# vlad17/runlmc

Measured on AMD Instinct MI355X. Metric: kronecker_toeplitz_mvms_per_sec, higher is better.
Workload: dtype f64

## Files before the change

### runlmc_amd/csrc/rl_direct.h

```cpp
#pragma once
#include "rl_device.h"

#define RL_DZ_VB 4

static __global__ void __launch_bounds__(256)
k_dz_mix(const double* __restrict__ part, const int* __restrict__ run_ptr, int nvec, int D, int r,
         const double* __restrict__ Zt, double* __restrict__ zhat) {
    RL_SMEM(smem);
    double* S = reinterpret_cast<double*>(smem);
    const int tid = threadIdx.x, Dr = D * r;
    const int v0 = blockIdx.x * RL_DZ_VB;
    for (int e = tid; e < Dr; e += 256) {
        const int b = e / r, j = e - b * r;
        const int c0 = run_ptr[b], c1 = run_ptr[b + 1];
#pragma unroll
        for (int k = 0; k < RL_DZ_VB; ++k) {
            const int v = v0 + k < nvec ? v0 + k : nvec - 1;
            const double* src = part + (size_t)v * r + j;
            double s = 0.0;
            for (int c = c0; c < c1; ++c) s += src[(size_t)c * nvec * r];
            S[k * Dr + e] = s;
        }
    }
    __syncthreads();
// ... 154 lines not shown
    S[(size_t)v * Dr + e] = s;
}
static __global__ void __launch_bounds__(256)
k_hz_map(const double* __restrict__ S, const double* __restrict__ Zt, int nvec, int Dr,
         double* __restrict__ P) {
    RL_SMEM(smem);
    double* Sl = reinterpret_cast<double*>(smem);
    const int tid = threadIdx.x, e = blockIdx.x * 256 + tid, v0 = blockIdx.y * RL_HZ_VB;
    const int per = (Dr + gridDim.z - 1) / gridDim.z;
    const int f0 = blockIdx.z * per, f1 = f0 + per < Dr ? f0 + per : Dr, flen = f1 > f0 ? f1 - f0 : 0;
    for (int t = tid; t < flen * RL_HZ_VB; t += 256) {
        const int q = t / flen, f = t - q * flen;
        const int v = v0 + q < nvec ? v0 + q : nvec - 1;
        Sl[f * RL_HZ_VB + q] = S[(size_t)v * Dr + f0 + f];
    }
    __syncthreads();
    if (e >= Dr) return;
    double acc[RL_HZ_VB];
#pragma unroll
    for (int q = 0; q < RL_HZ_VB; ++q) acc[q] = 0.0;
    const double* z = Zt + (size_t)f0 * Dr + e;
#pragma unroll 4
    for (int f = 0; f < flen; ++f) {
        const double zf = z[(size_t)f * Dr];
#pragma unroll
        for (int q = 0; q < RL_HZ_VB; ++q) acc[q] = fma(zf, Sl[f * RL_HZ_VB + q], acc[q]);
    }
#pragma unroll
    for (int q = 0; q < RL_HZ_VB; ++q)
        if (v0 + q < nvec) P[((size_t)blockIdx.z * nvec + v0 + q) * Dr + e] = acc[q];
}
static __global__ void __launch_bounds__(256)
k_hz_collect(const double* __restrict__ P, int nvec, int D, int NB, int slices,
             double* __restrict__ zhat, int nvp = 0) {
    const int R = NB * RL_HZ_BLK, Dr = D * R;
    const int e = blockIdx.x * 256 + threadIdx.x, v = blockIdx.y;
    if (e >= Dr) return;
    if (nvp > 0) {
        double s = 0.0;
        if (v < nvec)
            for (int t = 0; t < slices; ++t) s += P[((size_t)t * nvec + v) * Dr + e];
        zhat[(size_t)e * nvp + v] = s;
        return;
    }
    double s = 0.0;
    for (int t = 0; t < slices; ++t) s += P[((size_t)t * nvec + v) * Dr + e];
    const int a = e / R, ig = e - a * R, k = ig / RL_HZ_BLK, i = ig - k * RL_HZ_BLK;
    zhat[(((size_t)k * nvec + v) * D + a) * RL_HZ_BLK + i] = s;
}

template <int NVT, int RT = 2>
__global__ void __launch_bounds__(256)
k_hz_expand_mm(const double* __restrict__ zT, const double* __restrict__ F, int n, int nvec, int nvp,
               int D, int R, const int* __restrict__ out_end, double* __restrict__ out,
               const double* __restrict__ diag, const double* __restrict__ X2) {
    const int tid = threadIdx.x;
    const int vt0 = blockIdx.y * NVT, nvt = nvp / 16 - vt0 < NVT ? nvp / 16 - vt0 : NVT;
    constexpr int WR = 16 * RT;
#if !defined(RL_EMU)
    const int lane = tid & 63, wave = tid >> 6, li = lane & 15, lk = lane >> 4;
    const int r0 = blockIdx.x * (4 * WR) + wave * WR;
    if (r0 >= n) return;
    rp_double4 C[RT][NVT];
#pragma unroll
    for (int rt = 0; rt < RT; ++rt) {
        const int i = r0 + 16 * rt + li;
        const double dg = i < n ? diag[i] : 0.0;
#pragma unroll
        for (int t = 0; t < NVT; ++t) {
            rp_double4 c = rp_double4{0.0, 0.0, 0.0, 0.0};
            if (t < nvt) {
#pragma unroll
                for (int r = 0; r < 4; ++r) {
                    const int v = (vt0 + t) * 16 + lk + 4 * r;
                    c[r] = i < n && v < nvec ? dg * X2[(size_t)v * n + i] : 0.0;
                }
            }
            C[rt][t] = c;
        }
    }
    const int rlast = r0 + WR - 1 < n ? r0 + WR - 1 : n - 1;
    const int dlo = RL_LR_UNIFORM(rp_output_of(out_end, D, r0));
    const int dhi = RL_LR_UNIFORM(rp_output_of(out_end, D, rlast));
    int irow[RT], drow[RT];
#pragma unroll
    for (int rt = 0; rt < RT; ++rt) {
        irow[rt] = r0 + 16 * rt + li;
        drow[rt] = dlo == dhi ? dlo : rp_output_of(out_end, D, irow[rt] < n ? irow[rt] : n - 1);
    }
    for (int d = dlo; d <= dhi; ++d) {
        bool on[RT];
        const double* fr[RT];
#pragma unroll
        for (int rt = 0; rt < RT; ++rt) {
            on[rt] = irow[rt] < n && drow[rt] == d;
            fr[rt] = F + (size_t)lk * n + (irow[rt] < n ? irow[rt] : n - 1);
        }
        const double* za = zT + ((size_t)d * R + lk) * nvp + (size_t)vt0 * 16 + li;
        double a[3][NVT], b[3][RT];
        auto request = [&](int slot, int j) {
            const int jc = j < R ? j : R - 4;
            const double* zj = za + (size_t)jc * nvp;
#pragma unroll
            for (int t = 0; t < NVT; ++t) a[slot][t] = t < nvt ? zj[16 * t] : 0.0;
#pragma unroll
            for (int rt = 0; rt < RT; ++rt) b[slot][rt] = on[rt] ? fr[rt][(size_t)jc * n] : 0.0;
        };
        request(0, 0);
        request(1, 4);
        for (int j0 = 0; j0 < R; j0 += 12) {
#pragma unroll
            for (int u = 0; u < 3; ++u) {
                request((u + 2) % 3, j0 + 4 * u + 8);
#pragma unroll
                for (int t = 0; t < NVT; ++t) {
                    if (t < nvt) {
#pragma unroll
                        for (int rt = 0; rt < RT; ++rt)
                            C[rt][t] = __builtin_amdgcn_mfma_f64_16x16x4f64(a[u][t], b[u][rt], C[rt][t], 0, 0, 0);
                    }
                }
            }
        }
    }
#pragma unroll
    for (int rt = 0; rt < RT; ++rt) {
        const int i = r0 + 16 * rt + li;
#pragma unroll
        for (int t = 0; t < NVT; ++t) {
            if (t < nvt) {
#pragma unroll
                for (int r = 0; r < 4; ++r) {
                    const int v = (vt0 + t) * 16 + lk + 4 * r;
                    if (i < n && v < nvec) out[(size_t)v * n + i] = C[rt][t][r];
                }
            }
        }
    }
#else
    if (tid >= 4 * WR) return;
    const int i = blockIdx.x * (4 * WR) + tid;
    if (i >= n) return;
    const int d = rp_output_of(out_end, D, i);
    for (int t = 0; t < nvt; ++t)
        for (int q = 0; q < 16; ++q) {
            const int v = (vt0 + t) * 16 + q;
            if (v >= nvec) continue;
            double acc = diag[i] * X2[(size_t)v * n + i];
            for (int j = 0; j < R; ++j) acc = fma(F[(size_t)j * n + i], zT[((size_t)d * R + j) * nvp + v], acc);
            out[(size_t)v * n + i] = acc;
        }
#endif
}
```

### runlmc_amd/csrc/rl_exact.h

```cpp
#pragma once
#include "rl_device.h"

#define EX_T 64
#define EX_KC 32
#define EX_LDK (EX_KC + 1)
#define EX_LDT (EX_T + 1)
#define EX_MAX_SLOT 32
#define EX_MAX_COLS 4
#define EX_MAX_D 64

#define EX_RBF 0
#define EX_MATERN32 1
#define EX_STDPERIODIC 2
#define EX_MATERN52 3
#define EX_COSINE 4
#define EX_SCALED 16
#define EX_MAX_FACT 3
#define EX_PRM2 (4 * EX_MAX_SLOT)

#if !defined(RL_EMU)
typedef double ex_d4 __attribute__((ext_vector_type(4)));
#endif

__device__ __forceinline__ bool ex_bad_pivot(double p) { return !(p > 0.0 && p <= 1.7976931348623157e308); }
// ... 99 lines not shown
            k[f] = t[0];
            d[f][0] = t[1];
            if (leaf == EX_STDPERIODIC) d[f][1] = t[2];
        }
    }
    double val = k[0];
#pragma unroll
    for (int f = 1; f < NF; ++f) val = val * k[f];
#pragma unroll
    for (int p = 1; p < 8; ++p) v[p] = 0.0;
#pragma unroll
    for (int f = 0; f < NF; ++f) {
        double others = 1.0;
#pragma unroll
        for (int g = 0; g < NF; ++g)
            if (g != f) others = others * k[g];
        v[1 + 2 * f] = d[f][0] * others;
        v[2 + 2 * f] = d[f][1] * others;
    }
    v[0] = val;
    if (desc & EX_SCALED) {
        const double c = p0[2];
        v[7] = val;
#pragma unroll
        for (int p = 1; p < 7; ++p) v[p] = c * v[p];
        v[0] = c * val;
    }
}

template <int NF>
__device__ __forceinline__ double ex_value(int desc, const double* prm, int q, double r) {
    double v[8];
    ex_eval_fact<NF>(desc, prm, q, r, v);
    return v[0];
}

__device__ __forceinline__ double ex_dist(const double* xa, const double* xb, const int* cols) {
    double s = 0.0;
    for (int c = 0; c < EX_MAX_COLS; ++c) {
        const int col = cols[c];
        if (col < 0) break;
        const double d = xa[col] - xb[col];
        s += d * d;
    }
    return sqrt(s);
}

#define EX_LEAF_COLS (EX_MAX_FACT * EX_MAX_COLS)

__device__ __forceinline__ void ex_eval_sep(int desc, const double* prm, int q, const double* xa,
                                            const double* xb, const int* lq, double v[8]) {
    const int nf = ex_desc_nf(desc);
    const double r0 = ex_dist(xa, xb, lq);
    const double r1 = nf > 1 ? ex_dist(xa, xb, lq + EX_MAX_COLS) : 0.0;
    const double r2 = nf > 2 ? ex_dist(xa, xb, lq + 2 * EX_MAX_COLS) : 0.0;
    ex_eval_fact<EX_MAX_FACT, true>(desc, prm, q, r0, v, r1, r2);
}

template <int NF, bool SEP = false>
__global__ void __launch_bounds__(256)
k_ex_assemble(double* __restrict__ out, long long ldo, int nrows, int ncols,
              const double* __restrict__ Xa, const int* __restrict__ oa,
              const double* __restrict__ Xb, const int* __restrict__ ob, int P, int Q,
              const int* __restrict__ kinds, const double* __restrict__ prm,
              const int* __restrict__ cols, const double* __restrict__ Bm, int D,
              const double* __restrict__ noise, int diag_off, int lower) {
    if (lower && blockIdx.x > blockIdx.y) return;
    const int i0 = blockIdx.y * EX_T, j0 = blockIdx.x * EX_T;
    for (int u = 0; u < 16; ++u) {
        const int e = threadIdx.x + 256 * u;
        const int i = i0 + e / EX_T, j = j0 + e % EX_T;
        if (i >= nrows || j >= ncols) continue;
        const int a = oa[i], b = ob[j];
        double acc = 0.0;
        for (int q = 0; q < Q; ++q) {
            if constexpr (SEP) {
                double v[8];
                ex_eval_sep(kinds[q], prm, q, Xa + (long long)i * P, Xb + (long long)j * P,
                            cols + q * EX_LEAF_COLS, v);
                acc += Bm[((long long)q * D + a) * D + b] * v[0];
                continue;
            }
            const double r = ex_dist(Xa + (long long)i * P, Xb + (long long)j * P, cols + q * EX_MAX_COLS);
            if constexpr (NF == 1) {
                double v[4];
                ex_eval(kinds[q], prm + 4 * q, r, v);
                acc += Bm[((long long)q * D + a) * D + b] * v[0];
            } else {
                acc += Bm[((long long)q * D + a) * D + b] * ex_value<NF>(kinds[q], prm, q, r);
            }
        }
        if (noise && i + diag_off == j) acc += noise[a];
        out[(long long)i * ldo + j] = acc;
    }
}

#define EX_CR_COLS 256
template <int NF, bool SEP = false>
__global__ void __launch_bounds__(EX_CR_COLS)
k_ex_cross_rows(double* __restrict__ out, long long ldo, int nrows, int ncols, int rg,
                const double* __restrict__ Xt, const int* __restrict__ ot,
                const double* __restrict__ Xb, const int* __restrict__ ob, int P, int Q,
                const int* __restrict__ kinds, const double* __restrict__ prm,
                const int* __restrict__ cols, const double* __restrict__ Bm, int D,
                int stage_cols, int ldx) {
    RL_SMEM(smem);
    double* sx = reinterpret_cast<double*>(smem);
    double* sb = sx + (long long)rg * P;
    double* sc = sb + (long long)rg * Q * D;
    const int tid = threadIdx.x;
    const int t0 = blockIdx.y * rg;
    const int nt = nrows - t0 < rg ? nrows - t0 : rg;
    const long long j = (long long)blockIdx.x * EX_CR_COLS + tid;
    for (int e = tid; e < nt * P; e += EX_CR_COLS) sx[e] = Xt[(long long)t0 * P + e];
    const int QD = Q * D;
    for (int e = tid; e < nt * QD; e += EX_CR_COLS) {
        const int t = e / QD, r = e % QD, q = r / D, b = r % D;
        sb[e] = Bm[((long long)q * D + ot[t0 + t]) * D + b];
    }
    const double* xb = Xb + j * P;
    if (stage_cols) {
        if (j < ncols)
            for (int c = 0; c < P; ++c) sc[tid * ldx + c] = xb[c];
        xb = sc + tid * ldx;
    }
    __syncthreads();
    if (j >= ncols) return;
    const int b = ob[j];
    for (int t = 0; t < nt; ++t) {
        const double* xa = sx + t * P;
        const double* bt = sb + (long long)t * QD + b;
        double acc = 0.0;
        for (int q = 0; q < Q; ++q) {
            if constexpr (SEP) {
                double v[8];
                ex_eval_sep(kinds[q], prm, q, xa, xb, cols + q * EX_LEAF_COLS, v);
                acc += bt[q * D] * v[0];
                continue;
            }
            const double r = ex_dist(xa, xb, cols + q * EX_MAX_COLS);
            if constexpr (NF == 1) {
                double v[4];
                ex_eval(kinds[q], prm + 4 * q, r, v);
                acc += bt[q * D] * v[0];
            } else {
                acc += bt[q * D] * ex_value<NF>(kinds[q], prm, q, r);
            }
        }
        out[(long long)(t0 + t) * ldo + j] = acc;
    }
}

#define EX_RD_CHUNKS 64
__global__ void __launch_bounds__(256)
k_ex_rowdot_part(const double* __restrict__ B, const double* __restrict__ X, long long n,
                 double* __restrict__ part) {
    RL_SMEM(smem);
    double* rd = reinterpret_cast<double*>(smem);
    const int tid = threadIdx.x;
    const long long len = (n + EX_RD_CHUNKS - 1) / EX_RD_CHUNKS;
    const long long i0 = (long long)blockIdx.x * len;
    const long long i1 = i0 + len < n ? i0 + len : n;
    const double* b = B + (long long)blockIdx.y * n;
    const double* x = X + (long long)blockIdx.y * n;
    double dot = 0.0, sq = 0.0;
    for (long long i = i0 + tid; i < i1; i += 256) {
        const double xi = x[i];
        dot += b[i] * xi;
        sq += xi * xi;
    }
    rd[tid] = dot;
    rd[256 + tid] = sq;
    __syncthreads();
    for (int w = 128; w > 0; w >>= 1) {
        if (tid < w) {
            rd[tid] += rd[tid + w];
            rd[256 + tid] += rd[256 + tid + w];
        }
        __syncthreads();
    }
    if (tid == 0) {
        double* p = part + ((long long)blockIdx.y * EX_RD_CHUNKS + blockIdx.x) * 2;
        p[0] = rd[0];
        p[1] = rd[256];
    }
}

__global__ void __launch_bounds__(64)
k_ex_rowdot_sum(const double* __restrict__ part, int k, double* __restrict__ dots,
                double* __restrict__ sqn) {
    const int v = blockIdx.x * 64 + threadIdx.x;
    if (v >= k) return;
    double dot = 0.0, sq = 0.0;
    for (int c = 0; c < EX_RD_CHUNKS; ++c) {
        dot += part[((long long)v * EX_RD_CHUNKS + c) * 2];
        sq += part[((long long)v * EX_RD_CHUNKS + c) * 2 + 1];
    }
    dots[v] = dot;
    sqn[v] = sq;
}

__global__ void __launch_bounds__(256)
k_ex_potrf_diag(double* __restrict__ A, long long lda, int k0, int nk, double* __restrict__ logd,
                int* __restrict__ flag) {
    RL_SMEM(smem);
    double* s = reinterpret_cast<double*>(smem);
    const int tid = threadIdx.x;
    double* base = A + (long long)k0 * lda + k0;
    for (int e = tid; e < nk * nk; e += 256) {
        const int r = e / nk, c = e % nk;
        s[r * EX_LDT + c] = c <= r ? base[(long long)r * lda + c] : 0.0;
    }
    __syncthreads();
    for (int j = 0; j < nk; ++j) {
        const double piv = s[j * EX_LDT + j];
        const double d = sqrt(piv);
        if (tid == 0 && ex_bad_pivot(piv) && *flag > k0 + j) *flag = k0 + j;
        if (tid > j && tid < nk) s[tid * EX_LDT + j] /= d;
        __syncthreads();
        const int m = nk - j - 1;
        for (int e = tid; e < m * m; e += 256) {
            const int r = j + 1 + e / m, c = j + 1 + e % m;
            if (c <= r) s[r * EX_LDT + c] -= s[r * EX_LDT + j] * s[c * EX_LDT + j];
        }
        if (tid == 0) s[j * EX_LDT + j] = d;
        __syncthreads();
    }
    for (int e = tid; e < nk * nk; e += 256) {
        const int r = e / nk, c = e % nk;
        if (c <= r) base[(long long)r * lda + c] = s[r * EX_LDT + c];
    }
    if (tid < nk) logd[k0 + tid] = log(s[tid * EX_LDT + tid]);
}

__global__ void __launch_bounds__(64)
k_ex_trsm_panel(double* __restrict__ A, long long lda, int k0, int nk, int r0, int nrows) {
    RL_SMEM(smem);
    double* L = reinterpret_cast<double*>(smem);
    double* X = L + EX_T * EX_LDT;
    const int tid = threadIdx.x;
    const int row0 = r0 + blockIdx.x * EX_T;
    const int rows = nrows - blockIdx.x * EX_T < EX_T ? nrows - blockIdx.x * EX_T : EX_T;
    const double* Lg = A + (long long)k0 * lda + k0;
    double* Xg = A + (long long)row0 * lda + k0;
    for (int e = tid; e < nk * nk; e += 64) {
        const int r = e / nk, c = e % nk;
        L[r * EX_LDT + c] = c <= r ? Lg[(long long)r * lda + c] : 0.0;
    }
    for (int e = tid; e < rows * nk; e += 64) {
        const int r = e / nk, c = e % nk;
        X[r * EX_LDT + c] = Xg[(long long)r * lda + c];
    }
    __syncthreads();
    if (tid < rows) {
        double* x = X + tid * EX_LDT;
        for (int c = 0; c < nk; ++c) {
            double v = x[c];
            for (int t = 0; t < c; ++t) v -= x[t] * L[c * EX_LDT + t];
            x[c] = v / L[c * EX_LDT + c];
        }
    }
    __syncthreads();
    for (int e = tid; e < rows * nk; e += 64) {
        const int r = e / nk, c = e % nk;
        Xg[(long long)r * lda + c] = X[r * EX_LDT + c];
    }
}

__global__ void __launch_bounds__(64)
k_ex_trtri_diag(double* __restrict__ A, long long lda, int j0, int nk) {
    RL_SMEM(smem);
    double* L = reinterpret_cast<double*>(smem);
    double* W = L + EX_T * EX_LDT;
    const int tid = threadIdx.x;
    double* base = A + (long long)j0 * lda + j0;
    for (int e = tid; e < nk * nk; e += 64) {
        const int r = e / nk, c = e % nk;
        L[r * EX_LDT + c] = c <= r ? base[(long long)r * lda + c] : 0.0;
    }
    __syncthreads();
    if (tid < nk) {
        const int c = tid;
        for (int r = 0; r < c; ++r) W[r * EX_LDT + c] = 0.0;
        W[c * EX_LDT + c] = 1.0 / L[c * EX_LDT + c];
        for (int r = c + 1; r < nk; ++r) {
            double v = 0.0;
            for (int t = c; t < r; ++t) v += L[r * EX_LDT + t] * W[t * EX_LDT + c];
            W[r * EX_LDT + c] = -v / L[r * EX_LDT + r];
        }
    }
    __syncthreads();
    for (int e = tid; e < nk * nk; e += 64) {
        const int r = e / nk, c = e % nk;
        base[(long long)r * lda + c] = W[r * EX_LDT + c];
    }
}

__global__ void __launch_bounds__(64)
k_ex_trsv_diag(const double* __restrict__ A, long long lda, int k0, int nk, double* __restrict__ R,
               long long ldr, int nrhs, int trans) {
    RL_SMEM(smem);
    double* L = reinterpret_cast<double*>(smem);
    double* X = L + EX_T * EX_LDT;
    const int tid = threadIdx.x;
    const int v0 = blockIdx.x * EX_T;
    const int nv = nrhs - v0 < EX_T ? nrhs - v0 : EX_T;
    const double* Lg = A + (long long)k0 * lda + k0;
    for (int e = tid; e < nk * nk; e += 64) {
        const int r = e / nk, c = e % nk;
        L[r * EX_LDT + c] = c <= r ? Lg[(long long)r * lda + c] : 0.0;
    }
    for (int e = tid; e < nv * nk; e += 64) {
        const int v = e / nk, c = e % nk;
        X[v * EX_LDT + c] = R[(long long)(v0 + v) * ldr + k0 + c];
    }
    __syncthreads();
    if (tid < nv) {
        double* x = X + tid * EX_LDT;
        if (!trans) {
            for (int c = 0; c < nk; ++c) {
                double s = x[c];
                for (int t = 0; t < c; ++t) s -= L[c * EX_LDT + t] * x[t];
                x[c] = s / L[c * EX_LDT + c];
            }
        } else {
            for (int c = nk - 1; c >= 0; --c) {
                double s = x[c];
                for (int t = c + 1; t < nk; ++t) s -= L[t * EX_LDT + c] * x[t];
                x[c] = s / L[c * EX_LDT + c];
            }
        }
    }
    __syncthreads();
    for (int e = tid; e < nv * nk; e += 64) {
        const int v = e / nk, c = e % nk;
        R[(long long)(v0 + v) * ldr + k0 + c] = X[v * EX_LDT + c];
    }
}

__global__ void __launch_bounds__(256)
k_ex_gemm(double* __restrict__ C, long long ldc, const double* __restrict__ A, long long sai,
          long long sak, const double* __restrict__ B, long long sbj, long long sbk, int M, int N,
          int K, int kchunk, int a_lower, double s, int beta, int lower_tiles,
          double* __restrict__ P) {
    const int tn = blockIdx.x, tm = blockIdx.y, z = blockIdx.z;
    if (lower_tiles && tn > tm) return;
    const int i0 = tm * EX_T, j0 = tn * EX_T;
    const int kb = z * kchunk;
    int ke = K < kb + kchunk ? K : kb + kchunk;
    if (a_lower && ke > i0 + EX_T) ke = i0 + EX_T;
    RL_SMEM(smem);
    double* sA = reinterpret_cast<double*>(smem);
    double* sB = sA + EX_T * EX_LDK;
    const int tid = threadIdx.x;
#if !defined(RL_EMU)
    const int lane = tid & 63, wave = tid >> 6, li = lane & 15, lk = lane >> 4;
    const int wm = (wave >> 1) * 32, wn = (wave & 1) * 32;
    ex_d4 acc[2][2];
#pragma unroll
    for (int a = 0; a < 2; ++a)
#pragma unroll
        for (int b = 0; b < 2; ++b) acc[a][b] = ex_d4{0.0, 0.0, 0.0, 0.0};
#else
    const int er = tid >> 2, ec = (tid & 3) * 16;
    double acc[16];
    for (int c = 0; c < 16; ++c) acc[c] = 0.0;
#endif
    for (int k0 = kb; k0 < ke; k0 += EX_KC) {
        for (int e = tid; e < EX_T * EX_KC; e += 256) {
            int r, k;
            if (sak == 1) { r = e / EX_KC; k = e % EX_KC; } else { k = e / EX_T; r = e % EX_T; }
            const int gi = i0 + r, gk = k0 + k;
            sA[r * EX_LDK + k] = gi < M && gk < ke ? A[(long long)gi * sai + (long long)gk * sak] : 0.0;
            if (sbk == 1) { r = e / EX_KC; k = e % EX_KC; } else { k = e / EX_T; r = e % EX_T; }
            const int gj = j0 + r, gk2 = k0 + k;
            sB[r * EX_LDK + k] = gj < N && gk2 < ke ? B[(long long)gj * sbj + (long long)gk2 * sbk] : 0.0;
        }
        __syncthreads();
#if !defined(RL_EMU)
#pragma unroll
        for (int kk = 0; kk < EX_KC; kk += 4) {
            const double a0 = sA[(wm + li) * EX_LDK + kk + lk];
            const double a1 = sA[(wm + 16 + li) * EX_LDK + kk + lk];
            const double b0 = sB[(wn + li) * EX_LDK + kk + lk];
            const double b1 = sB[(wn + 16 + li) * EX_LDK + kk + lk];
            acc[0][0] = __builtin_amdgcn_mfma_f64_16x16x4f64(a0, b0, acc[0][0], 0, 0, 0);
            acc[0][1] = __builtin_amdgcn_mfma_f64_16x16x4f64(a0, b1, acc[0][1], 0, 0, 0);
            acc[1][0] = __builtin_amdgcn_mfma_f64_16x16x4f64(a1, b0, acc[1][0], 0, 0, 0);
            acc[1][1] = __builtin_amdgcn_mfma_f64_16x16x4f64(a1, b1, acc[1][1], 0, 0, 0);
        }
#else
        for (int c = 0; c < 16; ++c)
            for (int kk = 0; kk < EX_KC; ++kk) acc[c] += sA[er * EX_LDK + kk] * sB[(ec + c) * EX_LDK + kk];
#endif
        __syncthreads();
    }
    auto put = [&](int i, int j, double v) {
        if (i >= M || j >= N) return;
        if (P) {
            P[(long long)z * M * N + (long long)i * N + j] = v;
        } else {
            double* c = C + (long long)i * ldc + j;
            *c = beta ? *c + s * v : s * v;
        }
    };
#if !defined(RL_EMU)
#pragma unroll
    for (int a = 0; a < 2; ++a)
#pragma unroll
        for (int b = 0; b < 2; ++b)
#pragma unroll
            for (int r = 0; r < 4; ++r)
                put(i0 + wm + 16 * a + lk + 4 * r, j0 + wn + 16 * b + li, acc[a][b][r]);
#else
    for (int c = 0; c < 16; ++c) put(i0 + er, j0 + ec + c, acc[c]);
#endif
}

__global__ void __launch_bounds__(256)
k_ex_reduce(double* __restrict__ C, long long ldc, const double* __restrict__ P, int M, int N,
            int nsplit, double s, int beta) {
    const long long e = (long long)blockIdx.x * 256 + threadIdx.x;
    const long long MN = (long long)M * N;
    if (e >= MN) return;
    double acc = 0.0;
    for (int z = 0; z < nsplit; ++z) acc += P[z * MN + e];
    const long long i = e / N, j = e % N;
    double* c = C + i * ldc + j;
    *c = beta ? *c + s * acc : s * acc;
}

__global__ void __launch_bounds__(256)
k_ex_rownorm2(const double* __restrict__ V, long long n, double* __restrict__ out) {
    RL_SMEM(smem);
    double* red = reinterpret_cast<double*>(smem);
    const double* row = V + (long long)blockIdx.x * n;
    double acc = 0.0;
    for (long long i = threadIdx.x; i < n; i += 256) acc += row[i] * row[i];
    red[threadIdx.x] = acc;
    __syncthreads();
    for (int w = 128; w > 0; w >>= 1) {
        if ((int)threadIdx.x < w) red[threadIdx.x] += red[threadIdx.x + w];
        __syncthreads();
    }
    if (threadIdx.x == 0) out[blockIdx.x] = red[0];
}

__global__ void __launch_bounds__(256)
k_ex_sum2(const double* __restrict__ x, int n, double* __restrict__ out) {
    RL_SMEM(smem);
    double* red = reinterpret_cast<double*>(smem);
    double acc = 0.0;
    for (int i = threadIdx.x; i < n; i += 256) acc += x[i];
    red[threadIdx.x] = acc;
    __syncthreads();
    for (int w = 128; w > 0; w >>= 1) {
        if ((int)threadIdx.x < w) red[threadIdx.x] += red[threadIdx.x + w];
        __syncthreads();
    }
    if (threadIdx.x == 0) *out = 2.0 * red[0];
}

template <int NF, bool SEP = false>
__global__ void __launch_bounds__(256)
k_ex_grad_tiles(const double* __restrict__ Kinv, long long n, const double* __restrict__ alpha,
                const int* __restrict__ tiles, const int* __restrict__ bounds,
                const double* __restrict__ X, int P, int Q, const int* __restrict__ kinds,
                const double* __restrict__ prm, const int* __restrict__ cols,
                const int* __restrict__ dslot, int nslot, double* __restrict__ part) {
    RL_SMEM(smem);
    double* red = reinterpret_cast<double*>(smem);
    const int tid = threadIdx.x, w = blockIdx.x;
    const int r0 = tiles[4 * w], c0 = tiles[4 * w + 1], a = tiles[4 * w + 2], b = tiles[4 * w + 3];
    const int re = bounds[a + 1] < r0 + EX_T ? bounds[a + 1] : r0 + EX_T;
    const int ce = bounds[b + 1] < c0 + EX_T ? bounds[b + 1] : c0 + EX_T;
    double mw[16];
    double dsum = 0.0;
    for (int u = 0; u < 16; ++u) {
        const int e = tid + 256 * u;
        const int i = r0 + e / EX_T, j = c0 + e % EX_T;
        double m = 0.0;
        if (i < re && j < ce && (a != b || j <= i)) {
            m = alpha[i] * alpha[j] - Kinv[(long long)i * n + j];
            if (i == j) dsum += m;
            else if (a == b) m *= 2.0;
        }
        mw[u] = m;
    }
    red[nslot * 256 + tid] = dsum;
    for (int q = 0; q < Q; ++q) {
        const int kind = kinds[q];
        const double* pq = prm + 4 * q;
        const int* cq = cols + q * (SEP ? EX_LEAF_COLS : EX_MAX_COLS);
        if constexpr (NF == 1) {
            double s0 = 0.0, s1 = 0.0, s2 = 0.0, s3 = 0.0;
            int np = 0;
            for (int u = 0; u < 16; ++u) {
                const int e = tid + 256 * u;
                const int i = r0 + e / EX_T, j = c0 + e % EX_T;
                if (i >= re || j >= ce || (a == b && j > i)) continue;
                double v[4];
                np = ex_eval(kind, pq, ex_dist(X + (long long)i * P, X + (long long)j * P, cq), v);
                const double m = mw[u];
                s0 += m * v[0];
                s1 += m * v[1];
                if (np > 1) s2 += m * v[2];
                if (np > 2) s3 += m * v[3];
            }
            np = ex_nder(kind);
            red[q * 256 + tid] = s0;
            red[(dslot[q] + 0) * 256 + tid] = s1;
            if (np > 1) red[(dslot[q] + 1) * 256 + tid] = s2;
            if (np > 2) red[(dslot[q] + 2) * 256 + tid] = s3;
        } else {
            double s[8];
#pragma unroll
            for (int p = 0; p < 8; ++p) s[p] = 0.0;
            for (int u = 0; u < 16; ++u) {
                const int e = tid + 256 * u;
                const int i = r0 + e / EX_T, j = c0 + e % EX_T;
                if (i >= re || j >= ce || (a == b && j > i)) continue;
                double v[8];
                if constexpr (SEP)
                    ex_eval_sep(kind, prm, q, X + (long long)i * P, X + (long long)j * P, cq, v);
                else
                    ex_eval_fact<NF>(kind, prm, q, ex_dist(X + (long long)i * P, X + (long long)j * P, cq), v);
                const double m = mw[u];
#pragma unroll
                for (int p = 0; p < 8; ++p) s[p] += m * v[p];
            }
            red[q * 256 + tid] = s[0];
            int slot = dslot[q];
            const int nf = ex_desc_nf(kind);
#pragma unroll
            for (int f = 0; f < NF; ++f) {
                if (f >= nf) continue;
                red[slot * 256 + tid] = s[1 + 2 * f];
                if (ex_leaf_nder(ex_desc_leaf(kind, f)) > 1) red[(slot + 1) * 256 + tid] = s[2 + 2 * f];
                slot += ex_leaf_nder(ex_desc_leaf(kind, f));
            }
            if (kind & EX_SCALED) red[slot * 256 + tid] = s[7];
        }
    }
    __syncthreads();
    if (tid <= nslot) {
        double acc = 0.0;
        for (int t = 0; t < 256; ++t) acc += red[tid * 256 + t];
        part[(long long)w * (nslot + 1) + tid] = acc;
    }
}

__global__ void __launch_bounds__(64)
k_ex_grad_reduce(const double* __restrict__ part, const int* __restrict__ pair_start, int D,
                 int nslot, double* __restrict__ out) {
    const int p = blockIdx.x;
    int a = 0;
    while ((a + 1) * (a + 2) / 2 <= p) ++a;
    const int b = p - a * (a + 1) / 2;
    for (int s = threadIdx.x; s <= nslot; s += 64) {
        double acc = 0.0;
        for (int w = pair_start[p]; w < pair_start[p + 1]; ++w) acc += part[(long long)w * (nslot + 1) + s];
        if (s < nslot) {
            out[((long long)s * D + a) * D + b] = acc;
            out[((long long)s * D + b) * D + a] = acc;
        } else if (a == b) {
            out[(long long)nslot * D * D + a] = acc;
        }
    }
}
```

### runlmc_amd/csrc/rl_exact.hip

```cpp
#include "rl_host.h"
#include "rl_exact.h"

enum { EX_EMPTY = 0, EX_SET, EX_ASSEMBLED, EX_FACTORED, EX_INVERTED };

struct rl_exact {
    int device = 0, n = 0, P = 0, D = 0, Q = 0, nslot = 0, ncu = 1;
    int maxf = 1;
    int sep = 0;
    int state = EX_EMPTY;
    double* A = nullptr;
    double* X = nullptr;
    int* out_of = nullptr;
    int* bounds = nullptr;
    int* kinds = nullptr;
    double* prm = nullptr;
    int* cols = nullptr;
    int* dslot = nullptr;
    double* Bm = nullptr;
    double* noise = nullptr;
    double* logd = nullptr;
    double* scal = nullptr;
    int* flag = nullptr;
    double* ws = nullptr;
    size_t ws_cap = 0;
    int* tiles = nullptr;
    int* pair_start = nullptr;
    int ntiles = 0;
    double* gout = nullptr;
    double* xt = nullptr;
    int* ot = nullptr;
    size_t xt_cap = 0, ot_cap = 0;
    std::vector<int> lens, hbounds;
};

static int ex_ws(rl_exact* h, size_t doubles) {
    if (doubles <= h->ws_cap) return RL_OK;
    if (h->ws) RL_HIP(hipFree(h->ws));
    h->ws = nullptr;
    h->ws_cap = 0;
    if (hipMalloc((void**)&h->ws, doubles * sizeof(double)) != hipSuccess) {
        (void)hipGetLastError();
        return fail(RL_ENOMEM, "rl_exact: no device memory for a workspace of " +
                                   std::to_string(doubles * 8 >> 20) + " MB");
    }
    h->ws_cap = doubles;
    return RL_OK;
}

#define EX_LAUNCH_FACT(h, kern, grid, block, smem, stream, ...)                         \
    do {                                                                                \
        if ((h)->sep)                                                                   \
            RL_LAUNCH((kern<EX_MAX_FACT, true>), grid, block, smem, stream, __VA_ARGS__); \
        else if ((h)->maxf == 1)                                                        \
            RL_LAUNCH(kern<1>, grid, block, smem, stream, __VA_ARGS__);                 \
        else                                                                            \
            RL_LAUNCH(kern<EX_MAX_FACT>, grid, block, smem, stream, __VA_ARGS__);       \
    } while (0)

static inline int ex_tiles(long long v) { return (int)((v + EX_T - 1) / EX_T); }
static const size_t kGemmLds = 2 * EX_T * EX_LDK * sizeof(double);
static const size_t kTileLds = 2 * EX_T * EX_LDT * sizeof(double);

static int ex_gemm(rl_exact* h, hipStream_t st, double* C, long long ldc, const double* A,
                   long long sai, long long sak, const double* B, long long sbj, long long sbk,
                   int M, int N, int K, double s, int beta, int lower_tiles, int a_lower,
                   bool via_partials) {
    if (M <= 0 || N <= 0) return RL_OK;
    const int tm = ex_tiles(M), tn = ex_tiles(N);
    const long long ntile = lower_tiles ? (long long)tm * (tm + 1) / 2 : (long long)tm * tn;
    const long long target = 2LL * h->ncu;
    int nsplit = 1;
    if (!lower_tiles && ntile < target) {
        const long long want = (target + ntile - 1) / ntile;
        const int kmax = ex_tiles(K);
        nsplit = (int)(want < kmax ? want : kmax);
    }
    if (nsplit < 1) nsplit = 1;
    int kchunk = (K + nsplit - 1) / nsplit;
    kchunk = (kchunk + EX_KC - 1) / EX_KC * EX_KC;
    if (kchunk < EX_KC) kchunk = EX_KC;
    nsplit = (K + kchunk - 1) / kchunk;
    if (nsplit < 1) nsplit = 1;
    if (nsplit == 1 && !via_partials) {
        RL_LAUNCH(k_ex_gemm, dim3(tn, tm, 1), dim3(256), kGemmLds, st, C, ldc, A, sai, sak, B, sbj,
                  sbk, M, N, K, kchunk, a_lower, s, beta, lower_tiles, (double*)nullptr);
        RL_HIP(hipGetLastError());
        return RL_OK;
    }
    RL_TRY(ex_ws(h, (size_t)nsplit * M * N));
    RL_LAUNCH(k_ex_gemm, dim3(tn, tm, nsplit), dim3(256), kGemmLds, st, C, ldc, A, sai, sak, B, sbj,
              sbk, M, N, K, kchunk, a_lower, s, beta, 0, h->ws);
    RL_HIP(hipGetLastError());
    const long long MN = (long long)M * N;
    RL_LAUNCH(k_ex_reduce, dim3((unsigned)((MN + 255) / 256)), dim3(256), 0, st, C, ldc,
              (const double*)h->ws, M, N, nsplit, s, beta);
    RL_HIP(hipGetLastError());
    return RL_OK;
}

static int ex_trsv(rl_exact* h, hipStream_t st, double* R, int nrhs, bool forward, bool backward) {
    const int n = h->n, nb = ex_tiles(n);
    const dim3 g(ex_tiles(nrhs));
    if (forward) {
        for (int k = 0; k < nb; ++k) {
            const int k0 = k * EX_T, nk = std::min(EX_T, n - k0), rest = n - k0 - nk;
            RL_LAUNCH(k_ex_trsv_diag, g, dim3(64), kTileLds, st, (const double*)h->A, (long long)n,
                      k0, nk, R, (long long)n, nrhs, 0);
            RL_HIP(hipGetLastError());
            RL_TRY(ex_gemm(h, st, R + k0 + nk, n, R + k0, n, 1, h->A + (long long)(k0 + nk) * n + k0,
                           n, 1, nrhs, rest, nk, -1.0, 1, 0, 0, false));
        }
    }
    if (backward) {
        for (int k = nb - 1; k >= 0; --k) {
            const int k0 = k * EX_T, nk = std::min(EX_T, n - k0);
            RL_LAUNCH(k_ex_trsv_diag, g, dim3(64), kTileLds, st, (const double*)h->A, (long long)n,
                      k0, nk, R, (long long)n, nrhs, 1);
            RL_HIP(hipGetLastError());
            RL_TRY(ex_gemm(h, st, R, n, R + k0, n, 1, h->A + (long long)k0 * n, 1, n, nrhs, k0, nk,
                           -1.0, 1, 0, 0, false));
        }
    }
    return RL_OK;
}

static int ex_cross(rl_exact* h, hipStream_t st, double* out, const double* Xa, const int* oa,
                    int nrows, const double* noise, int diag_off) {
    if (nrows <= 0) return RL_OK;
    EX_LAUNCH_FACT(h, k_ex_assemble, dim3(ex_tiles(h->n), ex_tiles(nrows)), dim3(256), 0, st, out,
              (long long)h->n, nrows, h->n, Xa, oa, (const double*)h->X, (const int*)h->out_of,
              h->P, h->Q, (const int*)h->kinds, (const double*)h->prm, (const int*)h->cols,
              (const double*)h->Bm, h->D, noise, diag_off, 0);
    RL_HIP(hipGetLastError());
    return RL_OK;
}

extern "C" int rl_exact_create(int device, int n, int P, rl_exact** out) {
    if (!out) return fail(RL_EINVAL, "rl_exact_create: out is NULL");
    *out = nullptr;
    if (n < 1 || P < 1) return fail(RL_EINVAL, "rl_exact_create: n and P must be >= 1");
    if ((long long)n * P > (1LL << 31)) return fail(RL_ELIMIT, "rl_exact_create: n * P too large");
    RL_HIP(hipSetDevice(device));
    rl_exact* h = new rl_exact;
    HandleGuard<rl_exact, rl_exact_destroy> guard(h);
    h->device = device;
    h->n = n;
    h->P = P;
    hipDeviceProp_t prop;
    RL_HIP(hipGetDeviceProperties(&prop, device));
    h->ncu = std::max(1, prop.multiProcessorCount);
    RL_HIP(hipMalloc((void**)&h->X, (size_t)n * P * sizeof(double)));
    RL_HIP(hipMalloc((void**)&h->out_of, (size_t)n * sizeof(int)));
    RL_HIP(hipMalloc((void**)&h->bounds, (EX_MAX_D + 1) * sizeof(int)));
    RL_HIP(hipMalloc((void**)&h->kinds, EX_MAX_SLOT * sizeof(int)));
    RL_HIP(hipMalloc((void**)&h->prm, 2 * EX_PRM2 * sizeof(double)));
    RL_HIP(hipMalloc((void**)&h->cols, EX_MAX_SLOT * EX_LEAF_COLS * sizeof(int)));
    RL_HIP(hipMalloc((void**)&h->dslot, EX_MAX_SLOT * sizeof(int)));
    RL_HIP(hipMalloc((void**)&h->Bm, (size_t)EX_MAX_SLOT * EX_MAX_D * EX_MAX_D * sizeof(double)));
    RL_HIP(hipMalloc((void**)&h->noise, EX_MAX_D * sizeof(double)));
    RL_HIP(hipMalloc((void**)&h->logd, (size_t)n * sizeof(double)));
    RL_HIP(hipMalloc((void**)&h->scal, sizeof(double)));
    RL_HIP(hipMalloc((void**)&h->flag, sizeof(int)));
    RL_HIP(hipMalloc((void**)&h->gout,
                     ((size_t)EX_MAX_SLOT * EX_MAX_D * EX_MAX_D + EX_MAX_D) * sizeof(double)));
    (void)hipFuncSetAttribute((const void*)k_ex_grad_tiles<1>,
                              hipFuncAttributeMaxDynamicSharedMemorySize,
                              (EX_MAX_SLOT + 1) * 256 * (int)sizeof(double));
    (void)hipFuncSetAttribute((const void*)k_ex_grad_tiles<EX_MAX_FACT>,
                              hipFuncAttributeMaxDynamicSharedMemorySize,
                              (EX_MAX_SLOT + 1) * 256 * (int)sizeof(double));
    (void)hipFuncSetAttribute((const void*)k_ex_grad_tiles<EX_MAX_FACT, true>,
                              hipFuncAttributeMaxDynamicSharedMemorySize,
                              (EX_MAX_SLOT + 1) * 256 * (int)sizeof(double));
    *out = guard.release();
    return RL_OK;
}

extern "C" int rl_exact_destroy(rl_exact* h) {
    if (!h) return RL_OK;
    (void)hipSetDevice(h->device);
    for (void* p : {(void*)h->A, (void*)h->X, (void*)h->out_of, (void*)h->bounds, (void*)h->kinds,
                    (void*)h->prm, (void*)h->cols, (void*)h->dslot, (void*)h->Bm, (void*)h->noise,
                    (void*)h->logd, (void*)h->scal, (void*)h->flag, (void*)h->ws, (void*)h->tiles,
                    (void*)h->pair_start, (void*)h->gout, (void*)h->xt, (void*)h->ot})
        if (p) (void)hipFree(p);
    delete h;
    return RL_OK;
}

template <class Describe>
static int ex_set(rl_exact* h, const char* what, const double* X, const int* lens, int D, int Q,
                  Describe describe, const int* active_cols, const double* B, const double* noise,
                  bool sep = false) {
    const std::string fn = what;
    const int stride = sep ? EX_LEAF_COLS : EX_MAX_COLS;
    if (D > EX_MAX_D) return fail(RL_ELIMIT, fn + ": D > 64 outputs");
    long long total = 0;
    for (int d = 0; d < D; ++d) {
        if (lens[d] < 0) return fail(RL_EINVAL, fn + ": negative output length");
        total += lens[d];
    }
    if (total != h->n)
        return fail(RL_EINVAL, fn + ": lens sum to " + std::to_string(total) + ", handle has n = " +
                                   std::to_string(h->n));
    long long nslot = Q;
    int maxf = 1;
    std::vector<int> descs(EX_MAX_SLOT, 0), dslot(EX_MAX_SLOT, 0), cols((size_t)EX_MAX_SLOT * EX_LEAF_COLS, -1);
    std::vector<double> prm(2 * EX_PRM2, 0.0);
    for (int q = 0; q < Q; ++q) {
        int desc = 0;
        double p0[4] = {0.0, 0.0, 0.0, 0.0}, p1[4] = {0.0, 0.0, 0.0, 0.0};
        RL_TRY(describe(q, &desc, p0, p1));
        const int slot = (int)std::min<long long>(nslot, EX_MAX_SLOT);
        nslot += ex_desc_nder(desc);
        maxf = std::max(maxf, ex_desc_nf(desc));
        if (ex_desc_leaf(desc, 0) == EX_COSINE) maxf = EX_MAX_FACT;
        const bool keep = q < EX_MAX_SLOT;
        if (keep) {
            descs[q] = desc;
            dslot[q] = slot;
            for (int p = 0; p < 4; ++p) {
                prm[4 * q + p] = p0[p];
                prm[EX_PRM2 + 4 * q + p] = p1[p];
            }
        }
        for (int f = 0; f < (sep ? ex_desc_nf(desc) : 1); ++f) {
            const int* list = active_cols + (size_t)q * stride + f * EX_MAX_COLS;
            int nc = 0;
            for (int c = 0; c < EX_MAX_COLS; ++c) {
                const int col = list[c];
                if (col >= h->P) return fail(RL_EINVAL, fn + ": active column beyond P");
                if (col < 0) break;
                ++nc;
            }
            if (nc == 0)
                return fail(RL_EINVAL, fn + (sep ? ": leaf " + std::to_string(f) + " of kernel " + std::to_string(q) +
                                                       " without active columns"
                                                 : std::string(": a kernel without active columns")));
            if (keep)
                for (int c = 0; c < EX_MAX_COLS; ++c)
                    cols[(size_t)q * stride + f * EX_MAX_COLS + c] = c < nc ? list[c] : -1;
        }
    }
    if (nslot > EX_MAX_SLOT)
        return fail(RL_ELIMIT, fn + ": Q + sum of kernel parameters = " + std::to_string(nslot) +
                                   " > 32");
    RL_HIP(hipSetDevice(h->device));
    std::vector<int> out_of(h->n), bounds(D + 1, 0);
    for (int d = 0, i = 0; d < D; ++d) {
        for (int k = 0; k < lens[d]; ++k) out_of[i++] = d;
        bounds[d + 1] = bounds[d] + lens[d];
    }
    RL_HIP(hipMemcpy(h->X, X, (size_t)h->n * h->P * sizeof(double), hipMemcpyHostToDevice));
    RL_HIP(hipMemcpy(h->out_of, out_of.data(), (size_t)h->n * sizeof(int), hipMemcpyHostToDevice));
    RL_HIP(hipMemcpy(h->bounds, bounds.data(), (D + 1) * sizeof(int), hipMemcpyHostToDevice));
    RL_HIP(hipMemcpy(h->kinds, descs.data(), Q * sizeof(int), hipMemcpyHostToDevice));
    RL_HIP(hipMemcpy(h->prm, prm.data(), 2 * EX_PRM2 * sizeof(double), hipMemcpyHostToDevice));
    RL_HIP(hipMemcpy(h->cols, cols.data(), (size_t)Q * stride * sizeof(int), hipMemcpyHostToDevice));
    RL_HIP(hipMemcpy(h->dslot, dslot.data(), Q * sizeof(int), hipMemcpyHostToDevice));
    RL_HIP(hipMemcpy(h->Bm, B, (size_t)Q * D * D * sizeof(double), hipMemcpyHostToDevice));
    RL_HIP(hipMemcpy(h->noise, noise, D * sizeof(double), hipMemcpyHostToDevice));
    if (h->lens != std::vector<int>(lens, lens + D) || h->D != D) {
        std::vector<int> tl, ps(1, 0);
        for (int a = 0; a < D; ++a)
            for (int b = 0; b <= a; ++b) {
                for (int r0 = bounds[a]; r0 < bounds[a + 1]; r0 += EX_T)
                    for (int c0 = bounds[b]; c0 < bounds[b + 1]; c0 += EX_T) {
                        if (a == b && c0 - bounds[b] > r0 - bounds[a]) continue;
                        tl.insert(tl.end(), {r0, c0, a, b});
                    }
                ps.push_back((int)tl.size() / 4);
            }
        if (h->tiles) RL_HIP(hipFree(h->tiles));
        if (h->pair_start) RL_HIP(hipFree(h->pair_start));
        h->tiles = nullptr;
        h->pair_start = nullptr;
        RL_TRY(upload(&h->tiles, tl));
        RL_TRY(upload(&h->pair_start, ps));
        h->ntiles = (int)tl.size() / 4;
        h->lens.assign(lens, lens + D);
    }
    h->D = D;
    h->Q = Q;
    h->nslot = (int)nslot;
    h->maxf = sep ? EX_MAX_FACT : maxf;
    h->sep = sep ? 1 : 0;
    h->hbounds = bounds;
    h->state = EX_SET;
    return RL_OK;
}

extern "C" int rl_exact_set(rl_exact* h, const double* X, const int* lens, int D, int Q,
                            const int* kinds, const double* params, const int* active_cols,
                            const double* B, const double* noise) {
    if (!h || !X || !lens || !kinds || !params || !active_cols || !B || !noise)
        return fail(RL_EINVAL, "rl_exact_set: NULL argument");
    if (D < 1 || Q < 1) return fail(RL_EINVAL, "rl_exact_set: D and Q must be >= 1");
    auto describe = [&](int q, int* desc, double* p0, double*) -> int {
        const int base = kinds[q] & ~EX_SCALED;
        if (base != EX_RBF && base != EX_MATERN32 && base != EX_STDPERIODIC && base != EX_MATERN52)
            return fail(RL_EINVAL, "rl_exact_set: unknown kernel kind " + std::to_string(kinds[q]));
        *desc = kinds[q];
        for (int p = 0; p < 4; ++p) p0[p] = params[q * 4 + p];
        return RL_OK;
    };
    return ex_set(h, "rl_exact_set", X, lens, D, Q, describe, active_cols, B, noise);
}

extern "C" int rl_exact_set_factors(rl_exact* h, const double* X, const int* lens, int D, int Q,
                                    const int* nfact, const int* leaf_kinds,
                                    const double* leaf_params, const int* scaled,
                                    const double* scales, const int* active_cols, const double* B,
                                    const double* noise) {
    if (!h || !X || !lens || !nfact || !leaf_kinds || !leaf_params || !scaled || !scales ||
        !active_cols || !B || !noise)
        return fail(RL_EINVAL, "rl_exact_set_factors: NULL argument");
    if (D < 1 || Q < 1) return fail(RL_EINVAL, "rl_exact_set_factors: D and Q must be >= 1");
    auto describe = [&](int q, int* desc, double* p0, double* p1) -> int {
        const int nf = nfact[q];
        if (nf < 1 || nf > EX_MAX_FACT)
            return fail(RL_EINVAL, "rl_exact_set_factors: kernel " + std::to_string(q) + " has " +
                                       std::to_string(nf) + " factors (1 .. 3)");
        const int* leaf = leaf_kinds + (size_t)q * EX_MAX_FACT;
        for (int f = 0; f < nf; ++f) {
            if (leaf[f] != EX_RBF && leaf[f] != EX_MATERN32 && leaf[f] != EX_STDPERIODIC &&
                leaf[f] != EX_MATERN52 && leaf[f] != EX_COSINE)
                return fail(RL_EINVAL, "rl_exact_set_factors: unknown kernel kind " + std::to_string(leaf[f]));
            double* pf = f == 0 ? p0 : p1 + 2 * (f - 1);
            pf[0] = leaf_params[((size_t)q * EX_MAX_FACT + f) * 2];
            pf[1] = leaf_params[((size_t)q * EX_MAX_FACT + f) * 2 + 1];
        }
        p0[2] = scaled[q] ? scales[q] : 0.0;
        *desc = ex_desc(leaf, nf, scaled[q] != 0);
        return RL_OK;
    };
    return ex_set(h, "rl_exact_set_factors", X, lens, D, Q, describe, active_cols, B, noise);
}

extern "C" int rl_exact_set_separable(rl_exact* h, const double* X, const int* lens, int D, int Q,
                                      const int* nfact, const int* leaf_kinds,
                                      const double* leaf_params, const int* leaf_cols,
                                      const int* scaled, const double* scales, const double* B,
                                      const double* noise) {
    if (!h || !X || !lens || !nfact || !leaf_kinds || !leaf_params || !leaf_cols || !scaled ||
        !scales || !B || !noise)
        return fail(RL_EINVAL, "rl_exact_set_separable: NULL argument");
    if (D < 1 || Q < 1) return fail(RL_EINVAL, "rl_exact_set_separable: D and Q must be >= 1");
    auto describe = [&](int q, int* desc, double* p0, double* p1) -> int {
        const int nf = nfact[q];
        if (nf < 1 || nf > EX_MAX_FACT)
            return fail(RL_EINVAL, "rl_exact_set_separable: kernel " + std::to_string(q) + " has " +
                                       std::to_string(nf) + " factors (1 .. 3)");
        const int* leaf = leaf_kinds + (size_t)q * EX_MAX_FACT;
        for (int f = 0; f < nf; ++f) {
            if (leaf[f] != EX_RBF && leaf[f] != EX_MATERN32 && leaf[f] != EX_STDPERIODIC &&
                leaf[f] != EX_MATERN52 && leaf[f] != EX_COSINE)
                return fail(RL_EINVAL, "rl_exact_set_separable: unknown kernel kind " + std::to_string(leaf[f]));
            double* pf = f == 0 ? p0 : p1 + 2 * (f - 1);
            pf[0] = leaf_params[((size_t)q * EX_MAX_FACT + f) * 2];
            pf[1] = leaf_params[((size_t)q * EX_MAX_FACT + f) * 2 + 1];
        }
        p0[2] = scaled[q] ? scales[q] : 0.0;
        *desc = ex_desc(leaf, nf, scaled[q] != 0);
        return RL_OK;
    };
    return ex_set(h, "rl_exact_set_separable", X, lens, D, Q, describe, leaf_cols, B, noise, true);
}

extern "C" int rl_exact_assemble(rl_exact* h) {
    if (!h) return fail(RL_EINVAL, "rl_exact_assemble: NULL handle");
    if (h->state < EX_SET) return fail(RL_EINVAL, "rl_exact_assemble: no parameters (rl_exact_set)");
    RL_HIP(hipSetDevice(h->device));
    const int n = h->n;
    if (!h->A) {
        const size_t bytes = (size_t)n * n * sizeof(double);
        size_t fr = 0, tot = 0;
        RL_HIP(hipMemGetInfo(&fr, &tot));
        if (bytes + ((size_t)64 << 20) > fr)
            return fail(RL_ENOMEM, "rl_exact: the " + std::to_string(n) + " x " + std::to_string(n) +
                                       " matrix needs " + std::to_string(bytes >> 20) + " MB, " +
                                       std::to_string(fr >> 20) + " MB free");
        if (hipMalloc((void**)&h->A, bytes) != hipSuccess) {
            (void)hipGetLastError();
            h->A = nullptr;
            return fail(RL_ENOMEM, "rl_exact: hipMalloc of the n x n matrix failed");
        }
    }
    const int nb = ex_tiles(n);
    EX_LAUNCH_FACT(h, k_ex_assemble, dim3(nb, nb), dim3(256), 0, (hipStream_t)0, h->A, (long long)n, n, n,
              (const double*)h->X, (const int*)h->out_of, (const double*)h->X,
              (const int*)h->out_of, h->P, h->Q, (const int*)h->kinds, (const double*)h->prm,
              (const int*)h->cols, (const double*)h->Bm, h->D, (const double*)h->noise, 0, 1);
    RL_HIP(hipGetLastError());
    RL_HIP(hipStreamSynchronize(0));
    h->state = EX_ASSEMBLED;
    return RL_OK;
}

extern "C" int rl_exact_factor(rl_exact* h, double* logdet, int* bad_col) {
    if (!h) return fail(RL_EINVAL, "rl_exact_factor: NULL handle");
    if (bad_col) *bad_col = -1;
    if (h->state != EX_ASSEMBLED) RL_TRY(rl_exact_assemble(h));
    RL_HIP(hipSetDevice(h->device));
    const int n = h->n, nb = ex_tiles(n);
    const hipStream_t st = 0;
    RL_HIP(hipMemsetAsync(h->flag, 0x7f, sizeof(int), st));
    for (int k = 0; k < nb; ++k) {
        const int k0 = k * EX_T, nk = std::min(EX_T, n - k0), r0 = k0 + nk, rest = n - r0;
        RL_LAUNCH(k_ex_potrf_diag, dim3(1), dim3(256), EX_T * EX_LDT * sizeof(double), st, h->A,
                  (long long)n, k0, nk, h->logd, h->flag);
        RL_HIP(hipGetLastError());
        if (rest == 0) break;
        RL_LAUNCH(k_ex_trsm_panel, dim3(ex_tiles(rest)), dim3(64), kTileLds, st, h->A, (long long)n,
                  k0, nk, r0, rest);
        RL_HIP(hipGetLastError());
        double* L21 = h->A + (long long)r0 * n + k0;
        RL_TRY(ex_gemm(h, st, h->A + (long long)r0 * n + r0, n, L21, n, 1, L21, n, 1, rest, rest, nk,
                       -1.0, 1, 1, 0, false));
    }
    RL_LAUNCH(k_ex_sum2, dim3(1), dim3(256), 256 * sizeof(double), st, (const double*)h->logd, n,
              h->scal);
    RL_HIP(hipGetLastError());
    int flag = 0;
    double ld = 0.0;
    RL_HIP(hipMemcpy(&flag, h->flag, sizeof(int), hipMemcpyDeviceToHost));
    RL_HIP(hipMemcpy(&ld, h->scal, sizeof(double), hipMemcpyDeviceToHost));
    if (flag >= 0 && flag < n) {
        h->state = EX_SET;
        if (bad_col) *bad_col = flag;
        return fail(RL_ENOTPD, "rl_exact_factor: the matrix is not positive definite: pivot of column " +
                                   std::to_string(flag) + " is not a positive finite number");
    }
    if (logdet) *logdet = ld;
    h->state = EX_FACTORED;
    return RL_OK;
}

extern "C" int rl_exact_solve(rl_exact* h, const double* B, double* X, int nrhs, void* stream) {
    if (!h || !B || !X) return fail(RL_EINVAL, "rl_exact_solve: NULL argument");
    if (nrhs < 0) return fail(RL_EINVAL, "rl_exact_solve: nrhs < 0");
    if (h->state != EX_FACTORED)
        return fail(RL_EINVAL, "rl_exact_solve: the handle holds no Cholesky factor (rl_exact_factor)");
    if (nrhs == 0) return RL_OK;
    RL_HIP(hipSetDevice(h->device));
    const hipStream_t st = (hipStream_t)stream;
    if (X != B)
        RL_HIP(hipMemcpyAsync(X, B, (size_t)nrhs * h->n * sizeof(double), hipMemcpyDeviceToDevice, st));
    return ex_trsv(h, st, X, nrhs, true, true);
}

static int ex_upload_test(rl_exact* h, const double* Xt, const int* tlens, double** dX, int** dO, int* nt) {
    long long total = 0;
    for (int d = 0; d < h->D; ++d) {
        if (tlens[d] < 0) return fail(RL_EINVAL, "rl_exact: negative test length");
        total += tlens[d];
    }
    if (total > (1LL << 30)) return fail(RL_ELIMIT, "rl_exact: too many test points");
    *nt = (int)total;
    std::vector<int> o((size_t)total);
    for (int d = 0, i = 0; d < h->D; ++d)
        for (int k = 0; k < tlens[d]; ++k) o[i++] = d;
    RL_HIP(hipMalloc((void**)dX, std::max<size_t>(1, (size_t)total * h->P) * sizeof(double)));
    RL_HIP(hipMalloc((void**)dO, std::max<size_t>(1, (size_t)total) * sizeof(int)));
    if (total) {
        RL_HIP(hipMemcpy(*dX, Xt, (size_t)total * h->P * sizeof(double), hipMemcpyHostToDevice));
        RL_HIP(hipMemcpy(*dO, o.data(), (size_t)total * sizeof(int), hipMemcpyHostToDevice));
    }
    return RL_OK;
}

struct ExTmp {
    void* p[3] = {nullptr, nullptr, nullptr};
    ~ExTmp() { for (void* q : p) if (q) (void)hipFree(q); }
};

static int ex_chunk_rows(const rl_exact* h) {
    const long long r = ((long long)256 << 20) / (8LL * h->n);
    return (int)std::max(1LL, std::min(r, (long long)1 << 20));
}

static int ex_cross_rows(rl_exact* h, const double* Xt, const int* tlens, const double* noise,
                         double* out_host, double* var_out) {
    if (h->state < EX_SET) return fail(RL_EINVAL, "rl_exact: no parameters (rl_exact_set)");
    RL_HIP(hipSetDevice(h->device));
    ExTmp t;
    int nt = 0;
    if (Xt) {
        RL_TRY(ex_upload_test(h, Xt, tlens, (double**)&t.p[0], (int**)&t.p[1], &nt));
    } else {
        nt = h->n;
    }
    if (nt == 0) return RL_OK;
    const int rows = std::min(nt, ex_chunk_rows(h));
    if (hipMalloc(&t.p[2], (size_t)rows * h->n * sizeof(double)) != hipSuccess) {
        (void)hipGetLastError();
        return fail(RL_ENOMEM, "rl_exact: no device memory for the cross-covariance");
    }
    double* V = (double*)t.p[2];
    double* norms = nullptr;
    if (var_out) RL_TRY(ex_ws(h, (size_t)rows));
    for (int r0 = 0; r0 < nt; r0 += rows) {
        const int nr = std::min(rows, nt - r0);
        const double* xa = Xt ? (const double*)t.p[0] + (long long)r0 * h->P : h->X + (long long)r0 * h->P;
        const int* oa = Xt ? (const int*)t.p[1] + r0 : h->out_of + r0;
        RL_TRY(ex_cross(h, 0, V, xa, oa, nr, noise, r0));
        if (var_out) {
            RL_TRY(ex_trsv(h, 0, V, nr, true, false));
            norms = h->ws;
            RL_LAUNCH(k_ex_rownorm2, dim3(nr), dim3(256), 256 * sizeof(double), (hipStream_t)0,
                      (const double*)V, (long long)h->n, norms);
            RL_HIP(hipGetLastError());
            RL_HIP(hipMemcpy(var_out + r0, norms, (size_t)nr * sizeof(double), hipMemcpyDeviceToHost));
        } else {
            RL_HIP(hipMemcpy(out_host + (long long)r0 * h->n, V, (size_t)nr * h->n * sizeof(double),
                             hipMemcpyDeviceToHost));
        }
    }
    return RL_OK;
}

extern "C" int rl_exact_cross_host(rl_exact* h, const double* Xtest, const int* test_lens,
                                   double* out) {
    if (!h || !Xtest || !test_lens || !out) return fail(RL_EINVAL, "rl_exact_cross_host: NULL argument");
    return ex_cross_rows(h, Xtest, test_lens, nullptr, out, nullptr);
}

extern "C" int rl_exact_dense_host(rl_exact* h, double* out) {
    if (!h || !out) return fail(RL_EINVAL, "rl_exact_dense_host: NULL argument");
    return ex_cross_rows(h, nullptr, nullptr, h->noise, out, nullptr);
}

extern "C" int rl_exact_explained_variance(rl_exact* h, const double* Xtest, const int* test_lens,
                                           double* out) {
    if (!h || !Xtest || !test_lens || !out)
        return fail(RL_EINVAL, "rl_exact_explained_variance: NULL argument");
    if (h->state != EX_FACTORED)
        return fail(RL_EINVAL, "rl_exact_explained_variance: the handle holds no Cholesky factor");
    return ex_cross_rows(h, Xtest, test_lens, nullptr, nullptr, out);
}

static const size_t kCrossRowLds = 32 << 10, kCrossColLds = 16 << 10;

extern "C" int rl_exact_cross_dev(rl_exact* h, const double* Xtest, const int* test_lens, int row0,
                                  int nrows, double* out, void* stream) {
    if (!h || !Xtest || !test_lens || !out) return fail(RL_EINVAL, "rl_exact_cross_dev: NULL argument");
    if (h->state < EX_SET) return fail(RL_EINVAL, "rl_exact_cross_dev: no parameters (rl_exact_set)");
    long long nt = 0;
    for (int d = 0; d < h->D; ++d) {
        if (test_lens[d] < 0) return fail(RL_EINVAL, "rl_exact_cross_dev: negative test length");
        nt += test_lens[d];
    }
    if (nt > (1LL << 30)) return fail(RL_ELIMIT, "rl_exact_cross_dev: too many test points");
    if (row0 < 0 || nrows < 0 || (long long)row0 + nrows > nt)
        return fail(RL_EINVAL, "rl_exact_cross_dev: rows " + std::to_string(row0) + " .. " +
                                   std::to_string((long long)row0 + nrows) + " of " +
                                   std::to_string(nt) + " test points");
    if (nrows == 0) return RL_OK;
    const int P = h->P, Q = h->Q, D = h->D;
    const size_t row_bytes = ((size_t)P + (size_t)Q * D) * sizeof(double);
    if (row_bytes > kCrossRowLds)
        return fail(RL_ELIMIT, "rl_exact_cross_dev: one test row (P + Q D = " +
                                   std::to_string(row_bytes / 8) + " values) exceeds the kernel's LDS");
    RL_HIP(hipSetDevice(h->device));
    const hipStream_t st = (hipStream_t)stream;
    std::vector<int> o((size_t)nrows);
    {
        long long begin = 0;
        for (int d = 0; d < D; ++d) {
            const long long end = begin + test_lens[d];
            const long long a = std::max<long long>(begin, row0), b = std::min<long long>(end, (long long)row0 + nrows);
            for (long long i = a; i < b; ++i) o[(size_t)(i - row0)] = d;
            begin = end;
        }
    }
    if (h->xt_cap < (size_t)nrows * P) {
        if (h->xt) RL_HIP(hipFree(h->xt));
        h->xt = nullptr;
        h->xt_cap = 0;
        RL_HIP(hipMalloc((void**)&h->xt, (size_t)nrows * P * sizeof(double)));
        h->xt_cap = (size_t)nrows * P;
    }
    if (h->ot_cap < (size_t)nrows) {
        if (h->ot) RL_HIP(hipFree(h->ot));
        h->ot = nullptr;
        h->ot_cap = 0;
        RL_HIP(hipMalloc((void**)&h->ot, (size_t)nrows * sizeof(int)));
        h->ot_cap = (size_t)nrows;
    }
    RL_HIP(hipMemcpyAsync(h->xt, Xtest + (long long)row0 * P, (size_t)nrows * P * sizeof(double),
                          hipMemcpyHostToDevice, st));
    RL_HIP(hipMemcpyAsync(h->ot, o.data(), (size_t)nrows * sizeof(int), hipMemcpyHostToDevice, st));
    RL_HIP(hipStreamSynchronize(st));
    const int ldx = P | 1;
    const int stage_cols = (size_t)EX_CR_COLS * ldx * sizeof(double) <= kCrossColLds ? 1 : 0;
    const int rg = (int)std::min<size_t>({(size_t)nrows, (size_t)EX_T, kCrossRowLds / row_bytes});
    const size_t lds = (size_t)rg * row_bytes + (stage_cols ? (size_t)EX_CR_COLS * ldx * sizeof(double) : 0);
    const long long gx = ((long long)h->n + EX_CR_COLS - 1) / EX_CR_COLS;
    const int gy = (nrows + rg - 1) / rg;
    if (gy > 65535) return fail(RL_ELIMIT, "rl_exact_cross_dev: too many row groups in one call");
    EX_LAUNCH_FACT(h, k_ex_cross_rows, dim3((unsigned)gx, (unsigned)gy), dim3(EX_CR_COLS), lds, st, out,
              (long long)h->n, nrows, h->n, rg, (const double*)h->xt, (const int*)h->ot,
              (const double*)h->X, (const int*)h->out_of, P, Q, (const int*)h->kinds,
              (const double*)h->prm, (const int*)h->cols, (const double*)h->Bm, D, stage_cols, ldx);
    RL_HIP(hipGetLastError());
    return RL_OK;
}

extern "C" int rl_row_dots(const double* B, const double* X, int nvec, long long n, double* dots,
                           double* sqnorms, double* ws, void* stream) {
    if (!B || !X || !dots || !sqnorms || !ws) return fail(RL_EINVAL, "rl_row_dots: NULL argument");
    if (nvec < 0 || n < 1) return fail(RL_EINVAL, "rl_row_dots: bad sizes");
    if (nvec > 65535) return fail(RL_ELIMIT, "rl_row_dots: more than 65535 rows in one call");
    if (nvec == 0) return RL_OK;
    const hipStream_t st = (hipStream_t)stream;
    RL_LAUNCH(k_ex_rowdot_part, dim3(EX_RD_CHUNKS, nvec), dim3(256), 512 * sizeof(double), st, B, X,
              n, ws);
    RL_HIP(hipGetLastError());
    RL_LAUNCH(k_ex_rowdot_sum, dim3((nvec + 63) / 64), dim3(64), 0, st, (const double*)ws, nvec,
              dots, sqnorms);
    RL_HIP(hipGetLastError());
    return RL_OK;
}

extern "C" int rl_exact_invert(rl_exact* h) {
    if (!h) return fail(RL_EINVAL, "rl_exact_invert: NULL handle");
    if (h->state == EX_INVERTED) return RL_OK;
    if (h->state != EX_FACTORED)
        return fail(RL_EINVAL, "rl_exact_invert: the handle holds no Cholesky factor (rl_exact_factor)");
    RL_HIP(hipSetDevice(h->device));
    const int n = h->n, nb = ex_tiles(n);
    const long long ld = n;
    double* A = h->A;
    const hipStream_t st = 0;
    double* tmp = nullptr;
    if (hipMalloc((void**)&tmp, (size_t)n * EX_T * sizeof(double)) != hipSuccess) {
        (void)hipGetLastError();
        return fail(RL_ENOMEM, "rl_exact_invert: no device memory for an n x 64 panel");
    }
    ExTmp guard;
    guard.p[0] = tmp;
    for (int j = nb - 1; j >= 0; --j) {
        const int j0 = j * EX_T, nj = std::min(EX_T, n - j0), r0 = j0 + nj, rest = n - r0;
        RL_LAUNCH(k_ex_trtri_diag, dim3(1), dim3(64), kTileLds, st, A, ld, j0, nj);
        RL_HIP(hipGetLastError());
        if (rest == 0) continue;
        RL_TRY(ex_gemm(h, st, tmp, EX_T, A + (long long)r0 * n + r0, n, 1, A + (long long)r0 * n + j0, 1, n,
                       rest, nj, rest, 1.0, 0, 0, 1, false));
        RL_TRY(ex_gemm(h, st, A + (long long)r0 * n + j0, n, tmp, EX_T, 1, A + (long long)j0 * n + j0, 1, n,
                       rest, nj, nj, -1.0, 0, 0, 0, false));
    }
    for (int i = 0; i < nb; ++i) {
        const int i0 = i * EX_T, ni = std::min(EX_T, n - i0);
        RL_TRY(ex_gemm(h, st, A + (long long)i0 * n, n, A + (long long)i0 * n + i0, 1, n,
                       A + (long long)i0 * n, 1, n, ni, i0 + ni, n - i0, 1.0, 0, 0, 0, true));
    }
    RL_HIP(hipStreamSynchronize(st));
    h->state = EX_INVERTED;
    return RL_OK;
}

extern "C" int rl_exact_grad_sums(rl_exact* h, const double* alpha, double* out) {
    if (!h || !alpha || !out) return fail(RL_EINVAL, "rl_exact_grad_sums: NULL argument");
    if (h->state != EX_INVERTED) RL_TRY(rl_exact_invert(h));
    RL_HIP(hipSetDevice(h->device));
    const int D = h->D, ns = h->nslot;
    const hipStream_t st = 0;
    const size_t nout = (size_t)ns * D * D + D;
    RL_HIP(hipMemsetAsync(h->gout, 0, nout * sizeof(double), st));
    if (h->ntiles > 0) {
        RL_TRY(ex_ws(h, (size_t)h->ntiles * (ns + 1)));
        EX_LAUNCH_FACT(h, k_ex_grad_tiles, dim3(h->ntiles), dim3(256), (size_t)(ns + 1) * 256 * sizeof(double),
                  st, (const double*)h->A, (long long)h->n, alpha, (const int*)h->tiles,
                  (const int*)h->bounds, (const double*)h->X, h->P, h->Q, (const int*)h->kinds,
                  (const double*)h->prm, (const int*)h->cols, (const int*)h->dslot, ns, h->ws);
        RL_HIP(hipGetLastError());
    }
    RL_LAUNCH(k_ex_grad_reduce, dim3(D * (D + 1) / 2), dim3(64), 0, st, (const double*)h->ws,
              (const int*)h->pair_start, D, ns, h->gout);
    RL_HIP(hipGetLastError());
    RL_HIP(hipMemcpy(out, h->gout, nout * sizeof(double), hipMemcpyDeviceToHost));
    return RL_OK;
}
```

### runlmc_amd/csrc/rl_gridop.hip

```cpp
#include "rl_host.h"
#include "rl_lead.h"

static thread_local std::string g_err;

int fail(int code, const std::string& msg) {
    g_err = msg;
    return code;
}

extern "C" const char* rl_last_error(void) { return g_err.c_str(); }
extern "C" const char* rl_backend(void) { return RL_BACKEND_NAME; }
extern "C" int rl_abi_version(void) { return RL_ABI_VERSION; }
extern "C" int rl_device_count(int* count) {
    if (!count) return fail(RL_EINVAL, "count is NULL");
    RL_HIP(hipGetDeviceCount(count));
    return RL_OK;
}

void trace_once(const char* what) {
    static const bool on = getenv("RUNLMC_TRACE") != nullptr;
    if (!on) return;
    static std::vector<std::string> seen;
    for (const std::string& s : seen)
        if (s == what) return;
    seen.push_back(what);
    fprintf(stderr, "[runlmc] %s\n", what);
}

bool first_on_device(unsigned long long* seen) {
    int dev = 0;
    (void)hipGetDevice(&dev);
    const unsigned long long bit = 1ull << (dev & 63);
    if (*seen & bit) return false;
    *seen |= bit;
    return true;
}

RlKnobs read_knobs() {
    RlKnobs k;
    const char* dbg = getenv("RUNLMC_DEBUG");
    const bool debug = dbg != nullptr && dbg[0] != '\0' && dbg[0] != '0';
    auto ignored = [](const char* n) {
        static std::vector<std::string> told;
        if (std::find(told.begin(), told.end(), std::string(n)) == told.end()) {
            told.push_back(n);
            fprintf(stderr, "runlmc_hip: %s is a debug switch and is ignored without RUNLMC_DEBUG=1\n", n);
        }
    };
    auto user_flag = [](const char* n) { return getenv(n) != nullptr; };
    auto user_num = [](const char* n, long long dflt) {
        const char* e = getenv(n);
        return e ? atoll(e) : dflt;
    };
    auto flag = [&](const char* n) {
        if (getenv(n) == nullptr) return false;
        if (!debug) ignored(n);
        return debug;
    };
    auto num = [&](const char* n, long long dflt) {
        const char* e = getenv(n);
        if (e == nullptr) return dflt;
        if (!debug) ignored(n);
        return debug ? atoll(e) : dflt;
    };
    k.pow2_only = user_flag("RUNLMC_POW2_ONLY");
    k.chunk_mb = (int)num("RUNLMC_CHUNK_MB", 0);
    k.two_streams = (int)num("RUNLMC_TWO_STREAMS", -1);
    k.affine = (int)num("RUNLMC_AFFINE", -1);
    k.affine_kb = (int)num("RUNLMC_AFFINE_KB", 0);
    k.affine_max_kb = (int)num("RUNLMC_AFFINE_MAX_KB", 2048);
    k.no_v1p = flag("RUNLMC_NO_V1P");
    k.v1p_min = (int)num("RUNLMC_V1P_MIN", 0);
    k.no_lowrank = flag("RUNLMC_NO_LOWRANK");
    k.no_filter = flag("RUNLMC_NO_FILTER");
    k.no_lr_bound = flag("RUNLMC_NO_LR_BOUND");
    k.sf_carries1 = flag("RUNLMC_SF_CARRIES1");
    k.sf_scan2 = flag("RUNLMC_SF_SCAN2");
    k.poly_round = flag("RUNLMC_POLY_ROUND");
    k.no_poly_round = flag("RUNLMC_NO_POLY_ROUND");
    k.lr_min = num("RUNLMC_LR_MIN", -1);
    k.staged_wt = flag("RUNLMC_STAGED_WT");
    k.no_staged_wt = flag("RUNLMC_NO_STAGED_WT");
    k.no_w_poly = flag("RUNLMC_NO_W_POLY");
    k.no_rp = flag("RUNLMC_NO_RP");
    k.rp_stagger = (int)num("RUNLMC_RP_STAGGER", 7);
    k.no_lr_small = flag("RUNLMC_NO_LR_SMALL");
    k.lr_expand_plain = (int)num("RUNLMC_LR_EXPAND_PLAIN", 0);
    k.lr_policy = (int)num("RUNLMC_LR_POLICY", -1);
    if (k.lr_policy < 0) {
        k.lr_policy = -1;
    } else if (k.lr_policy > RL_LR_POLICY_MAX || ((k.lr_policy >> 1) & 3) == 3) {
        fprintf(stderr, "runlmc_hip: RUNLMC_LR_POLICY=%d names no policy and is ignored\n", k.lr_policy);
        k.lr_policy = -1;
    }
    k.no_precond_approx = flag("RUNLMC_NO_PRECOND_APPROX");
    k.no_precond_hi = flag("RUNLMC_NO_PRECOND_HI");
    k.precond_hi_passes = flag("RUNLMC_PRECOND_HI_PASSES");
    k.no_precond_hi_mixed = flag("RUNLMC_NO_PRECOND_HI_MIXED");
    k.precond_hi_min = num("RUNLMC_PRECOND_HI_MIN", 100000);
    k.precond_hi_rank = (int)num("RUNLMC_PRECOND_HI_RANK", 192);
    k.precond_hi_use = (int)num("RUNLMC_PRECOND_HI_USE", 0);
    k.rp_fly = (int)num("RUNLMC_RP_FLY", 1);
    k.no_rp_small = flag("RUNLMC_NO_RP_SMALL");
    k.no_rp_fuse = flag("RUNLMC_NO_RP_FUSE");
    k.rp_pfuse = !flag("RUNLMC_NO_RP_PFUSE");
    k.w_pfuse = !flag("RUNLMC_NO_W_PFUSE");
    k.rp_runlen = (int)num("RUNLMC_RP_RUNLEN", 0);
    k.w_poly_rmax = std::min(36, (int)num("RUNLMC_W_POLY_RMAX", 32));
    k.no_sort = flag("RUNLMC_NO_SORT");
    k.ws_cache_mb = user_num("RUNLMC_WS_CACHE_MB", -1);
    k.solver_maxblk = (int)num("RUNLMC_SOLVER_MAXBLK", 0);
    k.no_fuse_w = flag("RUNLMC_NO_FUSE_W");
    k.no_fuse_wt = flag("RUNLMC_NO_FUSE_WT");
    k.no_graph = flag("RUNLMC_NO_GRAPH");
#if defined(RL_EMU)
    k.minres_v1 = flag("RUNLMC_MINRES_V1");
#endif
    return k;
}

static int ilog2(int x) {
    int l = 0;
    while ((1 << l) < x) ++l;
    return l;
}

static FftPlan make_plan(int n) {
    FftPlan p;
    p.n = n;
    p.npass = 0;
    for (int i = 0; i < RL_MAX_PASSES; ++i) p.radix[i] = 1;
    int rem = n;
    for (int odd : {3, 5})
        while (rem % odd == 0 && p.npass < 2) {
            p.radix[p.npass++] = odd;
            rem /= odd;
        }
    const int fixed[7][4] = {{8, 8, 0, 0},     {16, 16, 0, 0},   {64, 8, 8, 0},
                             {128, 8, 16, 0},  {256, 16, 16, 0}, {512, 8, 8, 8},
                             {1024, 8, 8, 16}};
    for (const auto& f : fixed)
        if (f[0] == rem) {
            for (int i = 1; i < 4 && f[i]; ++i) p.radix[p.npass++] = f[i];
            return p;
        }
    while (rem > 1) {
        int r = 8;
        while (rem % r) r /= 2;
        p.radix[p.npass++] = r;
        rem /= r;
    }
    return p;
}

static bool make_plan_rows3(int n, FftPlan* p) {
    int ra, rb;
    switch (n) {
        case 128: ra = 8; rb = 8; break;
        case 256: ra = 16; rb = 8; break;
        case 512: ra = 16; rb = 16; break;
        default: return false;
    }
    p->n = n;
    p->npass = 3;
    for (int i = 0; i < RL_MAX_PASSES; ++i) p->radix[i] = 1;
    p->radix[0] = ra;
    p->radix[1] = rb;
    p->radix[2] = 2;
    return true;
}

static int fused_code(const FftPlan& p) {
    if (p.npass < 2 || p.npass > 4) return 0;
    const int ra = p.radix[0], rb = p.radix[p.npass - 1];
    const int code = ra * 100 + rb;
    switch (code) {
        case 808: case 816: case 1616: return p.n >= 64 ? code : 0;
        case 308: case 316: case 508: case 516: return code;
        default: return 0;
    }
}

static void choose_length(int m, bool pow2_only, int* L_out, int* N1_out, int* N2_out) {
    long best = 0;
    int best_odd = 1;
    for (int odd : {1, 3, 5, 9, 15, 25}) {
        if (odd != 1 && pow2_only) continue;
        long L = odd;
        while (L < 2L * m || L < 16) L *= 2;
        if (odd != 1 && L / odd < 64 * 8) continue;
        if (best == 0 || L < best) { best = L; best_odd = odd; }
    }
    const int L = (int)best;
    const int P = L / best_odd;
    const int l = ilog2(P);
    int N2 = 1 << ((l + 1) / 2);
    if (best_odd != 1) {
        int bestN2 = 0;
        double bestScore = 1e300;
        for (int n2 = 64; n2 <= 1024 && n2 <= P / 8; n2 *= 2) {
            const int p1 = P / n2;
            if (p1 != 8 && p1 != 16 && p1 != 64 && p1 != 128 && p1 != 256) continue;
            const double score = std::fabs(std::log2((double)best_odd * p1 / n2));
            if (score < bestScore) { bestScore = score; bestN2 = n2; }
        }
        if (bestN2) N2 = bestN2;
    }
    *L_out = L;
    *N2_out = N2;
    *N1_out = L / N2;
}

static std::vector<int> position_to_freq(const FftPlan& p) {
    std::vector<int> f(p.n);
    for (int pos = 0; pos < p.n; ++pos) {
        int rem = pos, ns = p.n, mult = 1, k = 0;
        for (int s = 0; s < p.npass; ++s) {
            int sub = ns / p.radix[s];
            int d = rem / sub;
            rem -= d * sub;
            k += d * mult;
            mult *= p.radix[s];
            ns = sub;
        }
        f[pos] = k;
    }
    return f;
}

static void root_of_unity(long k, long n, double* re, double* im) {
    k %= n;
    const long double two_pi = 6.283185307179586476925286766559005768L;
    long double ang = two_pi * (long double)k / (long double)n;
    *re = (double)cosl(ang);
    *im = (double)(-sinl(ang));
}

static std::vector<cplx> unity_table(long count, long stride, long n) {
    std::vector<cplx> t(count);
    for (long i = 0; i < count; ++i) root_of_unity(i * stride, n, &t[i].x, &t[i].y);
    return t;
}


static size_t lds_cols(const rl_gridop* g) {
    return ((size_t)g->N1 * g->colsA + g->N1) * sizeof(cplx);
}
static size_t lds_rows(int N2, int cols) {
    return ((size_t)N2 * (cols | 1) + N2) * sizeof(cplx);
}

static int ensure_workspace(rl_gridop* g, size_t pairs) {
    if (pairs <= g->T_pairs) return RL_OK;
    if (g->T) RL_HIP(hipFree(g->T));
// ... 2392 lines not shown
```

### runlmc_amd/csrc/rl_host.h

```cpp
#pragma once
#include "../../include/runlmc_hip.h"

#include <algorithm>
#include <cmath>
#include <cstdio>
#include <cstdlib>
#include <cstring>
#include <functional>
#include <string>
#include <thread>
#include <vector>

#include "rl_kernels.h"
#include "rl_kernels2.h"
#include "rl_kernels3.h"
#include "rl_lowrank.h"
#include "rl_rowpoly.h"
#include "rl_filter.h"

#define RL_MAX_D 16

int fail(int code, const std::string& msg);
#define RL_HIP(expr)                                                                   \
    do {                                                                               \
        hipError_t e_ = (expr);                                                        \
        if (e_ != hipSuccess)                                                          \
            return fail(RL_EHIP, std::string(#expr) + ": " + hipGetErrorString(e_));   \
    } while (0)

#define RL_TRY(expr)              \
    do {                          \
        int rc_ = (expr);         \
        if (rc_ != RL_OK) return rc_; \
    } while (0)


void trace_once(const char* what);
bool first_on_device(unsigned long long* seen);

struct RlKnobs {
    bool pow2_only = false;
    int chunk_mb = 0;
    int two_streams = -1;
    int affine = -1;
    int affine_kb = 0;
    int affine_max_kb = 2048;
    bool no_v1p = false;
    int v1p_min = 0;
    bool no_lowrank = false;
    bool no_filter = false;
    bool sf_scan2 = false;
    bool sf_carries1 = false;
    bool no_lr_bound = false;
    bool poly_round = false;
    bool no_poly_round = false;
    long long lr_min = -1;
    bool staged_wt = false;
    bool no_staged_wt = false;
    bool no_w_poly = false;
    bool no_rp = false;
    int rp_stagger = 7;
    int rp_runlen = 0;
    bool no_rp_small = false;
    bool rp_pfuse = true;
    bool w_pfuse = true;
    bool no_rp_fuse = false;
    bool no_lr_small = false;
    int lr_expand_plain = 0;
    int lr_policy = -1;
    bool no_precond_approx = false;
    long long precond_hi_min = 100000;
    int precond_hi_use = 0;
    int precond_hi_rank = 192;
    bool no_precond_hi_mixed = false;
    bool precond_hi_passes = false;
    bool no_precond_hi = false;
    int rp_fly = 1;
    int w_poly_rmax = 32;
    bool no_sort = false;
    long long ws_cache_mb = -1;
    int solver_maxblk = 0;
    bool no_fuse_w = false;
    bool no_fuse_wt = false;
    bool no_graph = false;
    bool minres_v1 = false;
};
RlKnobs read_knobs();

template <class T>
static int upload(T** dev, const std::vector<T>& host) {
    RL_HIP(hipMalloc((void**)dev, std::max<size_t>(host.size(), 1) * sizeof(T)));
    if (!host.empty())
        RL_HIP(hipMemcpy(*dev, host.data(), host.size() * sizeof(T), hipMemcpyHostToDevice));
    return RL_OK;
}

static const size_t kLdsSoft = 76 * 1024;
static const size_t kLdsHard = 156 * 1024;

struct rl_gridop {
    RlKnobs kn;
    int device = 0;
    int D = 0, m = 0, L = 0, N1 = 0, N2 = 0;
    Geom geo{0, 0, 0};
    int colsA = 0;
    int rowsB = 0;
    int rowsS = 0;
    int code1 = 0, code2 = 0;
    bool v2 = false;
    bool rows3 = false;
    bool lr_try = false;
    bool lr_ok = false;
    bool lr_round_try = false;
    bool wide = false;
    rl_gridop* child = nullptr;
    double* wide_B = nullptr;
    double* wide_Z = nullptr;
    size_t wide_Z_cap = 0;
    bool lead = false;
    int m0 = 0, N0 = 0;
    std::vector<rl_gridop*> kids;
    double* lead_tw = nullptr;
    double *lead_x = nullptr, *lead_y = nullptr;
    size_t lead_cap = 0;
    bool defer_expand = false;
    bool expand_deferred = false;
    int lr_rejects = 0;
    int lr_skip = 0;
    double* lr_stat = nullptr;
    bool lr_dirty = false;
    std::vector<double> lr_A, lr_W, lr_kap;
    std::vector<int> lr_Qi;
    bool lr_bypass = false;
    int lr_r = 0;
    int lr_rank_hint = 0;
    size_t lr_min = 0;
    double* lr_beta = nullptr;
    double* lr_nu = nullptr;
    double* lr_phiJ = nullptr;
    double* lr_C = nullptr;
    double* lr_M = nullptr;
    std::vector<double> lr_hC;
    double* lr_spart = nullptr;
    size_t lr_spart_cap = 0;
    double* lr_Cx = nullptr;
    double* lr_Mf = nullptr;
    size_t lr_Mf_cap = 0;
    bool lr_Mf_ok = false;
    std::vector<double> lr_hB;
    std::vector<double> lr_hnu;
    unsigned long long param_ver = 0;
    double* lr_B = nullptr;
    double* lr_eye = nullptr;
    double* lr_part = nullptr;
    size_t lr_part_cap = 0;
    double* lr_zhat = nullptr;
    size_t lr_zhat_cap = 0;
    double* lr_scr = nullptr;
    double* lr_pw = nullptr;
    double* lr_sel = nullptr;
    std::vector<double> lr_vstat;
    double* lr_Cc = nullptr;
    double* lr_Bc = nullptr;
    int lr_np = 0;
    std::vector<double> h_tops;
    std::vector<int> top_form;
    bool st_ok = false;
    bool sf_try = false;
    int sf_n = 0;
    int sf_nfac = 0;
    int sf_ns = 2;
    std::vector<int> sf_slot;
    std::vector<int> sf_top_ns;
    SfTop* sf_tops = nullptr;
    double* sf_pwp = nullptr;
    double* sf_blob = nullptr;
    double* sf_blob_top = nullptr;
    double* sf_pw = nullptr;
    double* sf_kappa = nullptr;
    double* sf_facA = nullptr;
    double* sf_facAW = nullptr;
    int* sf_facJ = nullptr;
    double* sf_E = nullptr;
    size_t sf_E_cap = 0;
    double* sf_Cin = nullptr;
    int* sf_next = nullptr;
    size_t sf_Cin_cap = 0;
    double* mixtab = nullptr;
    size_t mixtab_rows = 0;
    bool mixtab_ok = false;
    int max_tops = 0;
    FftPlan plan1, plan2;
    cplx *tw1 = nullptr, *tw2 = nullptr, *twlo = nullptr, *twhi = nullptr;
    int* freq1 = nullptr;
    TwiddleL twl;
    std::vector<int> h_freq1, h_freq2;
    int Q = 0, nfac = 0;
    double* tops = nullptr;
    double* spec = nullptr;
    double* facA = nullptr;
    double* facW = nullptr;
    int* facQ = nullptr;
    double* kappa = nullptr;
    double* ones = nullptr;
    int max_fac = 0;
    cplx* T = nullptr;
    size_t T_pairs = 0;
    cplx* T2[3] = {nullptr, nullptr, nullptr};
    size_t T2_pairs = 0;
    int nside = 0;
    cplx* Tcur = nullptr;
    hipStream_t aux[3] = {nullptr, nullptr, nullptr};
    hipEvent_t ev_fork = nullptr, ev_join[3] = {nullptr, nullptr, nullptr};
    size_t chunk_pairs = 1;
    bool affine = false;
    bool v1p = false;
    FftPlan planL;
    cplx* twL = nullptr;
    double* spec1 = nullptr;
    size_t lds1 = 0;
    int thr1 = 256;
    int v1p_min = 64;
};

struct SkiTerm {
    rl_gridop* g = nullptr;
    int ngrid = 0;
    int *W_indptr = nullptr, *W_indices = nullptr;
    double* W_data = nullptr;
    int *WT_indptr = nullptr, *WT_indices = nullptr;
    double* WT_data = nullptr;
    int nnzWT = 0;
    int* W4_base = nullptr;
    double* W4_w = nullptr;
    int* WT_lo = nullptr;
    int wt_xmax = 0, wt_emax = 0;
    int w_xmax = 0;
    std::vector<int> h_base;
};

struct SolverWork {
    double* vec[10] = {nullptr, nullptr, nullptr, nullptr, nullptr,
                       nullptr, nullptr, nullptr, nullptr, nullptr};
    double* S[2] = {nullptr, nullptr};
    int* I = nullptr;
    double* part[4] = {nullptr, nullptr, nullptr, nullptr};
    int* count = nullptr;
    double* resid = nullptr;
    double* lanczos = nullptr;
};

struct rl_ski {
    RlKnobs kn;
    double* lanczos_buf = nullptr;
    size_t lanczos_bytes = 0;
    int device = 0;
    std::vector<SkiTerm> extra;
    int max_ngrid = 0;
    rl_gridop* g = nullptr;
    int n = 0, ngrid = 0, nnz = 0, nnzWT = 0;
    int *W4_base = nullptr, *WT_lo = nullptr;
    int wt_xmax = 0, wt_emax = 0, w_xmax = 0;
    double* W4_w = nullptr;
    int *W_indptr = nullptr, *W_indices = nullptr;
    double* W_data = nullptr;
    int *WT_indptr = nullptr, *WT_indices = nullptr;
    double* WT_data = nullptr;
    double* noise_diag = nullptr;
    bool has_noise = false;
    double *G1 = nullptr, *G2 = nullptr;
    int cap = 0;
    std::vector<int> h_base;
    int *poly_tab = nullptr, *poly_ob = nullptr;
    int poly_nblk = 0;
    double* poly_part = nullptr;
    size_t poly_part_cap = 0;
    double* rp_F = nullptr;
    int rp_R = 0;
    double* rp_Fc = nullptr;
    int rp_Fc_R = 0;
    int* rp_base_c = nullptr;
    double* rp_w4_c = nullptr;
    int *rp_runs = nullptr, *rp_run_ptr = nullptr, *rp_out_end = nullptr;
    int rp_nruns = 0;
    double* rp_part = nullptr;
    size_t rp_part_cap = 0;
    double* rp_nrm = nullptr;
    size_t rp_nrm_cap = 0;
    RpFuse rp_fuse{nullptr, nullptr, nullptr};
    RpPFuse rp_pfuse{nullptr, nullptr, nullptr, nullptr, nullptr, nullptr, nullptr};
    std::function<void(hipStream_t)> rp_mid;
    double* rp_pp = nullptr;
    size_t rp_pp_cap = 0;
    std::vector<int> eps_end;
    std::vector<double> eps_val;
    bool permuted = false;
    int* perm = nullptr;
    std::vector<int> h_perm;
    int caller_ranges_same = -1;
    bool caller_noise_same = true;
    double *P1 = nullptr, *P2 = nullptr;
    int pcap = 0;
    hipStream_t solver_stream = nullptr;
    int* pin_count = nullptr;
    hipEvent_t count_ev[2] = {nullptr, nullptr};
    SolverWork ws;
    bool ws_valid = false;
    size_t ws_vec_cap = 0, ws_rhs_cap = 0, ws_part_cap = 0;
    unsigned long long noise_ver = 0;
    std::vector<double> h_noise;
    std::vector<int> h_run_ptr, h_out_end;
    std::vector<double> dz_U;
    int dz_U_R = 0;
    double* dz_Zt = nullptr;
    size_t dz_Zt_cap = 0;
    double* dz_inv = nullptr;
    std::vector<double> dz_eps;
    const char* dz_eps_why = nullptr;
    unsigned long long dz_eps_ver = ~0ull;
    bool dz_valid = false;
    bool dz_exact = false;
    const char* dz_fail_why = nullptr;
    unsigned long long dz_fail_param_ver = 0, dz_fail_noise_ver = 0;
    int dz_fail_streak = 0, dz_fail_skip = 0;
    double *dz_p = nullptr, *dz_q = nullptr;
    size_t dz_pq_cap = 0;
    double* dz_scal = nullptr;
    size_t dz_scal_cap = 0;
    unsigned long long dz_param_ver = 0, dz_noise_ver = 0;
    int dz_R = 0;
    bool dz_want_sample = false;
    double* dz_Zh = nullptr;
    size_t dz_Zh_cap = 0;
    bool dz_Zh_valid = false;
    double* dz_isq = nullptr;
    unsigned long long dz_isq_ver = ~0ull;
    double* dz_smp = nullptr;
    size_t dz_smp_cap = 0;
    double* dz_rec = nullptr;
    size_t dz_rec_cap = 0;
    bool dz_hz = false;
    int hz_R = 0;
    bool hz_traced = false;
    int hz_Ruse = 0;
    bool hz_basis_tried = false;
    const char* hz_why = nullptr;
    std::vector<double> hz_hnu;
    double* hz_beta = nullptr;
    double* hz_phi = nullptr;
    double* hz_tphi = nullptr;
    double* hz_C = nullptr;
    double* hz_F = nullptr;
    double* hz_ones = nullptr;
    std::vector<double> hz_U;
    double* hz_part = nullptr;
    double* hz_zhat = nullptr;
    double* hz_tmp = nullptr;
    double* hz_S = nullptr;
    double* hz_P = nullptr;
    size_t hz_vec_cap = 0;
    double dz_logdet = 0.0;
    double dz_cond = 0.0;
    double *dz_res = nullptr, *dz_cor = nullptr;
    size_t dz_vec_cap = 0;
    double* dz_part = nullptr;
    int* dz_go = nullptr;
    size_t dz_rhs_cap = 0;
};

template <class H, int (*Destroy)(H*)>
struct HandleGuard {
    H* h;
    explicit HandleGuard(H* h_) : h(h_) {}
    ~HandleGuard() { if (h) (void)Destroy(h); }
    H* release() { H* r = h; h = nullptr; return r; }
};

bool stream_capturing(hipStream_t stream);
int lr_ensure(rl_gridop* g);
int lr_prepare(rl_gridop* g, int nvec);
int lr_reserve(rl_gridop* g, int nvec);
int gridop_prepare(rl_gridop* g, int nvec);
int lr_all_coeffs(rl_gridop* g, int R, std::vector<double>* hC, std::vector<char>* exact,
                  std::vector<double>* captured);
int mvm_chunk_v2(rl_gridop* g, const MixParams& mp, const double* Xc, double* Yc, int nv, size_t pairs,
                 hipStream_t st, const Gather* gather = nullptr, int* bump = nullptr,
                 cplx* Tbuf = nullptr);
int mvm_chunk_v1(rl_gridop* g, const MixParams& mp, const double* Xc, double* Yc, int nv, size_t pairs,
                 hipStream_t stream, const Gather* gather = nullptr, int* bump = nullptr);
int upload_raw(void** dev, const void* host, size_t bytes);
int ski_reserve(rl_ski* s, int nvec);
int ski_wt_int(rl_ski* s, const double* Xp, double* G, int nvec, hipStream_t st, int* bump = nullptr);
int ski_reserve_perm(rl_ski* s, int nvec);
void permute_rows(rl_ski* s, const double* X, double* Y, int nvec, int scatter, hipStream_t st);
bool w_staged_p_ok(const rl_ski* s, int nvec);
bool rp_ok(const rl_ski* s, int nvec);
int rp_prepare(rl_ski* s, int nvec);
bool rp_ready(const rl_ski* s, int nvec);
int ski_mvm_int(rl_ski* s, const double* Xp, double* Yp, int nvec, hipStream_t st,
                int* bump = nullptr, bool noise = true);
void free_work(SolverWork& w);
```

### runlmc_amd/csrc/rl_ski.hip

```cpp
#include "rl_host.h"


static void launch_spmv(const int* indptr, const int* indices, const double* vals, int nrows,
                        int ncols, int nvec, const double* X, double* Y, const double* diag,
                        const double* X2, hipStream_t st, int accumulate = 0,
                        int* bump = nullptr, int avg_nnz = 0) {
    const unsigned gx = (nrows + RL_THREADS - 1) / RL_THREADS;
    const bool blocked = (size_t)nrows * nvec >= ((size_t)1 << 22);
    if (!blocked && avg_nnz > 12 && diag == nullptr && !accumulate) {
        const unsigned gw = (unsigned)(((size_t)nrows * 8 + RL_THREADS - 1) / RL_THREADS);
        RL_LAUNCH(k_spmv_wide<8>, dim3(gw, nvec), dim3(RL_THREADS), RL_THREADS * sizeof(double), st,
                  indptr, indices, vals, nrows, ncols, X, Y, bump);
        return;
    }
    if (blocked) {
        RL_LAUNCH(k_spmv<8>, dim3(gx, (nvec + 7) / 8), dim3(RL_THREADS), 0, st, indptr, indices,
                  vals, nrows, ncols, nvec, X, Y, diag, X2, accumulate, bump);
    } else {
        RL_LAUNCH(k_spmv<1>, dim3(gx, nvec), dim3(RL_THREADS), 0, st, indptr, indices, vals,
                  nrows, ncols, nvec, X, Y, diag, X2, accumulate, bump);
    }
}

static int check_csr(const int* indptr, const int* indices, int nrows, int ncols,
// ... 60 lines not shown
        base.resize(n);
        w4.assign((size_t)4 * n, 0.0);
        int prev = 0;
        for (int i = 0; i < n && ok; ++i) {
            const int k0 = W_indptr[i], cnt = W_indptr[i + 1] - k0;
            if (cnt > 4) { ok = false; break; }
            for (int j = 1; j < cnt; ++j)
                if (W_indices[k0 + j] != W_indices[k0] + j) ok = false;
            int b = cnt ? W_indices[k0] : prev, shift = 0;
            if (b > ngrid - 4) { shift = b - (ngrid - 4); b = ngrid - 4; }
            if (shift + cnt > 4 || b < prev) { ok = false; break; }
            prev = b;
            base[i] = b;
            for (int j = 0; j < cnt; ++j) w4[(size_t)4 * i + shift + j] = W_data[k0 + j];
        }
        if (ok) {
            lo.resize(ngrid);
            sp_ptr.assign(ngrid + 1, 0);
            int a = 0, e = 0;
            for (int r = 0; r < ngrid; ++r) {
                while (a < n && base[a] < r - 3) ++a;
                while (e < n && base[e] <= r) ++e;
                lo[r] = a;
                sp_ptr[r + 1] = sp_ptr[r] + (e - a);
                for (int i = a; i < e; ++i) {
                    sp_idx.push_back(i);
                    sp_val.push_back(w4[(size_t)4 * i + (r - base[i])]);
                }
            }
            t->h_base = base;
            RL_TRY(upload_raw((void**)&t->W4_base, base.data(), (size_t)n * sizeof(int)));
            RL_TRY(upload_raw((void**)&t->W4_w, w4.data(), (size_t)4 * n * sizeof(double)));
            RL_TRY(upload_raw((void**)&t->WT_lo, lo.data(), (size_t)ngrid * sizeof(int)));
            WT_indptr = sp_ptr.data(); WT_indices = sp_idx.data(); WT_data = sp_val.data();
            for (int r0 = 0; r0 < n; r0 += RL_THREADS)
                t->w_xmax = std::max(t->w_xmax,
                                     base[std::min(n, r0 + RL_THREADS) - 1] + 4 - base[r0]);
            for (int r0 = 0; r0 < ngrid; r0 += RL_THREADS) {
                const int rl = std::min(ngrid, r0 + RL_THREADS) - 1;
                const int c1 = lo[rl] + (sp_ptr[rl + 1] - sp_ptr[rl]);
                t->wt_xmax = std::max(t->wt_xmax, c1 - lo[r0]);
                t->wt_emax = std::max(t->wt_emax, sp_ptr[rl + 1] - sp_ptr[r0]);
            }
        }
    }
    const size_t nnzT = WT_indptr[ngrid];
    t->nnzWT = (int)nnzT;
    RL_TRY(upload_raw((void**)&t->W_indptr, W_indptr, (size_t)(n + 1) * sizeof(int)));
    RL_TRY(upload_raw((void**)&t->W_indices, W_indices, nnz * sizeof(int)));
    RL_TRY(upload_raw((void**)&t->W_data, W_data, nnz * sizeof(double)));
    RL_TRY(upload_raw((void**)&t->WT_indptr, WT_indptr, (size_t)(ngrid + 1) * sizeof(int)));
    RL_TRY(upload_raw((void**)&t->WT_indices, WT_indices, nnzT * sizeof(int)));
    RL_TRY(upload_raw((void**)&t->WT_data, WT_data, nnzT * sizeof(double)));
    return RL_OK;
}

extern "C" int rl_ski_create(rl_gridop* g, int n, const int* W_indptr, const int* W_indices,
                             const double* W_data, const int* WT_indptr, const int* WT_indices,
                             const double* WT_data, rl_ski** out) {
    if (!out) return fail(RL_EINVAL, "out is NULL");
    *out = nullptr;
    if (!g) return fail(RL_EINVAL, "gridop is NULL");
    if (n < 1) return fail(RL_EINVAL, "rl_ski_create: n < 1");
    const int ngrid = g->D * g->m;
    RL_TRY(check_csr(W_indptr, W_indices, n, ngrid, "W"));
    RL_TRY(check_csr(WT_indptr, WT_indices, ngrid, n, "WT"));
    if (W_indptr[n] != WT_indptr[ngrid])
        return fail(RL_EINVAL, "rl_ski_create: W and WT have different nnz");
    RL_HIP(hipSetDevice(g->device));
    rl_ski* s = new rl_ski;
    HandleGuard<rl_ski, rl_ski_destroy> guard(s);
    s->kn = read_knobs();
    s->g = g;
    s->device = g->device;
    s->n = n;
    s->ngrid = ngrid;
    std::vector<int> perm(n);
    for (int i = 0; i < n; ++i) perm[i] = i;
    auto key = [&](int i) {
        return W_indptr[i + 1] > W_indptr[i] ? W_indices[W_indptr[i]] : 0x7fffffff;
    };
    std::stable_sort(perm.begin(), perm.end(), [&](int a, int b) { return key(a) < key(b); });
    bool identity = true;
    for (int i = 0; i < n && identity; ++i) identity = perm[i] == i;
    if (s->kn.no_sort) identity = true;
    if (!identity) {
        s->permuted = true;
        s->h_perm = perm;
        RL_TRY(upload_raw((void**)&s->perm, perm.data(), (size_t)n * sizeof(int)));
    }
    SkiTerm t0;
    RL_TRY(upload_term(&t0, n, ngrid, W_indptr, W_indices, W_data, WT_indptr, WT_indices,
                       WT_data, s->permuted ? &s->h_perm : nullptr));
    s->W_indptr = t0.W_indptr; s->W_indices = t0.W_indices; s->W_data = t0.W_data;
    s->WT_indptr = t0.WT_indptr; s->WT_indices = t0.WT_indices; s->WT_data = t0.WT_data;
    s->W4_base = t0.W4_base; s->W4_w = t0.W4_w; s->WT_lo = t0.WT_lo; s->nnzWT = t0.nnzWT;
    s->h_base.swap(t0.h_base);
    s->wt_xmax = t0.wt_xmax; s->wt_emax = t0.wt_emax; s->w_xmax = t0.w_xmax;
    s->max_ngrid = ngrid;
    s->nnz = W_indptr[n];
    RL_HIP(hipMalloc((void**)&s->noise_diag, (size_t)n * sizeof(double)));
    RL_HIP(hipMemset(s->noise_diag, 0, (size_t)n * sizeof(double)));
    *out = guard.release();
    return RL_OK;
}

extern "C" int rl_ski_add_term(rl_ski* s, rl_gridop* g, const int* W_indptr,
                               const int* W_indices, const double* W_data,
                               const int* WT_indptr, const int* WT_indices,
                               const double* WT_data) {
    if (!s || !g) return fail(RL_EINVAL, "rl_ski_add_term: NULL handle");
    if (g->D != s->g->D || g->device != s->g->device)
        return fail(RL_EINVAL, "rl_ski_add_term: grid operator has another D or device");
    const int ngrid = g->D * g->m;
    RL_TRY(check_csr(W_indptr, W_indices, s->n, ngrid, "W"));
    RL_TRY(check_csr(WT_indptr, WT_indices, ngrid, s->n, "WT"));
    if (W_indptr[s->n] != WT_indptr[ngrid])
        return fail(RL_EINVAL, "rl_ski_add_term: W and WT have different nnz");
    RL_HIP(hipSetDevice(g->device));
    SkiTerm t;
    t.g = g;
    int rc = upload_term(&t, s->n, ngrid, W_indptr, W_indices, W_data, WT_indptr, WT_indices,
                         WT_data, s->permuted ? &s->h_perm : nullptr);
    s->extra.push_back(t);
    if (rc != RL_OK) return rc;
    if (ngrid > s->max_ngrid) {
        s->max_ngrid = ngrid;
        s->cap = 0;
    }
    return RL_OK;
}


extern "C" int rl_ski_destroy(rl_ski* s) {
    if (!s) return RL_OK;
    (void)hipSetDevice(s->device);
    for (SkiTerm& t : s->extra) {
        void* tp[] = {t.W_indptr, t.W_indices, t.W_data, t.WT_indptr, t.WT_indices, t.WT_data,
                      t.W4_base, t.W4_w, t.WT_lo};
        for (void* p : tp)
            if (p) (void)hipFree(p);
    }
    if (s->solver_stream) (void)hipStreamDestroy(s->solver_stream);
    if (s->pin_count) (void)hipHostFree(s->pin_count);
    for (hipEvent_t e : s->count_ev)
        if (e) (void)hipEventDestroy(e);
    if (s->ws_valid) free_work(s->ws);
    void* ptrs[] = {s->W_indptr, s->W_indices, s->W_data, s->WT_indptr, s->WT_indices,
                    s->WT_data, s->noise_diag, s->G1, s->G2, s->perm, s->P1, s->P2,
                    s->W4_base, s->W4_w, s->WT_lo, s->lanczos_buf, s->poly_tab, s->poly_ob,
                    s->poly_part, s->rp_F, s->rp_Fc, s->rp_runs, s->rp_run_ptr, s->rp_out_end, s->rp_part, s->rp_nrm, s->rp_pp,
                    s->rp_base_c, s->rp_w4_c, s->dz_Zt, s->dz_inv, s->dz_res, s->dz_cor, s->dz_part,
                    s->dz_go, s->dz_p, s->dz_q, s->dz_scal, s->hz_beta, s->hz_phi, s->hz_tphi, s->hz_C,
                    s->hz_F, s->hz_ones, s->hz_part, s->hz_zhat, s->hz_tmp, s->hz_S, s->hz_P, s->dz_Zh, s->dz_isq, s->dz_smp, s->dz_rec};
    for (void* p : ptrs)
        if (p) (void)hipFree(p);
    delete s;
    return RL_OK;
}

extern "C" int rl_ski_set_noise(rl_ski* s, const double* noise, const int* lens) {
    if (!s || !noise || !lens) return fail(RL_EINVAL, "rl_ski_set_noise: NULL argument");
    std::vector<double> diag;
    diag.reserve(s->n);
    for (int d = 0; d < s->g->D; ++d) {
        if (lens[d] < 0) return fail(RL_EINVAL, "rl_ski_set_noise: negative length");
        diag.insert(diag.end(), (size_t)lens[d], noise[d]);
    }
    if ((int)diag.size() != s->n)
        return fail(RL_EINVAL, "rl_ski_set_noise: sum(lens) != n");
    s->caller_noise_same = true;
    if (s->permuted) {
        std::vector<double> sorted(diag.size());
        for (int i = 0; i < s->n; ++i) sorted[i] = diag[s->h_perm[i]];
        for (int i = 0; i < s->n && s->caller_noise_same; ++i)
            s->caller_noise_same = sorted[i] == diag[i];
        diag.swap(sorted);
    }
    s->eps_end.clear();
    s->eps_val.clear();
    for (int i = 0; i < s->n; ++i) {
        if (i == 0 || diag[i] != diag[i - 1]) {
            if ((int)s->eps_val.size() == RL_MAX_D) {
                s->eps_end.clear();
                s->eps_val.clear();
                break;
            }
            if (i > 0) s->eps_end.push_back(i);
            s->eps_val.push_back(diag[i]);
        }
    }
    if (!s->eps_val.empty()) s->eps_end.push_back(s->n);
    RL_HIP(hipSetDevice(s->g->device));
    RL_HIP(hipMemcpy(s->noise_diag, diag.data(), diag.size() * sizeof(double),
                     hipMemcpyHostToDevice));
    s->has_noise = true;
    s->h_noise.swap(diag);
    ++s->noise_ver;
    return RL_OK;
}

int ski_reserve(rl_ski* s, int nvec) {
    if (nvec <= s->cap && s->G1) return RL_OK;
    if (s->G1) RL_HIP(hipFree(s->G1));
    if (s->G2) RL_HIP(hipFree(s->G2));
    s->G1 = s->G2 = nullptr;
    s->cap = 0;
    RL_HIP(hipMalloc((void**)&s->G1, (size_t)nvec * s->max_ngrid * sizeof(double)));
    RL_HIP(hipMalloc((void**)&s->G2, (size_t)nvec * s->max_ngrid * sizeof(double)));
    s->cap = nvec;
    return RL_OK;
}

int ski_reserve_perm(rl_ski* s, int nvec) {
    if (!s->permuted || nvec <= s->pcap) return RL_OK;
    if (s->P1) RL_HIP(hipFree(s->P1));
    if (s->P2) RL_HIP(hipFree(s->P2));
    s->P1 = s->P2 = nullptr;
    s->pcap = 0;
    RL_HIP(hipMalloc((void**)&s->P1, (size_t)nvec * s->n * sizeof(double)));
    RL_HIP(hipMalloc((void**)&s->P2, (size_t)nvec * s->n * sizeof(double)));
    s->pcap = nvec;
    return RL_OK;
}

void permute_rows(rl_ski* s, const double* X, double* Y, int nvec, int scatter,
                         hipStream_t st) {
    dim3 grid((((s->n + RL_THREADS - 1) / RL_THREADS) + 7) / 8 * 8, nvec);
    RL_LAUNCH(k_permute_rows, grid, dim3(RL_THREADS), 0, st, X, Y, (const int*)s->perm, s->n,
              scatter);
}

static int staged_vgroups() { return 4; }

int ski_wt_int(rl_ski* s, const double* Xp, double* G, int nvec, hipStream_t st, int* bump) {
    constexpr int VB = 8;
    const size_t lds = ((size_t)VB * s->wt_xmax + s->wt_emax) * sizeof(double);
    if (s->WT_lo != nullptr && s->wt_xmax > 0 && lds <= 64 * 1024 &&
        s->wt_xmax <= 4 * RL_THREADS &&
        ((size_t)s->ngrid * nvec >= ((size_t)1 << 22) || s->kn.staged_wt) && !s->kn.no_staged_wt) {
        trace_once("W^T product: k_spmv_wt_staged");
        static unsigned long long seen = 0;
        if (first_on_device(&seen)) {
            (void)hipFuncSetAttribute((const void*)k_spmv_wt_staged<VB, 1>,
                                      hipFuncAttributeMaxDynamicSharedMemorySize, 64 * 1024);
            (void)hipFuncSetAttribute((const void*)k_spmv_wt_staged<VB, 2>,
                                      hipFuncAttributeMaxDynamicSharedMemorySize, 64 * 1024);
            (void)hipFuncSetAttribute((const void*)k_spmv_wt_staged<VB, 4>,
                                      hipFuncAttributeMaxDynamicSharedMemorySize, 64 * 1024);
        }
        const unsigned gx = (s->ngrid + RL_THREADS - 1) / RL_THREADS;
        const int vg = staged_vgroups();
        const dim3 grid(gx, ((nvec + VB - 1) / VB + vg - 1) / vg);
#define RL_WT_STAGED(XPT)                                                                       \
    RL_LAUNCH((k_spmv_wt_staged<VB, XPT>), grid, dim3(RL_THREADS), lds, st,                     \
              (const int*)s->WT_indptr, (const int*)s->WT_lo, (const double*)s->WT_data,        \
              s->ngrid, s->n, nvec, Xp, G, s->wt_xmax, vg, bump)
        if (s->wt_xmax <= RL_THREADS) RL_WT_STAGED(1);
        else if (s->wt_xmax <= 2 * RL_THREADS) RL_WT_STAGED(2);
        else RL_WT_STAGED(4);
#undef RL_WT_STAGED
        RL_HIP(hipGetLastError());
        return RL_OK;
    }
    launch_spmv(s->WT_indptr, s->WT_indices, s->WT_data, s->ngrid, s->n, nvec, Xp, G, nullptr,
                nullptr, st, 0, bump, s->ngrid > 0 ? s->nnzWT / s->ngrid : 0);
    RL_HIP(hipGetLastError());
    return RL_OK;
}
static bool w_staged_ok(const rl_ski* s, int nvec) {
    constexpr int VB = 8;
    const size_t lds = (size_t)VB * s->w_xmax * sizeof(double);
    return s->W4_base != nullptr && s->w_xmax > 0 && lds <= 64 * 1024 &&
           s->w_xmax <= 4 * RL_THREADS &&
           ((size_t)s->n * nvec >= ((size_t)1 << 22) || s->kn.staged_wt) && !s->kn.no_staged_wt;
}
static size_t w_staged_p_lds(const rl_ski* s) {
    constexpr int VB = 8;
    size_t lds = ((size_t)VB * s->w_xmax + (size_t)staged_vgroups() * VB * 8) * sizeof(double);
#if defined(RL_EMU)
    lds += 256 * sizeof(double);
#endif
    return lds;
}
bool w_staged_p_ok(const rl_ski* s, int nvec) {
    return w_staged_ok(s, nvec) && w_staged_p_lds(s) <= 64 * 1024 && s->n < (1 << 28);
}
static int ski_w_int(rl_ski* s, const double* G, double* Yp, int nvec, const double* diag,
                     const double* X2p, hipStream_t st) {
    constexpr int VB = 8;
    const size_t lds = (size_t)VB * s->w_xmax * sizeof(double);
    const RpPFuse pf = s->rp_pfuse;
    if (pf.pc != nullptr) {
        if (!w_staged_p_ok(s, nvec))
            return fail(RL_EINVAL, "internal: MINRES update fused into a W product that does not run staged");
        trace_once("W product: k_spmv_w_staged_p (MINRES's P inside)");
        static unsigned long long seenp = 0;
        if (first_on_device(&seenp)) {
            (void)hipFuncSetAttribute((const void*)k_spmv_w_staged_p<VB, 1>,
                                      hipFuncAttributeMaxDynamicSharedMemorySize, 64 * 1024);
            (void)hipFuncSetAttribute((const void*)k_spmv_w_staged_p<VB, 2>,
                                      hipFuncAttributeMaxDynamicSharedMemorySize, 64 * 1024);
            (void)hipFuncSetAttribute((const void*)k_spmv_w_staged_p<VB, 4>,
                                      hipFuncAttributeMaxDynamicSharedMemorySize, 64 * 1024);
        }
        const unsigned gx = (s->n + RL_THREADS - 1) / RL_THREADS;
        const int vg = staged_vgroups();
// ... 410 lines not shown
```

### runlmc_amd/csrc/rl_solve.hip

```cpp
#include "rl_host.h"
#include "rl_solver.h"
#include "rl_direct.h"
#include "rl_loo.h"

void free_work(SolverWork& w) {
    for (double*& p : w.vec) { if (p) (void)hipFree(p); p = nullptr; }
    for (double*& p : w.S) { if (p) (void)hipFree(p); p = nullptr; }
    for (double*& p : w.part) { if (p) (void)hipFree(p); p = nullptr; }
    if (w.I) (void)hipFree(w.I);
    if (w.count) (void)hipFree(w.count);
    if (w.resid) (void)hipFree(w.resid);
    w.I = nullptr; w.count = nullptr; w.resid = nullptr; w.lanczos = nullptr;
}

static size_t ws_cache_limit(const rl_ski* s) {
    const size_t mb = s->kn.ws_cache_mb >= 0 ? (size_t)s->kn.ws_cache_mb : 16384;
    return mb << 20;
}

struct SolverWorkGuard {
    rl_ski* s;
    SolverWork* w;
    hipGraph_t graph = nullptr;
    hipGraphExec_t exec = nullptr;
    SolverWorkGuard(rl_ski* s_, SolverWork* w_) : s(s_), w(w_) {}
    ~SolverWorkGuard() {
        if (exec) (void)hipGraphExecDestroy(exec);
        if (graph) (void)hipGraphDestroy(graph);
        w->lanczos = nullptr;
        size_t nv = 0;
        for (double* p : w->vec) nv += p != nullptr;
        const size_t bytes = nv * s->ws_vec_cap * sizeof(double);
        if (w->I != nullptr && !s->ws_valid && bytes <= ws_cache_limit(s)) {
            s->ws = *w;
            s->ws_valid = true;
        } else {
            free_work(*w);
        }
    }
};

static int solver_alloc(rl_ski* s, SolverWork& w, unsigned need, int nrhs, int n, int nblk,
                        hipStream_t st) {
    const size_t ve = (size_t)nrhs * n, pe = (size_t)nrhs * nblk;
    if (s->ws_valid) {
        if (s->ws_vec_cap >= ve && s->ws_rhs_cap >= (size_t)nrhs && s->ws_part_cap >= pe)
            w = s->ws;
        else
            free_work(s->ws);
        s->ws = SolverWork();
        s->ws_valid = false;
    }
    if (w.I == nullptr) {
        s->ws_vec_cap = ve;
        s->ws_rhs_cap = (size_t)nrhs;
        s->ws_part_cap = pe;
        for (int i = 0; i < 2; ++i)
            RL_HIP(hipMalloc((void**)&w.S[i], (size_t)nrhs * S_NFIELDS * sizeof(double)));
        RL_HIP(hipMalloc((void**)&w.I, (size_t)nrhs * I_NFIELDS * sizeof(int)));
        for (int i = 0; i < 4; ++i)
            RL_HIP(hipMalloc((void**)&w.part[i], pe * sizeof(double)));
        RL_HIP(hipMalloc((void**)&w.count, 4 * sizeof(int)));
        RL_HIP(hipMalloc((void**)&w.resid, (size_t)nrhs * sizeof(double)));
    }
    for (int i = 0; i < 10; ++i)
        if (((need >> i) & 1u) && w.vec[i] == nullptr)
            RL_HIP(hipMalloc((void**)&w.vec[i], s->ws_vec_cap * sizeof(double)));
    RL_HIP(hipMemsetAsync(w.count, 0, 4 * sizeof(int), st));
    RL_HIP(hipMemsetAsync(w.resid, 0, (size_t)nrhs * sizeof(double), st));
    return RL_OK;
}

static int active_count(SolverWork& w, int nrhs, hipStream_t st, int* out) {
    RL_LAUNCH(k_count_active, dim3(1), dim3(64), 0, st, w.I, nrhs, w.count);
    RL_HIP(hipMemcpyAsync(out, w.count, sizeof(int), hipMemcpyDeviceToHost, st));
    RL_HIP(hipStreamSynchronize(st));
    return RL_OK;
}

static int residual_check(rl_ski* s, SolverWork& w, const double* B, const double* X,
                          double* scratch, int nrhs, int n, int nblk, double tol, int freeze,
                          hipStream_t st) {
    RL_TRY(ski_mvm_int(s, X, scratch, nrhs, st));
    dim3 grid(nblk, nrhs), blk(RL_SOLVER_THREADS);
    const size_t red = RL_SOLVER_THREADS * sizeof(double);
    RL_LAUNCH(k_resid_partial, grid, blk, red, st, B, (const double*)scratch, n, w.part[2]);
    RL_LAUNCH(k_resid_finish, dim3((nrhs + 63) / 64), dim3(64), 0, st,
              (const double*)w.part[2], nblk, nrhs, w.resid, w.I, tol, freeze);
    return RL_OK;
}

static int minres_iteration(rl_ski* s, const MinresBufs& mb, SolverWork& w, int nrhs, int n,
                            int nblk, double rtol, int maxiter, hipStream_t st) {
    dim3 grid(nblk, nrhs), blk(RL_SOLVER_THREADS);
    const size_t red = RL_SOLVER_THREADS * sizeof(double);
    RL_TRY(ski_mvm_int(s, mb.v, mb.q, nrhs, st));
    RL_LAUNCH(k_minres_a, grid, blk, red, st, mb, n, w.part[0]);
    RL_LAUNCH(k_minres_b, grid, blk, red, st, mb, n, (const double*)w.part[0], w.part[1]);
    RL_LAUNCH(k_minres_c, grid, blk, red, st, mb, n, (const double*)w.part[0],
              (const double*)w.part[1], w.part[2]);
    RL_LAUNCH(k_minres_test, dim3(1), blk, 0, st, mb, (const double*)w.part[2], nblk, nrhs,
              rtol, maxiter);
    return RL_OK;
}

static bool g_is_v2(const rl_gridop* g) { return g->v2; }

static int poly_round_prepare(rl_ski* s, int nrhs, int max_blk, bool* ok) {
    *ok = false;
    rl_gridop* g = s->g;
    if (!s->extra.empty() || s->W4_base == nullptr || s->h_base.empty() ||
        !g->lr_round_try || s->poly_nblk < 0 || s->kn.no_poly_round || g->kn.no_poly_round)
        return RL_OK;
    if (s->poly_nblk == 0) {
        const int D = g->D, m = g->m, n = s->n;
        std::vector<int> tab, ob(D + 1, 0);
        int i = 0;
        for (int d = 0; d < D; ++d) {
            ob[d] = (int)tab.size() / RL_PT;
            const int start = i;
            while (i < n && s->h_base[i] < (d + 1) * m) ++i;
            const int cnt = i - start;
            const int nb = (cnt + 1023) / 1024;
            for (int b = 0; b < nb; ++b) {
                const int per = (cnt + nb - 1) / nb;
                const int r0 = start + b * per, r1 = std::min(start + (b + 1) * per, i);
                tab.push_back(r0);
                tab.push_back(r1);
                tab.push_back(d);
                const int gfirst = s->h_base[r0] - d * m;
                tab.push_back(gfirst);
                tab.push_back(s->h_base[r1 - 1] - d * m + 4 - gfirst);
            }
        }
        ob[D] = (int)tab.size() / RL_PT;
        if (i != n || tab.empty()) {
            s->poly_nblk = -1;
            return RL_OK;
        }
        RL_TRY(upload_raw((void**)&s->poly_tab, tab.data(), tab.size() * sizeof(int)));
        RL_TRY(upload_raw((void**)&s->poly_ob, ob.data(), ob.size() * sizeof(int)));
        s->poly_nblk = (int)tab.size() / RL_PT;
    }
    if (s->poly_nblk > std::max(max_blk, RL_SOLVER_THREADS)) return RL_OK;
    RL_TRY(lr_ensure(g));
    if (!g->lr_ok || g->lr_r != RL_LR_RS) return RL_OK;
    const size_t need = (size_t)nrhs * s->poly_nblk * RL_LR_RS;
    if (s->poly_part_cap < need) {
        if (s->poly_part) RL_HIP(hipFree(s->poly_part));
        s->poly_part = nullptr;
        s->poly_part_cap = 0;
        RL_HIP(hipMalloc((void**)&s->poly_part, need * sizeof(double)));
        s->poly_part_cap = need;
    }
    *ok = true;
    return RL_OK;
// ... 640 lines not shown
            }
        if (!dz_chol(L[d], R)) { *why = "an output has too few (or degenerate) rows for the basis"; return false; }
        for (int i = 0; i < R; ++i)
            for (int j = i + 1; j < R; ++j) L[d][(size_t)i * R + j] = 0.0;
        dz_tri_inverse(L[d], R, Li[d]);
    }
    std::vector<double> S((size_t)Dr * Dr, 0.0);
    std::vector<std::pair<int, int>> blocks;
    for (int a = 0; a < D; ++a)
        for (int b = 0; b <= a; ++b) blocks.emplace_back(a, b);
    dz_parallel((int)blocks.size(), 1, [&](int first, int step) {
      std::vector<double> Mab((size_t)R * R), T1((size_t)R * R), A((size_t)R * R);
      for (size_t pb = first; pb < blocks.size(); pb += step) {
            const int a = blocks[pb].first, b = blocks[pb].second;
            std::fill(Mab.begin(), Mab.end(), 0.0);
            bool any = false;
            for (int q = 0; q < Q; ++q) {
                const double bq = 0.5 * (hB[((size_t)q * D + a) * D + b] + hB[((size_t)q * D + b) * D + a]);
                if (bq == 0.0) continue;
                any = true;
                const double* C = hC + (size_t)q * R * R;
                for (int i = 0; i < R; ++i)
                    for (int j = 0; j < R; ++j)
                        Mab[(size_t)i * R + j] += bq * 0.5 * (C[(size_t)i * R + j] + C[(size_t)j * R + i]);
            }
            if (!any) continue;
            std::fill(T1.begin(), T1.end(), 0.0);
            for (int i = 0; i < R; ++i) {
                double* t = T1.data() + (size_t)i * R;
                for (int k = 0; k < R; ++k) {
                    const double mk = Mab[(size_t)i * R + k];
                    const double* l = L[b].data() + (size_t)k * R;
                    for (int j = 0; j <= k; ++j) t[j] += mk * l[j];
                }
            }
            std::fill(A.begin(), A.end(), 0.0);
            for (int k = 0; k < R; ++k) {
                const double* t = T1.data() + (size_t)k * R;
                for (int i = 0; i <= k; ++i) {
                    const double lk = L[a][(size_t)k * R + i];
                    double* o = A.data() + (size_t)i * R;
                    for (int j = 0; j < R; ++j) o[j] += lk * t[j];
                }
            }
            for (int i = 0; i < R; ++i)
                for (int j = 0; j < R; ++j) {
                    const double acc = A[(size_t)i * R + j];
                    S[((size_t)a * R + i) * Dr + (size_t)b * R + j] = acc;
                    S[((size_t)b * R + j) * Dr + (size_t)a * R + i] = acc;
                }
      }
    });
    for (int i = 0; i < Dr; ++i)
        for (int j = 0; j < i; ++j) {
            const double v = 0.5 * (S[(size_t)i * Dr + j] + S[(size_t)j * Dr + i]);
            S[(size_t)i * Dr + j] = v;
            S[(size_t)j * Dr + i] = v;
        }
    for (int i = 0; i < Dr; ++i) S[(size_t)i * Dr + i] += 1.0;
    if (!dz_chol(S, Dr)) { *why = "I + L^T M L is not positive definite (M is not positive semi-definite to roundoff)"; return false; }
    double logdet = 0.0, pmin = 1e300, pmax = 0.0;
    for (int i = 0; i < Dr; ++i) {
        const double p = S[(size_t)i * Dr + i];
        logdet += 2.0 * std::log(p);
        pmin = std::min(pmin, p);
        pmax = std::max(pmax, p);
    }
    for (int d = 0; d < D; ++d) logdet += rows[d] * std::log(eps[d]);
    std::vector<double> Xt;
    dz_tri_inverse_t(S, Dr, Xt);
    std::vector<double> Y((size_t)Dr * Dr, 0.0);
    dz_parallel(Dr, 32, [&](int first, int step) {
        for (int i = first; i < Dr; i += step) {
            const double* xi = Xt.data() + (size_t)i * Dr;
            for (int j = 0; j <= i; ++j) {
                const double* xj = Xt.data() + (size_t)j * Dr;
                const double v = (i == j ? 1.0 : 0.0) - dz_dot(xi + i, xj + i, Dr - i);
                Y[(size_t)i * Dr + j] = v;
            }
        }
    });
    for (int i = 0; i < Dr; ++i)
        for (int j = 0; j < i; ++j) Y[(size_t)j * Dr + i] = Y[(size_t)i * Dr + j];
    Zs.assign((size_t)Dr * Dr, 0.0);
    dz_parallel((int)blocks.size(), 1, [&](int first, int step) {
      std::vector<double> T1((size_t)R * R), A((size_t)R * R);
      for (size_t pb = first; pb < blocks.size(); pb += step) {
            const int a = blocks[pb].first, b = blocks[pb].second;
            std::fill(T1.begin(), T1.end(), 0.0);
            for (int i = 0; i < R; ++i) {
                double* t = T1.data() + (size_t)i * R;
                const double* y = Y.data() + ((size_t)a * R + i) * Dr + (size_t)b * R;
                for (int k = 0; k < R; ++k) {
                    const double yk = y[k];
                    const double* l = Li[b].data() + (size_t)k * R;
                    for (int j = 0; j <= k; ++j) t[j] += yk * l[j];
                }
            }
            std::fill(A.begin(), A.end(), 0.0);
            for (int k = 0; k < R; ++k) {
                const double* t = T1.data() + (size_t)k * R;
                for (int i = 0; i <= k; ++i) {
                    const double lk = Li[a][(size_t)k * R + i];
                    double* o = A.data() + (size_t)i * R;
                    for (int j = 0; j < R; ++j) o[j] += lk * t[j];
                }
            }
            for (int i = 0; i < R; ++i)
                for (int j = 0; j < R; ++j) {
                    const double v = -(nu[i] / eps[a]) * A[(size_t)i * R + j] * (nu[j] / eps[b]);
                    Zs[((size_t)a * R + i) * Dr + (size_t)b * R + j] = v;
                    Zs[((size_t)b * R + j) * Dr + (size_t)a * R + i] = v;
                }
      }
    });
    if (Zh_t != nullptr) {
        Zh_t->assign((size_t)Dr * Dr, 0.0);
        dz_parallel((int)blocks.size(), 1, [&](int first, int step) {
          std::vector<double> T1((size_t)R * R), A((size_t)R * R);
          for (size_t pb = first; pb < blocks.size(); pb += step) {
                const int a = blocks[pb].first, b = blocks[pb].second;
                std::fill(T1.begin(), T1.end(), 0.0);
                for (int i = 0; i < R; ++i) {
                    double* t = T1.data() + (size_t)i * R;
                    const double* c = S.data() + ((size_t)a * R + i) * Dr + (size_t)b * R;
                    const int kmax = a == b ? i : R - 1;
                    for (int k = 0; k <= kmax; ++k) {
                        const double ck = c[k] - (a == b && k == i ? 1.0 : 0.0);
                        const double* l = Li[b].data() + (size_t)k * R;
                        for (int j = 0; j <= k; ++j) t[j] += ck * l[j];
                    }
                }
                std::fill(A.begin(), A.end(), 0.0);
                for (int k = 0; k < R; ++k) {
                    const double* t = T1.data() + (size_t)k * R;
                    for (int i = 0; i <= k; ++i) {
                        const double lk = Li[a][(size_t)k * R + i];
                        double* o = A.data() + (size_t)i * R;
                        for (int j = 0; j < R; ++j) o[j] += lk * t[j];
                    }
                }
                for (int i = 0; i < R; ++i)
                    for (int j = 0; j < R; ++j)
                        (*Zh_t)[((size_t)b * R + j) * Dr + (size_t)a * R + i] = nu[i] * A[(size_t)i * R + j] * nu[j];
          }
        });
    }
    *logdet_out = logdet;
    *pmin_out = pmin;
    *pmax_out = pmax;
    return true;
}

static_assert(RL_HZ_BLK == RL_RP_RMAX, "the blocks run the rank-48 kernels");
#define RL_HZ_RDEF 192
static int hz_rank(const rl_ski* s) {
    const int D = s->g->D;
    const int lim = RL_HZ_FS * RL_HZ_FMAX / D / RL_HZ_BLK * RL_HZ_BLK;
    for (int R = std::min(s->kn.precond_hi_rank / RL_HZ_BLK * RL_HZ_BLK, lim); R >= 2 * RL_HZ_BLK; R -= RL_HZ_BLK) {
        const double f = (double)D * R / 960.0;
        if (s->g->m >= 8 * R && (double)s->n >= 1e5 * f * f * f) return R;
    }
    return 0;
}
template <class T>
static int hz_grow(T** p, size_t count) {
    if (*p) RL_HIP(hipFree(*p));
    *p = nullptr;
    RL_HIP(hipMalloc((void**)p, count * sizeof(T)));
    return RL_OK;
}

static int dz_upload_sample_map(rl_ski* s, const std::vector<double>& Zh) {
    s->dz_Zh_valid = false;
    if (Zh.empty()) return RL_OK;
    if (s->dz_Zh_cap < Zh.size()) {
        s->dz_Zh_cap = 0;
        RL_TRY(hz_grow(&s->dz_Zh, Zh.size()));
        s->dz_Zh_cap = Zh.size();
    }
    RL_HIP(hipMemcpy(s->dz_Zh, Zh.data(), Zh.size() * sizeof(double), hipMemcpyHostToDevice));
    s->dz_Zh_valid = true;
    return RL_OK;
}

static int hz_reserve(rl_ski* s, int nvec) {
    const size_t cap = (size_t)std::max(nvec, RL_HZ_BLK);
    if (s->hz_vec_cap >= cap && s->hz_part != nullptr) return RL_OK;
    s->hz_vec_cap = 0;
    const size_t nb = (size_t)s->hz_R / RL_HZ_BLK;
    RL_TRY(hz_grow(&s->hz_part, nb * s->rp_nruns * cap * RL_HZ_BLK));
    RL_TRY(hz_grow(&s->hz_zhat, nb * (cap + 16) * s->g->D * RL_HZ_BLK));
    RL_TRY(hz_grow(&s->hz_tmp, cap * s->n));
    RL_TRY(hz_grow(&s->hz_S, cap * s->g->D * s->hz_R));
    RL_TRY(hz_grow(&s->hz_P, (size_t)RL_HZ_FS * cap * s->g->D * s->hz_R));
    s->hz_vec_cap = cap;
    return RL_OK;
}

static int hz_basis(rl_ski* s) {
    rl_gridop* g = s->g;
    if (s->hz_basis_tried) return RL_OK;
    s->hz_basis_tried = true;
    s->hz_why = "basis not built";
    const int m = g->m, n = s->n, D = g->D, R = hz_rank(s), NB = R / RL_HZ_BLK;
    if (R == 0) { s->hz_why = "no room for a larger basis at this many outputs"; return RL_OK; }
    s->hz_R = R;
    const int rows = (R + D - 1) / D * D;
    std::vector<double> phi((size_t)rows * m, 0.0), beta(R), nu(R);
    {
        std::vector<long double> prev(m, 0.0L), cur(m), nxt(m);
        const long double p0 = 1.0L / sqrtl((long double)m);
        for (int i = 0; i < m; ++i) cur[i] = p0;
        long double bj = 0.0L, nuj = p0;
        for (int j = 0; j < R; ++j) {
            for (int i = 0; i < m; ++i) phi[(size_t)j * m + i] = (double)cur[i];
            beta[j] = (double)(bj * bj);
            nu[j] = (double)nuj;
            long double nrm = 0.0L;
            for (int i = 0; i < m; ++i) {
                const long double si = -1.0L + 2.0L * i / (m - 1);
                nxt[i] = si * cur[i] - bj * prev[i];
                nrm += nxt[i] * nxt[i];
            }
            bj = sqrtl(nrm);
            if (!(bj > 0.0L)) { s->hz_why = "the larger basis is degenerate on this grid"; return RL_OK; }
            nuj /= bj;
            for (int i = 0; i < m; ++i) {
                prev[i] = cur[i];
                cur[i] = nxt[i] / bj;
            }
        }
    }
    {
        const int probe[] = {0, 1, R / 4, R / 2 - 1, R / 2, R - 3, R - 2};
        const double* last = phi.data() + (size_t)(R - 1) * m;
        double worst = std::fabs(dz_dot(last, last, m) - 1.0);
        for (int j : probe) worst = std::max(worst, std::fabs(dz_dot(last, phi.data() + (size_t)j * m, m)));
        if (!(worst < 1e-9)) { s->hz_why = "the larger basis is not orthonormal on this grid (too few points)"; return RL_OK; }
    }
    {
        size_t free_b = 0, total_b = 0;
        RL_HIP(hipMemGetInfo(&free_b, &total_b));
        const double need = 2.0 * (double)R * n * sizeof(double) + 2.0 * (double)rows * m * sizeof(double) + 1e9;
        if ((double)free_b < need) { s->hz_why = "not enough free device memory for the larger basis' table"; return RL_OK; }
    }
    RL_TRY(upload(&s->hz_phi, phi));
    RL_TRY(upload(&s->hz_beta, beta));
    s->hz_hnu = nu;
    RL_TRY(hz_grow(&s->hz_tphi, (size_t)rows * m));
    RL_TRY(hz_grow(&s->hz_C, (size_t)R * R));
    RL_TRY(hz_grow(&s->hz_F, (size_t)R * n));
    {
        std::vector<double> ones((size_t)n, 1.0);
        RL_TRY(upload(&s->hz_ones, ones));
    }
    hipStream_t st = nullptr;
    RL_LAUNCH(k_rp_build, dim3((n + 255) / 256), dim3(256), 0, st, (const int*)s->W4_base,
              (const double*)s->W4_w, n, m, R, (const double*)s->hz_beta, s->hz_F);
    RL_HIP(hipGetLastError());
    RL_TRY(hz_reserve(s, RL_HZ_BLK));
    s->hz_U.assign((size_t)D * R * R, 0.0);
    std::vector<double> part((size_t)s->rp_nruns * RL_HZ_BLK * RL_HZ_BLK);
    for (int cb = 0; cb < NB; ++cb)
        for (int rb = 0; rb < NB; ++rb) {
            rp_project_plain<RL_HZ_BLK>(s, s->hz_F + (size_t)cb * RL_HZ_BLK * n, RL_HZ_BLK, st,
                                        s->hz_F + (size_t)rb * RL_HZ_BLK * n, s->hz_part);
            RL_HIP(hipGetLastError());
            RL_HIP(hipMemcpy(part.data(), s->hz_part, part.size() * sizeof(double), hipMemcpyDeviceToHost));
            for (int d = 0; d < D; ++d)
                for (int c = s->h_run_ptr[d]; c < s->h_run_ptr[d + 1]; ++c)
                    for (int v = 0; v < RL_HZ_BLK; ++v)
                        for (int j = 0; j < RL_HZ_BLK; ++j)
                            s->hz_U[((size_t)d * R + rb * RL_HZ_BLK + j) * R + cb * RL_HZ_BLK + v] +=
                                part[((size_t)c * RL_HZ_BLK + v) * RL_HZ_BLK + j];
        }
    s->hz_why = nullptr;
    return RL_OK;
}

static bool hz_wanted(const rl_ski* s) {
    const rl_gridop* g = s->g;
    if (s->kn.no_precond_hi || g->lr_ok || (g->lr_np > 0 && s->kn.no_precond_hi_mixed)) return false;
    return hz_rank(s) > 0 && (double)s->n >= (double)s->kn.precond_hi_min;
}

static int hz_try(rl_ski* s, const std::vector<double>& eps, const std::vector<int>& rows, bool* ok,
                  const char** why) {
    rl_gridop* g = s->g;
    *ok = false;
    RL_TRY(hz_basis(s));
    if (s->hz_why != nullptr) { *why = s->hz_why; return RL_OK; }
    const int D = g->D, m = g->m, Q = g->Q, RT = s->hz_R;
    int R = RT;
    const int nv = (RT + D - 1) / D;
    hipStream_t st = nullptr;
    std::vector<double> hCT((size_t)Q * RT * RT), one((size_t)RT * RT);
    std::vector<double> capb((size_t)Q * (RT / RL_HZ_BLK), 0.0);
    const unsigned nb = ((RT + RL_XD_A - 1) / RL_XD_A) * ((RT + RL_XD_B - 1) / RL_XD_B);
    for (int q = 0; q < Q; ++q) {
        RL_TRY(rl_gridop_mvm_top(g, q, s->hz_phi, s->hz_tphi, nv, st));
        RL_LAUNCH(k_cross_dots_tiled, dim3(nb, 1), dim3(RL_SOLVER_THREADS), RL_SOLVER_THREADS * sizeof(double),
                  st, (const double*)s->hz_phi, (const double*)s->hz_tphi, RT, m, s->hz_C);
        RL_HIP(hipGetLastError());
        RL_HIP(hipMemcpy(one.data(), s->hz_C, one.size() * sizeof(double), hipMemcpyDeviceToHost));
        const double t0 = g->h_tops.size() > (size_t)q * m ? g->h_tops[(size_t)q * m] : 0.0;
        double tr = 0.0;
        double* dst = hCT.data() + (size_t)q * RT * RT;
        for (int i = 0; i < RT; ++i) {
            tr += one[(size_t)i * RT + i];
            if ((i + 1) % RL_HZ_BLK == 0) capb[(size_t)q * (RT / RL_HZ_BLK) + i / RL_HZ_BLK] = t0 > 0.0 ? tr / (t0 * m) : 0.0;
            for (int j = 0; j < RT; ++j) {
                dst[(size_t)i * RT + j] = 0.5 * (one[(size_t)i * RT + j] + one[(size_t)j * RT + i]);
                if (!std::isfinite(dst[(size_t)i * RT + j])) { *why = "a top row's projection is not finite"; return RL_OK; }
            }
        }
        if (!(t0 > 0.0 && tr / (t0 * m) >= 0.8)) {
            *why = "the larger subspace holds less than 0.8 of a row's spectrum either";
            return RL_OK;
        }
    }
    if (getenv("RUNLMC_TRACE") != nullptr && !s->hz_traced) {
        s->hz_traced = true;
        for (int q = 0; q < Q; ++q) {
            fprintf(stderr, "[runlmc] larger basis: row %d (form %d) holds", q, (int)g->top_form.size() > q ? g->top_form[q] : -1);
            for (int k = 0; k < RT / RL_HZ_BLK; ++k) fprintf(stderr, " %.6f", capb[(size_t)q * (RT / RL_HZ_BLK) + k]);
            fprintf(stderr, " of its trace in the first 48, 96 ... functions\n");
        }
    }
    if ((double)D * RT > 960.0)
        for (int k = 2; k < RT / RL_HZ_BLK; ++k) {
            double worst = 1.0;
            for (int q = 0; q < Q; ++q) worst = std::min(worst, capb[(size_t)q * (RT / RL_HZ_BLK) + k - 1]);
            if (worst >= 1.0 - 1e-5) { R = k * RL_HZ_BLK; break; }
        }
    if (s->kn.precond_hi_use > 0) R = std::max(2 * RL_HZ_BLK, std::min(RT, s->kn.precond_hi_use / RL_HZ_BLK * RL_HZ_BLK));
    std::vector<double> hC((size_t)Q * R * R);
    for (int q = 0; q < Q; ++q)
        for (int i = 0; i < R; ++i)
            std::memcpy(hC.data() + ((size_t)q * R + i) * R, hCT.data() + ((size_t)q * RT + i) * RT, (size_t)R * sizeof(double));
    std::vector<double> Zs;
    double logdet = 0.0, pmin = 1.0, pmax = 1.0;
    std::vector<double> Usub;
    const double* U = s->hz_U.data();
    if (R != RT) {
        Usub.resize((size_t)D * R * R);
        for (int d = 0; d < D; ++d)
            for (int i = 0; i < R; ++i)
                std::memcpy(Usub.data() + ((size_t)d * R + i) * R, s->hz_U.data() + ((size_t)d * RT + i) * RT,
                            (size_t)R * sizeof(double));
        U = Usub.data();
    }
    std::vector<double> Zh;
    if (!dz_host_map(D, R, Q, U, s->hz_hnu.data(), eps, rows, g->lr_hB.data(), hC.data(), Zs,
                     &logdet, &pmin, &pmax, why, s->dz_want_sample ? &Zh : nullptr))
        return RL_OK;
    RL_TRY(dz_upload_sample_map(s, Zh));
    for (double v : Zs)
        if (!std::isfinite(v)) { *why = "the solve map is not finite"; return RL_OK; }
    if (s->dz_Zt_cap < Zs.size()) {
        s->dz_Zt_cap = 0;
        RL_TRY(hz_grow(&s->dz_Zt, Zs.size()));
        s->dz_Zt_cap = Zs.size();
    }
    RL_HIP(hipMemcpy(s->dz_Zt, Zs.data(), Zs.size() * sizeof(double), hipMemcpyHostToDevice));
    s->dz_logdet = logdet;
    s->dz_cond = (pmax / pmin) * (pmax / pmin);
    s->hz_Ruse = R;
    *ok = true;
    return RL_OK;
}

static int hz_apply(rl_ski* s, const double* in, double* out, int nvec, hipStream_t st,
                    const double* map = nullptr, const double* diag = nullptr) {
    if (map == nullptr) map = s->dz_Zt;
    if (diag == nullptr) diag = s->dz_inv;
    rl_gridop* g = s->g;
    const int D = g->D, n = s->n, Dr = D * s->hz_Ruse, NB = s->hz_Ruse / RL_HZ_BLK;
    RL_TRY(hz_reserve(s, nvec));
    for (int k = 0; k < NB; ++k)
        rp_project_plain<RL_HZ_BLK>(s, in, nvec, st, s->hz_F + (size_t)k * RL_HZ_BLK * n,
                                    s->hz_part + (size_t)k * s->rp_nruns * nvec * RL_HZ_BLK);
    const dim3 egrid((Dr + 255) / 256, nvec);
    RL_LAUNCH(k_hz_sums, egrid, dim3(256), 0, st, (const double*)s->hz_part, (const int*)s->rp_run_ptr,
              s->rp_nruns, nvec, D, NB, s->hz_S);
    const int per = (Dr + RL_HZ_FS - 1) / RL_HZ_FS;
    RL_LAUNCH(k_hz_map, dim3((Dr + 255) / 256, (nvec + RL_HZ_VB - 1) / RL_HZ_VB, RL_HZ_FS), dim3(256),
              (size_t)per * RL_HZ_VB * sizeof(double), st, (const double*)s->hz_S, map,
              nvec, Dr, s->hz_P);
    if (!s->kn.precond_hi_passes && NB >= 3) {
        const int nvp = (nvec + 15) / 16 * 16, nvt = nvp / 16;
        RL_LAUNCH(k_hz_collect, dim3((Dr + 255) / 256, nvp), dim3(256), 0, st, (const double*)s->hz_P, nvec, D, NB,
                  RL_HZ_FS, s->hz_zhat, nvp);
        const dim3 xgrid((n + 127) / 128, (nvt + 8) / 9), xgrid2((n + 127) / 128, (nvt + 1) / 2);
        if (nvt <= 2)
            RL_LAUNCH((k_hz_expand_mm<2>), xgrid2, dim3(256), 0, st, (const double*)s->hz_zhat, (const double*)s->hz_F,
                      n, nvec, nvp, D, s->hz_Ruse, (const int*)s->rp_out_end, out, diag, in);
        else
            RL_LAUNCH((k_hz_expand_mm<9>), xgrid, dim3(256), 0, st, (const double*)s->hz_zhat, (const double*)s->hz_F,
                      n, nvec, nvp, D, s->hz_Ruse, (const int*)s->rp_out_end, out, diag, in);
        RL_HIP(hipGetLastError());
        return RL_OK;
    }
    RL_LAUNCH(k_hz_collect, egrid, dim3(256), 0, st, (const double*)s->hz_P, nvec, D, NB, RL_HZ_FS, s->hz_zhat, 0);
    const double* src = in;
    for (int k = 0; k < NB; ++k) {
        double* dst = (NB - 1 - k) % 2 == 0 ? out : s->hz_tmp;
        rp_expand_plain<RL_HZ_BLK>(s, s->hz_zhat + (size_t)k * nvec * D * RL_HZ_BLK, dst, nvec,
                                   k == 0 ? diag : (const double*)s->hz_ones, src, st, s->hz_F + (size_t)k * RL_HZ_BLK * n);
        src = dst;
    }
    RL_HIP(hipGetLastError());
    return RL_OK;
}

static int dz_available(rl_ski* s, bool* ok, const char** why) {
    rl_gridop* g = s->g;
    *ok = false;
    *why = "";
    if (g->lead) { *why = "3-D grid: no polynomial form and no factorisation on a three-dimensional grid"; return RL_OK; }
    if (!s->extra.empty()) { *why = "kernels on several grids"; return RL_OK; }
    if (g->wide) {
        *why = g->D > RL_MAX_D ? "more than 16 outputs"
                               : "2-D grid whose rows of D outputs exceed the LDS row tile";
        return RL_OK;
    }
    if (s->W4_base == nullptr || s->h_base.empty() || s->ngrid != g->D * g->m) {
        *why = "W is not a cubic interpolant of a 1-D grid"; return RL_OK;
    }
    if (!g->lr_try || g->kn.no_rp || (s->kn.rp_fly & 2)) { *why = "polynomial form switched off or grid not eligible"; return RL_OK; }
    if (s->n >= (1 << 28)) { *why = "n >= 2^28"; return RL_OK; }
    if (g->Q < 1) { *why = "no parameters set"; return RL_OK; }
    if (!s->has_noise || (int)s->h_noise.size() != s->n) { *why = "no noise set"; return RL_OK; }
    RL_HIP(hipSetDevice(g->device));
    RL_TRY(lr_ensure(g));
    if ((int)g->lr_hB.size() < g->Q * g->D * g->D) { *why = "no host copy of the couplings"; return RL_OK; }
    *ok = true;
    return RL_OK;
}

static int dz_ensure(rl_ski* s, bool* ok, const char** why) {
    rl_gridop* g = s->g;
    RL_TRY(dz_available(s, ok, why));
    if (!*ok) { s->dz_valid = false; return RL_OK; }
    const bool exact = g->lr_ok;
    const int R = exact || g->lr_np > 0 ? g->lr_r : RL_LR_RMAX;
    const int D = g->D, n = s->n, Dr = D * R, Q = g->Q;
    if (s->dz_valid && s->dz_param_ver == g->param_ver && s->dz_noise_ver == s->noise_ver &&
        (s->dz_R == R || s->dz_hz))
        return RL_OK;
    if (s->dz_fail_why != nullptr && s->dz_fail_param_ver == g->param_ver && s->dz_fail_noise_ver == s->noise_ver) {
        *ok = false;
        *why = s->dz_fail_why;
        return RL_OK;
    }
    if (!exact && s->dz_fail_streak > 0 && s->dz_fail_why != nullptr) {
        if (s->dz_fail_skip > 0) {
            --s->dz_fail_skip;
            *ok = false;
            *why = s->dz_fail_why;
            s->dz_fail_param_ver = g->param_ver;
            s->dz_fail_noise_ver = s->noise_ver;
            return RL_OK;
        }
    }
    struct FailNote {
        rl_ski* s; bool* ok; const char** why;
        ~FailNote() {
            if (!*ok) {
                s->dz_fail_why = *why;
                s->dz_fail_param_ver = s->g->param_ver;
                s->dz_fail_noise_ver = s->noise_ver;
                s->dz_fail_streak = std::min(s->dz_fail_streak + 1, 5);
                s->dz_fail_skip = (1 << s->dz_fail_streak) - 1;
            } else {
                s->dz_fail_why = nullptr;
                s->dz_fail_streak = 0;
                s->dz_fail_skip = 0;
            }
        }
    } note{s, ok, why};
    s->dz_hz = false;
    if (Dr > 576 && (double)n < 1e5 * ((double)Dr / 576.0) * ((double)Dr / 576.0) * ((double)Dr / 576.0)) {
        s->dz_valid = false;
        *ok = false;
        *why = "D * rank is large for this few rows: the factorisation would cost more than the Krylov solve";
        return RL_OK;
    }
    s->dz_valid = false;
    *ok = false;
    hipStream_t st = nullptr;
    std::vector<double> hCx;
    const double* hC = g->lr_hC.data();
    const char* cap_why = nullptr;
    if (!exact) {
        if (s->kn.no_precond_approx) { *why = "not every top row is in the polynomial form"; return RL_OK; }
        std::vector<char> ex;
        std::vector<double> cap;
        RL_TRY(lr_all_coeffs(g, R, &hCx, &ex, &cap));
        for (int q = 0; q < Q; ++q)
            if (!(cap[q] >= 0.8))
                cap_why = "not every top row is in the polynomial form, and the subspace holds less than 0.8 of a row's spectrum (no preconditioner either)";
        if (cap_why != nullptr && !hz_wanted(s)) { *why = cap_why; return RL_OK; }
        hC = hCx.data();
    } else if ((int)g->lr_hC.size() < Q * R * R) {
        *why = "no host copy of the coefficient maps";
        return RL_OK;
    }
    RL_TRY(rp_prepare(s, std::max(R, 1)));
    if (s->rp_F == nullptr || s->rp_R != R) { *why = "no table of F"; return RL_OK; }
    if (s->dz_eps_ver != s->noise_ver || (int)s->dz_eps.size() != D) {
        s->dz_eps.assign(D, 0.0);
        s->dz_eps_why = nullptr;
        for (int d = 0, a = 0; d < D && !s->dz_eps_why; ++d) {
            const int b = s->h_out_end[d];
            if (b > a) {
                s->dz_eps[d] = s->h_noise[a];
                for (int i = a; i < b; ++i)
                    if (s->h_noise[i] != s->dz_eps[d]) { s->dz_eps_why = "noise is not constant per output"; break; }
            } else {
                s->dz_eps[d] = 1.0;
            }
            if (!s->dz_eps_why && (!(s->dz_eps[d] > 0.0) || !std::isfinite(s->dz_eps[d])))
                s->dz_eps_why = "noise is not positive";
            a = b;
        }
        if (!s->dz_eps_why) {
            std::vector<double> inv((size_t)n);
            for (int i = 0; i < n; ++i) inv[i] = 1.0 / s->h_noise[i];
            if (!s->dz_inv) RL_HIP(hipMalloc((void**)&s->dz_inv, (size_t)n * sizeof(double)));
            RL_HIP(hipMemcpy(s->dz_inv, inv.data(), inv.size() * sizeof(double), hipMemcpyHostToDevice));
        }
        s->dz_eps_ver = s->noise_ver;
    }
    if (s->dz_eps_why) { *why = s->dz_eps_why; return RL_OK; }
    const std::vector<double>& eps = s->dz_eps;
    std::vector<int> rows(D, 0);
    for (int d = 0, a = 0; d < D; ++d) {
        rows[d] = s->h_out_end[d] - a;
        a = s->h_out_end[d];
    }
    if (!exact && hz_wanted(s)) {
        bool hz_ok = false;
        const char* hz_why = "";
        RL_TRY(hz_try(s, eps, rows, &hz_ok, &hz_why));
        if (hz_ok) {
            s->dz_param_ver = g->param_ver;
            s->dz_noise_ver = s->noise_ver;
            s->dz_R = s->hz_Ruse;
            s->dz_exact = false;
            s->dz_hz = true;
            s->dz_valid = true;
            *ok = true;
            return RL_OK;
        }
        if (cap_why != nullptr) { *why = cap_why; return RL_OK; }
    }
    if (s->dz_U_R != R) {
#define RL_DZ_PROJ(R_) rp_project_plain<R_>(s, s->rp_F, R_, st)
        RL_DZ_RANKS(RL_DZ_PROJ);
#undef RL_DZ_PROJ
        RL_HIP(hipGetLastError());
        std::vector<double> part((size_t)s->rp_nruns * R * R);
        RL_HIP(hipMemcpy(part.data(), s->rp_part, part.size() * sizeof(double), hipMemcpyDeviceToHost));
        s->dz_U.assign((size_t)D * R * R, 0.0);
        for (int d = 0; d < D; ++d)
            for (int c = s->h_run_ptr[d]; c < s->h_run_ptr[d + 1]; ++c)
                for (int e = 0; e < R * R; ++e)
                    s->dz_U[(size_t)d * R * R + e] += part[(size_t)c * R * R + e];
        s->dz_U_R = R;
    }
    if ((int)g->lr_hnu.size() < R) { *why = "no host copy of the basis normalisation"; return RL_OK; }
    std::vector<double> Zs;
    double logdet = 0.0, pmin = 1.0, pmax = 1.0;
    std::vector<double> Zh;
    if (!dz_host_map(D, R, Q, s->dz_U.data(), g->lr_hnu.data(), eps, rows, g->lr_hB.data(), hC, Zs, &logdet,
                     &pmin, &pmax, why, s->dz_want_sample ? &Zh : nullptr))
        return RL_OK;
    RL_TRY(dz_upload_sample_map(s, Zh));
    for (double v : Zs)
        if (!std::isfinite(v)) { *why = "the solve map is not finite"; return RL_OK; }
    if (s->dz_Zt_cap < Zs.size()) {
        if (s->dz_Zt) RL_HIP(hipFree(s->dz_Zt));
        s->dz_Zt = nullptr;
        s->dz_Zt_cap = 0;
        RL_HIP(hipMalloc((void**)&s->dz_Zt, Zs.size() * sizeof(double)));
        s->dz_Zt_cap = Zs.size();
    }
    RL_HIP(hipMemcpy(s->dz_Zt, Zs.data(), Zs.size() * sizeof(double), hipMemcpyHostToDevice));
    s->dz_logdet = logdet;
    s->dz_cond = (pmax / pmin) * (pmax / pmin);
    s->dz_param_ver = g->param_ver;
    s->dz_noise_ver = s->noise_ver;
    s->dz_R = R;
    s->dz_exact = exact;
    s->dz_valid = true;
    *ok = true;
    return RL_OK;
}

static int dz_apply(rl_ski* s, const double* in, double* out, int nvec, hipStream_t st,
                    const double* map = nullptr, const double* diag = nullptr) {
    rl_gridop* g = s->g;
    if (s->dz_hz) return hz_apply(s, in, out, nvec, st, map, diag);
    if (map == nullptr) map = s->dz_Zt;
    if (diag == nullptr) diag = s->dz_inv;
    const int R = g->lr_r, D = g->D;
#define RL_DZ_PROJ(R_) rp_project_plain<R_>(s, in, nvec, st)
    RL_DZ_RANKS(RL_DZ_PROJ);
#undef RL_DZ_PROJ
    RL_LAUNCH(k_dz_mix, dim3((nvec + RL_DZ_VB - 1) / RL_DZ_VB), dim3(256),
              (size_t)RL_DZ_VB * D * R * sizeof(double), st, (const double*)s->rp_part,
              (const int*)s->rp_run_ptr, nvec, D, R, map, g->lr_zhat);
#define RL_DZ_EXP(R_) rp_expand_plain<R_>(s, g->lr_zhat, out, nvec, diag, in, st)
    RL_DZ_RANKS(RL_DZ_EXP);
#undef RL_DZ_EXP
    RL_HIP(hipGetLastError());
    return RL_OK;
}

extern "C" int rl_ski_factor(rl_ski* s, int* available, double* logdet, double* cond) {
    if (!s) return fail(RL_EINVAL, "rl_ski_factor: NULL handle");
    bool ok = false;
    const char* why = "";
    RL_TRY(dz_ensure(s, &ok, &why));
    if (available) *available = ok ? (s->dz_exact ? 1 : s->dz_hz ? 3 : 2) : 0;
    if (logdet) *logdet = ok && s->dz_exact ? s->dz_logdet : 0.0;
    if (cond) *cond = ok ? s->dz_cond : 0.0;
    if (!ok) (void)fail(RL_OK, std::string("direct solve not available: ") + why);
    return RL_OK;
}

extern "C" int rl_ski_project(rl_ski* s, const double* X, int nvec, double* out, int* rank,
                              void* stream) {
    if (!s || !X || !out) return fail(RL_EINVAL, "rl_ski_project: NULL argument");
    if (nvec < 0) return fail(RL_EINVAL, "rl_ski_project: nvec < 0");
    rl_gridop* g = s->g;
    bool ok = false;
    const char* why = "";
    RL_TRY(dz_ensure(s, &ok, &why));
    if (!ok) return fail(RL_ELIMIT, std::string("rl_ski_project: not available for this operator: ") + why);
    if (!s->dz_exact) return fail(RL_ELIMIT, "rl_ski_project: not every top row is in the polynomial form");
    if (rank) *rank = g->lr_r;
    if (nvec == 0) return RL_OK;
    RL_HIP(hipSetDevice(g->device));
    hipStream_t st = (hipStream_t)stream;
    RL_TRY(rp_prepare(s, std::max(nvec, g->lr_r)));
    const double* Xi = X;
    if (s->permuted) {
        RL_TRY(ski_reserve_perm(s, nvec));
        permute_rows(s, X, s->P1, nvec, 0, st);
        Xi = s->P1;
    }
#define RL_DZ_PROJ(R_) rp_project_plain<R_>(s, Xi, nvec, st)
    RL_DZ_RANKS(RL_DZ_PROJ);
#undef RL_DZ_PROJ
    RL_LAUNCH(k_dz_coeffs, dim3(nvec), dim3(256), 0, st, (const double*)s->rp_part,
              (const int*)s->rp_run_ptr, nvec, g->D, g->lr_r, (const double*)g->lr_nu, out);
    RL_HIP(hipGetLastError());
    return RL_OK;
}

extern "C" int rl_solve_direct(rl_ski* s, const double* B, double* X, int nrhs, double tol,
                               int max_refine, int* iters_out, double* resid_out, int* istop_out,
                               void* stream) {
    if (!s || !B || !X) return fail(RL_EINVAL, "rl_solve_direct: NULL argument");
    if (nrhs < 0) return fail(RL_EINVAL, "rl_solve_direct: nrhs < 0");
    if (!(tol > 0.0)) return fail(RL_EINVAL, "rl_solve_direct: tol must be > 0");
    if (max_refine < 0) return fail(RL_EINVAL, "rl_solve_direct: max_refine < 0");
    if (nrhs == 0) return RL_OK;
    rl_gridop* g = s->g;
    RL_HIP(hipSetDevice(g->device));
    hipStream_t st = (hipStream_t)stream;
    bool ok = false;
    const char* why = "";
    RL_TRY(dz_ensure(s, &ok, &why));
    if (!ok) return fail(RL_ELIMIT, std::string("rl_solve_direct: not available for this operator: ") + why);
    if (!s->dz_exact)
        return fail(RL_ELIMIT, "rl_solve_direct: not every top row is in the polynomial form -- the "
                               "factorisation is a preconditioner here (rl_solve_pcg)");
    const int n = s->n, R = g->lr_r;
    RL_TRY(rp_prepare(s, std::max(nrhs, R)));
    RL_TRY(ski_reserve(s, nrhs));
    RL_TRY(gridop_prepare(g, nrhs));
    if (rp_ok(s, nrhs)) RL_TRY(rp_prepare(s, nrhs));
    RL_TRY(ski_reserve_perm(s, nrhs));
    const size_t ve = (size_t)nrhs * n;
    if (s->dz_vec_cap < ve) {
        if (s->dz_res) RL_HIP(hipFree(s->dz_res));
        if (s->dz_cor) RL_HIP(hipFree(s->dz_cor));
        s->dz_res = s->dz_cor = nullptr;
        s->dz_vec_cap = 0;
        RL_HIP(hipMalloc((void**)&s->dz_res, ve * sizeof(double)));
        RL_HIP(hipMalloc((void**)&s->dz_cor, ve * sizeof(double)));
        s->dz_vec_cap = ve;
    }
    if (s->dz_rhs_cap < (size_t)nrhs) {
        if (s->dz_part) RL_HIP(hipFree(s->dz_part));
        if (s->dz_go) RL_HIP(hipFree(s->dz_go));
        s->dz_part = nullptr;
        s->dz_go = nullptr;
        s->dz_rhs_cap = 0;
        RL_HIP(hipMalloc((void**)&s->dz_part, (size_t)nrhs * (2 * RL_DZ_NBLK + 1) * sizeof(double)));
        RL_HIP(hipMalloc((void**)&s->dz_go, (size_t)nrhs * sizeof(int)));
        s->dz_rhs_cap = (size_t)nrhs;
    }
    const double* Bi = B;
    double* Xi = X;
    if (s->permuted) {
        permute_rows(s, B, s->P1, nrhs, 0, st);
        Bi = s->P1;
        Xi = s->P2;
    }
    const int nblk = std::max(1, std::min(RL_DZ_NBLK, (n + 1023) / 1024));
    double* norms = s->dz_part + (size_t)nrhs * RL_DZ_NBLK;
    std::vector<double> res((size_t)nrhs, 0.0), best((size_t)nrhs, 1e300);
    std::vector<int> go((size_t)nrhs, 1), its((size_t)nrhs, 1), stop((size_t)nrhs, 0);
    trace_once("solve: direct, through the polynomial form (k_rp_project / k_dz_mix / k_rp_expand)");
    RL_TRY(dz_apply(s, Bi, Xi, nrhs, st));
    for (int it = 0;; ++it) {
        RL_TRY(ski_mvm_int(s, Xi, s->dz_res, nrhs, st));
        RL_LAUNCH(k_dz_resid, dim3(nblk, nrhs), dim3(256), 256 * sizeof(double), st, Bi, s->dz_res, n,
                  s->dz_part);
        RL_LAUNCH(k_dz_norms, dim3((nrhs + 63) / 64), dim3(64), 0, st, (const double*)s->dz_part, nblk,
                  nrhs, norms);
        RL_HIP(hipGetLastError());
        RL_HIP(hipMemcpyAsync(res.data(), norms, (size_t)nrhs * sizeof(double), hipMemcpyDeviceToHost, st));
        RL_HIP(hipStreamSynchronize(st));
        int active = 0;
        for (int v = 0; v < nrhs; ++v) {
            if (!go[v]) continue;
            if (res[v] < tol) {
                go[v] = 0;
                stop[v] = RL_ISTOP_RESIDUAL;
            } else if (!std::isfinite(res[v]) || it >= max_refine) {
                go[v] = 0;
                stop[v] = RL_ISTOP_DIRECT_STALL;
            } else {
                ++active;
            }
        }
        if (active == 0) break;
// ... 524 lines not shown
```

Measured before the change: 329,700.

## Build direct-solve map on device with blocked dense Cholesky kernels

Moves construction of the direct-solve map (coupling matrix, sandwich products, Cholesky, triangular inverse, LAUUM, scaling) from host code to a chain of device kernels. The blocked dense routines are factored out of rl_exact into a shared header so both paths can use them. The aim is to avoid host-side O((DR)^3) factorisation and the host/device copies, at the cost of many small kernel launches. Whether the metric benefits depends on whether map rebuilds fall inside the timed MVM loop, which looks unlikely.

```diff
diff --git a/runlmc_amd/csrc/rl_dense.h b/runlmc_amd/csrc/rl_dense.h
--- /dev/null
+++ b/runlmc_amd/csrc/rl_dense.h
@@ -0,0 +1,111 @@
+#pragma once
+#include "rl_host.h"
+#include "rl_exact.h"
+
+struct DenseCtx {
+    double** ws;
+    size_t* ws_cap;
+    int ncu;
+    hipStream_t st;
+    const char* who;
+};
+
+static int dn_ws(const DenseCtx& c, size_t doubles) {
+    if (doubles <= *c.ws_cap) return RL_OK;
+    if (*c.ws) RL_HIP(hipFree(*c.ws));
+    *c.ws = nullptr;
+    *c.ws_cap = 0;
+    if (hipMalloc((void**)c.ws, doubles * sizeof(double)) != hipSuccess) {
+        (void)hipGetLastError();
+        return fail(RL_ENOMEM, std::string(c.who) + ": no device memory for a workspace of " +
+                                   std::to_string(doubles * 8 >> 20) + " MB");
+    }
+    *c.ws_cap = doubles;
+    return RL_OK;
+}
+
+static inline int dn_tiles(long long v) { return (int)((v + EX_T - 1) / EX_T); }
+static const size_t kGemmLds = 2 * EX_T * EX_LDK * sizeof(double);
+static const size_t kTileLds = 2 * EX_T * EX_LDT * sizeof(double);
+
+static int dn_gemm(const DenseCtx& c, double* C, long long ldc, const double* A, long long sai,
+                   long long sak, const double* B, long long sbj, long long sbk, int M, int N, int K,
+                   double s, int beta, int lower_tiles, int a_lower, bool via_partials) {
+    if (M <= 0 || N <= 0) return RL_OK;
+    const hipStream_t st = c.st;
+    const int tm = dn_tiles(M), tn = dn_tiles(N);
+    const long long ntile = lower_tiles ? (long long)tm * (tm + 1) / 2 : (long long)tm * tn;
+    const long long target = 2LL * c.ncu;
+    int nsplit = 1;
+    if (!lower_tiles && ntile < target) {
+        const long long want = (target + ntile - 1) / ntile;
+        const int kmax = dn_tiles(K);
+        nsplit = (int)(want < kmax ? want : kmax);
+    }
+    if (nsplit < 1) nsplit = 1;
+    int kchunk = (K + nsplit - 1) / nsplit;
+    kchunk = (kchunk + EX_KC - 1) / EX_KC * EX_KC;
+    if (kchunk < EX_KC) kchunk = EX_KC;
+    nsplit = (K + kchunk - 1) / kchunk;
+    if (nsplit < 1) nsplit = 1;
+    if (nsplit == 1 && !via_partials) {
+        RL_LAUNCH(k_ex_gemm, dim3(tn, tm, 1), dim3(256), kGemmLds, st, C, ldc, A, sai, sak, B, sbj,
+                  sbk, M, N, K, kchunk, a_lower, s, beta, lower_tiles, (double*)nullptr);
+        RL_HIP(hipGetLastError());
+        return RL_OK;
+    }
+    RL_TRY(dn_ws(c, (size_t)nsplit * M * N));
+    RL_LAUNCH(k_ex_gemm, dim3(tn, tm, nsplit), dim3(256), kGemmLds, st, C, ldc, A, sai, sak, B, sbj,
+              sbk, M, N, K, kchunk, a_lower, s, beta, 0, *c.ws);
+    RL_HIP(hipGetLastError());
+    const long long MN = (long long)M * N;
+    RL_LAUNCH(k_ex_reduce, dim3((unsigned)((MN + 255) / 256)), dim3(256), 0, st, C, ldc,
+              (const double*)*c.ws, M, N, nsplit, s, beta);
+    RL_HIP(hipGetLastError());
+    return RL_OK;
+}
+
+static int dn_potrf(const DenseCtx& c, double* A, int n, double* logd, int* flag) {
+    const hipStream_t st = c.st;
+    const int nb = dn_tiles(n);
+    for (int k = 0; k < nb; ++k) {
+        const int k0 = k * EX_T, nk = std::min(EX_T, n - k0), r0 = k0 + nk, rest = n - r0;
+        RL_LAUNCH(k_ex_potrf_diag, dim3(1), dim3(256), EX_T * EX_LDT * sizeof(double), st, A,
+                  (long long)n, k0, nk, logd, flag);
+        RL_HIP(hipGetLastError());
+        if (rest == 0) break;
+        RL_LAUNCH(k_ex_trsm_panel, dim3(dn_tiles(rest)), dim3(64), kTileLds, st, A, (long long)n,
+                  k0, nk, r0, rest);
+        RL_HIP(hipGetLastError());
+        double* L21 = A + (long long)r0 * n + k0;
+        RL_TRY(dn_gemm(c, A + (long long)r0 * n + r0, n, L21, n, 1, L21, n, 1, rest, rest, nk,
+                       -1.0, 1, 1, 0, false));
+    }
+    return RL_OK;
+}
+
+static int dn_trtri(const DenseCtx& c, double* A, int n, double* tmp) {
+    const hipStream_t st = c.st;
+    const int nb = dn_tiles(n);
+    for (int j = nb - 1; j >= 0; --j) {
+        const int j0 = j * EX_T, nj = std::min(EX_T, n - j0), r0 = j0 + nj, rest = n - r0;
+        RL_LAUNCH(k_ex_trtri_diag, dim3(1), dim3(64), kTileLds, st, A, (long long)n, j0, nj);
+        RL_HIP(hipGetLastError());
+        if (rest == 0) continue;
+        RL_TRY(dn_gemm(c, tmp, EX_T, A + (long long)r0 * n + r0, n, 1, A + (long long)r0 * n + j0, 1, n,
+                       rest, nj, rest, 1.0, 0, 0, 1, false));
+        RL_TRY(dn_gemm(c, A + (long long)r0 * n + j0, n, tmp, EX_T, 1, A + (long long)j0 * n + j0, 1, n,
+                       rest, nj, nj, -1.0, 0, 0, 0, false));
+    }
+    return RL_OK;
+}
+
+static int dn_lauum(const DenseCtx& c, double* A, int n) {
+    const int nb = dn_tiles(n);
+    for (int i = 0; i < nb; ++i) {
+        const int i0 = i * EX_T, ni = std::min(EX_T, n - i0);
+        RL_TRY(dn_gemm(c, A + (long long)i0 * n, n, A + (long long)i0 * n + i0, 1, n,
+                       A + (long long)i0 * n, 1, n, ni, i0 + ni, n - i0, 1.0, 0, 0, 0, true));
+    }
+    return RL_OK;
+}
diff --git a/runlmc_amd/csrc/rl_direct.h b/runlmc_amd/csrc/rl_direct.h
--- a/runlmc_amd/csrc/rl_direct.h
+++ b/runlmc_amd/csrc/rl_direct.h
@@ -330,3 +330,95 @@
         }
 #endif
 }
+
+static __global__ void __launch_bounds__(256)
+k_dzd_couple(const double* __restrict__ B, const double* __restrict__ C, int ldc, long long cq, int D,
+             int R, int Q, double* __restrict__ M) {
+    const int n = D * R, e = blockIdx.x * 256 + threadIdx.x;
+    if (e >= n * n) return;
+    const int r = e / n, c = e - r * n, a = r / R, i = r - a * R, b = c / R, j = c - b * R;
+    double acc = 0.0;
+    if (b <= a)
+        for (int q = 0; q < Q; ++q) {
+            const double bq = 0.5 * (B[((size_t)q * D + a) * D + b] + B[((size_t)q * D + b) * D + a]);
+            if (bq == 0.0) continue;
+            const double* Cq = C + (size_t)q * cq;
+            acc += bq * 0.5 * (Cq[(size_t)i * ldc + j] + Cq[(size_t)j * ldc + i]);
+        }
+    M[e] = acc;
+}
+static __global__ void __launch_bounds__(256)
+k_dzd_spd(double* __restrict__ S, int D, int R) {
+    const int n = D * R, e = blockIdx.x * 256 + threadIdx.x;
+    if (e >= n * n) return;
+    const int r = e / n, c = e - r * n;
+    if (c > r || c / R != r / R) return;
+    S[e] = c == r ? S[e] + 1.0 : 0.5 * (S[e] + S[(size_t)c * n + r]);
+}
+static __global__ void __launch_bounds__(256)
+k_dzd_pivots(const double* __restrict__ L, int n, const int* __restrict__ flag, double* __restrict__ out) {
+    RL_SMEM(smem);
+    double* red = reinterpret_cast<double*>(smem);
+    double* lo = red + 256;
+    double* hi = lo + 256;
+    const int tid = threadIdx.x;
+    double acc = 0.0, mn = 1e300, mx = 0.0;
+    for (int i = tid; i < n; i += 256) {
+        const double p = L[(size_t)i * n + i];
+        acc += 2.0 * log(p);
+        mn = p < mn ? p : mn;
+        mx = p > mx ? p : mx;
+    }
+    red[tid] = acc;
+    lo[tid] = mn;
+    hi[tid] = mx;
+    __syncthreads();
+    for (int w = 128; w > 0; w >>= 1) {
+        if (tid < w) {
+            red[tid] += red[tid + w];
+            lo[tid] = lo[tid + w] < lo[tid] ? lo[tid + w] : lo[tid];
+            hi[tid] = hi[tid + w] > hi[tid] ? hi[tid + w] : hi[tid];
+        }
+        __syncthreads();
+    }
+    if (tid == 0) {
+        out[0] = red[0];
+        out[1] = lo[0];
+        out[2] = hi[0];
+        out[3] = (double)*flag;
+    }
+}
+static __global__ void __launch_bounds__(256)
+k_dzd_complement(double* __restrict__ A, int n) {
+    const int e = blockIdx.x * 256 + threadIdx.x;
+    if (e >= n * n) return;
+    const int r = e / n, c = e - r * n;
+    if (c > r) return;
+    const double v = (c == r ? 1.0 : 0.0) - A[e];
+    A[e] = v;
+    A[(size_t)c * n + r] = v;
+}
+static __global__ void __launch_bounds__(256)
+k_dzd_factor_minus_eye(double* __restrict__ C, int n) {
+    const int e = blockIdx.x * 256 + threadIdx.x;
+    if (e >= n * n) return;
+    const int r = e / n, c = e - r * n;
+    if (c > r) C[e] = 0.0;
+    else if (c == r) C[e] -= 1.0;
+}
+static __global__ void __launch_bounds__(256)
+k_dzd_scale(const double* __restrict__ A, const double* __restrict__ nu, const double* __restrict__ eps,
+            int D, int R, int sample, double* __restrict__ out, double* __restrict__ bad) {
+    const int n = D * R, e = blockIdx.x * 256 + threadIdx.x;
+    if (e >= n * n) return;
+    const int r = e / n, c = e - r * n, a = r / R, i = r - a * R, b = c / R, j = c - b * R;
+    if (sample) {
+        out[(size_t)c * n + r] = b <= a ? nu[i] * A[e] * nu[j] : 0.0;
+        return;
+    }
+    if (c > r) return;
+    const double v = -(nu[i] / eps[a]) * A[e] * (nu[j] / eps[b]);
+    out[e] = v;
+    out[(size_t)c * n + r] = v;
+    if (!(fabs(v) <= 1.7976931348623157e308)) *bad = 1.0;
+}
diff --git a/runlmc_amd/csrc/rl_exact.h b/runlmc_amd/csrc/rl_exact.h
--- a/runlmc_amd/csrc/rl_exact.h
+++ b/runlmc_amd/csrc/rl_exact.h
@@ -275,7 +275,7 @@
 }
 
 #define EX_RD_CHUNKS 64
-__global__ void __launch_bounds__(256)
+static __global__ void __launch_bounds__(256)
 k_ex_rowdot_part(const double* __restrict__ B, const double* __restrict__ X, long long n,
                  double* __restrict__ part) {
     RL_SMEM(smem);
@@ -309,7 +309,7 @@
     }
 }
 
-__global__ void __launch_bounds__(64)
+static __global__ void __launch_bounds__(64)
 k_ex_rowdot_sum(const double* __restrict__ part, int k, double* __restrict__ dots,
                 double* __restrict__ sqn) {
     const int v = blockIdx.x * 64 + threadIdx.x;
@@ -323,7 +323,7 @@
     sqn[v] = sq;
 }
 
-__global__ void __launch_bounds__(256)
+static __global__ void __launch_bounds__(256)
 k_ex_potrf_diag(double* __restrict__ A, long long lda, int k0, int nk, double* __restrict__ logd,
                 int* __restrict__ flag) {
     RL_SMEM(smem);
@@ -356,7 +356,7 @@
     if (tid < nk) logd[k0 + tid] = log(s[tid * EX_LDT + tid]);
 }
 
-__global__ void __launch_bounds__(64)
+static __global__ void __launch_bounds__(64)
 k_ex_trsm_panel(double* __restrict__ A, long long lda, int k0, int nk, int r0, int nrows) {
     RL_SMEM(smem);
     double* L = reinterpret_cast<double*>(smem);
@@ -390,7 +390,7 @@
     }
 }
 
-__global__ void __launch_bounds__(64)
+static __global__ void __launch_bounds__(64)
 k_ex_trtri_diag(double* __restrict__ A, long long lda, int j0, int nk) {
     RL_SMEM(smem);
     double* L = reinterpret_cast<double*>(smem);
@@ -419,7 +419,7 @@
     }
 }
 
-__global__ void __launch_bounds__(64)
+static __global__ void __launch_bounds__(64)
 k_ex_trsv_diag(const double* __restrict__ A, long long lda, int k0, int nk, double* __restrict__ R,
                long long ldr, int nrhs, int trans) {
     RL_SMEM(smem);
@@ -461,7 +461,7 @@
     }
 }
 
-__global__ void __launch_bounds__(256)
+static __global__ void __launch_bounds__(256)
 k_ex_gemm(double* __restrict__ C, long long ldc, const double* __restrict__ A, long long sai,
           long long sak, const double* __restrict__ B, long long sbj, long long sbk, int M, int N,
           int K, int kchunk, int a_lower, double s, int beta, int lower_tiles,
@@ -540,7 +540,7 @@
 #endif
 }
 
-__global__ void __launch_bounds__(256)
+static __global__ void __launch_bounds__(256)
 k_ex_reduce(double* __restrict__ C, long long ldc, const double* __restrict__ P, int M, int N,
             int nsplit, double s, int beta) {
     const long long e = (long long)blockIdx.x * 256 + threadIdx.x;
@@ -553,7 +553,7 @@
     *c = beta ? *c + s * acc : s * acc;
 }
 
-__global__ void __launch_bounds__(256)
+static __global__ void __launch_bounds__(256)
 k_ex_rownorm2(const double* __restrict__ V, long long n, double* __restrict__ out) {
     RL_SMEM(smem);
     double* red = reinterpret_cast<double*>(smem);
@@ -569,7 +569,7 @@
     if (threadIdx.x == 0) out[blockIdx.x] = red[0];
 }
 
-__global__ void __launch_bounds__(256)
+static __global__ void __launch_bounds__(256)
 k_ex_sum2(const double* __restrict__ x, int n, double* __restrict__ out) {
     RL_SMEM(smem);
     double* red = reinterpret_cast<double*>(smem);
@@ -673,7 +673,7 @@
     }
 }
 
-__global__ void __launch_bounds__(64)
+static __global__ void __launch_bounds__(64)
 k_ex_grad_reduce(const double* __restrict__ part, const int* __restrict__ pair_start, int D,
                  int nslot, double* __restrict__ out) {
     const int p = blockIdx.x;
diff --git a/runlmc_amd/csrc/rl_exact.hip b/runlmc_amd/csrc/rl_exact.hip
--- a/runlmc_amd/csrc/rl_exact.hip
+++ b/runlmc_amd/csrc/rl_exact.hip
@@ -1,5 +1,6 @@
 #include "rl_host.h"
 #include "rl_exact.h"
+#include "rl_dense.h"
 
 enum { EX_EMPTY = 0, EX_SET, EX_ASSEMBLED, EX_FACTORED, EX_INVERTED };
 
@@ -33,19 +34,10 @@
     std::vector<int> lens, hbounds;
 };
 
-static int ex_ws(rl_exact* h, size_t doubles) {
-    if (doubles <= h->ws_cap) return RL_OK;
-    if (h->ws) RL_HIP(hipFree(h->ws));
-    h->ws = nullptr;
-    h->ws_cap = 0;
-    if (hipMalloc((void**)&h->ws, doubles * sizeof(double)) != hipSuccess) {
-        (void)hipGetLastError();
-        return fail(RL_ENOMEM, "rl_exact: no device memory for a workspace of " +
-                                   std::to_string(doubles * 8 >> 20) + " MB");
-    }
-    h->ws_cap = doubles;
-    return RL_OK;
-}
+static inline DenseCtx ex_ctx(rl_exact* h, hipStream_t st) {
+    return DenseCtx{&h->ws, &h->ws_cap, h->ncu, st, "rl_exact"};
+}
+static int ex_ws(rl_exact* h, size_t doubles) { return dn_ws(ex_ctx(h, nullptr), doubles); }
 
 #define EX_LAUNCH_FACT(h, kern, grid, block, smem, stream, ...)                         \
     do {                                                                                \
@@ -57,45 +49,14 @@
             RL_LAUNCH(kern<EX_MAX_FACT>, grid, block, smem, stream, __VA_ARGS__);       \
     } while (0)
 
-static inline int ex_tiles(long long v) { return (int)((v + EX_T - 1) / EX_T); }
-static const size_t kGemmLds = 2 * EX_T * EX_LDK * sizeof(double);
-static const size_t kTileLds = 2 * EX_T * EX_LDT * sizeof(double);
+static inline int ex_tiles(long long v) { return dn_tiles(v); }
 
 static int ex_gemm(rl_exact* h, hipStream_t st, double* C, long long ldc, const double* A,
                    long long sai, long long sak, const double* B, long long sbj, long long sbk,
                    int M, int N, int K, double s, int beta, int lower_tiles, int a_lower,
                    bool via_partials) {
-    if (M <= 0 || N <= 0) return RL_OK;
-    const int tm = ex_tiles(M), tn = ex_tiles(N);
-    const long long ntile = lower_tiles ? (long long)tm * (tm + 1) / 2 : (long long)tm * tn;
-    const long long target = 2LL * h->ncu;
-    int nsplit = 1;
-    if (!lower_tiles && ntile < target) {
-        const long long want = (target + ntile - 1) / ntile;
-        const int kmax = ex_tiles(K);
-        nsplit = (int)(want < kmax ? want : kmax);
-    }
-    if (nsplit < 1) nsplit = 1;
-    int kchunk = (K + nsplit - 1) / nsplit;
-    kchunk = (kchunk + EX_KC - 1) / EX_KC * EX_KC;
-    if (kchunk < EX_KC) kchunk = EX_KC;
-    nsplit = (K + kchunk - 1) / kchunk;
-    if (nsplit < 1) nsplit = 1;
-    if (nsplit == 1 && !via_partials) {
-        RL_LAUNCH(k_ex_gemm, dim3(tn, tm, 1), dim3(256), kGemmLds, st, C, ldc, A, sai, sak, B, sbj,
-                  sbk, M, N, K, kchunk, a_lower, s, beta, lower_tiles, (double*)nullptr);
-        RL_HIP(hipGetLastError());
-        return RL_OK;
-    }
-    RL_TRY(ex_ws(h, (size_t)nsplit * M * N));
-    RL_LAUNCH(k_ex_gemm, dim3(tn, tm, nsplit), dim3(256), kGemmLds, st, C, ldc, A, sai, sak, B, sbj,
-              sbk, M, N, K, kchunk, a_lower, s, beta, 0, h->ws);
-    RL_HIP(hipGetLastError());
-    const long long MN = (long long)M * N;
-    RL_LAUNCH(k_ex_reduce, dim3((unsigned)((MN + 255) / 256)), dim3(256), 0, st, C, ldc,
-              (const double*)h->ws, M, N, nsplit, s, beta);
-    RL_HIP(hipGetLastError());
-    return RL_OK;
+    return dn_gemm(ex_ctx(h, st), C, ldc, A, sai, sak, B, sbj, sbk, M, N, K, s, beta, lower_tiles,
+                   a_lower, via_partials);
 }
 
 static int ex_trsv(rl_exact* h, hipStream_t st, double* R, int nrhs, bool forward, bool backward) {
@@ -402,22 +363,10 @@
     if (bad_col) *bad_col = -1;
     if (h->state != EX_ASSEMBLED) RL_TRY(rl_exact_assemble(h));
     RL_HIP(hipSetDevice(h->device));
-    const int n = h->n, nb = ex_tiles(n);
+    const int n = h->n;
     const hipStream_t st = 0;
     RL_HIP(hipMemsetAsync(h->flag, 0x7f, sizeof(int), st));
-    for (int k = 0; k < nb; ++k) {
-        const int k0 = k * EX_T, nk = std::min(EX_T, n - k0), r0 = k0 + nk, rest = n - r0;
-        RL_LAUNCH(k_ex_potrf_diag, dim3(1), dim3(256), EX_T * EX_LDT * sizeof(double), st, h->A,
-                  (long long)n, k0, nk, h->logd, h->flag);
-        RL_HIP(hipGetLastError());
-        if (rest == 0) break;
-        RL_LAUNCH(k_ex_trsm_panel, dim3(ex_tiles(rest)), dim3(64), kTileLds, st, h->A, (long long)n,
-                  k0, nk, r0, rest);
-        RL_HIP(hipGetLastError());
-        double* L21 = h->A + (long long)r0 * n + k0;
-        RL_TRY(ex_gemm(h, st, h->A + (long long)r0 * n + r0, n, L21, n, 1, L21, n, 1, rest, rest, nk,
-                       -1.0, 1, 1, 0, false));
-    }
+    RL_TRY(dn_potrf(ex_ctx(h, st), h->A, n, h->logd, h->flag));
     RL_LAUNCH(k_ex_sum2, dim3(1), dim3(256), 256 * sizeof(double), st, (const double*)h->logd, n,
               h->scal);
     RL_HIP(hipGetLastError());
@@ -628,9 +577,7 @@
     if (h->state != EX_FACTORED)
         return fail(RL_EINVAL, "rl_exact_invert: the handle holds no Cholesky factor (rl_exact_factor)");
     RL_HIP(hipSetDevice(h->device));
-    const int n = h->n, nb = ex_tiles(n);
-    const long long ld = n;
-    double* A = h->A;
+    const int n = h->n;
     const hipStream_t st = 0;
     double* tmp = nullptr;
     if (hipMalloc((void**)&tmp, (size_t)n * EX_T * sizeof(double)) != hipSuccess) {
@@ -639,21 +586,8 @@
     }
     ExTmp guard;
     guard.p[0] = tmp;
-    for (int j = nb - 1; j >= 0; --j) {
-        const int j0 = j * EX_T, nj = std::min(EX_T, n - j0), r0 = j0 + nj, rest = n - r0;
-        RL_LAUNCH(k_ex_trtri_diag, dim3(1), dim3(64), kTileLds, st, A, ld, j0, nj);
-        RL_HIP(hipGetLastError());
-        if (rest == 0) continue;
-        RL_TRY(ex_gemm(h, st, tmp, EX_T, A + (long long)r0 * n + r0, n, 1, A + (long long)r0 * n + j0, 1, n,
-                       rest, nj, rest, 1.0, 0, 0, 1, false));
-        RL_TRY(ex_gemm(h, st, A + (long long)r0 * n + j0, n, tmp, EX_T, 1, A + (long long)j0 * n + j0, 1, n,
-                       rest, nj, nj, -1.0, 0, 0, 0, false));
-    }
-    for (int i = 0; i < nb; ++i) {
-        const int i0 = i * EX_T, ni = std::min(EX_T, n - i0);
-        RL_TRY(ex_gemm(h, st, A + (long long)i0 * n, n, A + (long long)i0 * n + i0, 1, n,
-                       A + (long long)i0 * n, 1, n, ni, i0 + ni, n - i0, 1.0, 0, 0, 0, true));
-    }
+    RL_TRY(dn_trtri(ex_ctx(h, st), h->A, n, tmp));
+    RL_TRY(dn_lauum(ex_ctx(h, st), h->A, n));
     RL_HIP(hipStreamSynchronize(st));
     h->state = EX_INVERTED;
     return RL_OK;
diff --git a/runlmc_amd/csrc/rl_gridop.hip b/runlmc_amd/csrc/rl_gridop.hip
--- a/runlmc_amd/csrc/rl_gridop.hip
+++ b/runlmc_amd/csrc/rl_gridop.hip
@@ -100,6 +100,8 @@
     k.precond_hi_min = num("RUNLMC_PRECOND_HI_MIN", 100000);
     k.precond_hi_rank = (int)num("RUNLMC_PRECOND_HI_RANK", 192);
     k.precond_hi_use = (int)num("RUNLMC_PRECOND_HI_USE", 0);
+    k.dz_device = (int)num("RUNLMC_DZ_DEVICE", -1);
+    if (k.dz_device != 0 && k.dz_device != 1) k.dz_device = -1;
     k.rp_fly = (int)num("RUNLMC_RP_FLY", 1);
     k.no_rp_small = flag("RUNLMC_NO_RP_SMALL");
     k.no_rp_fuse = flag("RUNLMC_NO_RP_FUSE");
diff --git a/runlmc_amd/csrc/rl_host.h b/runlmc_amd/csrc/rl_host.h
--- a/runlmc_amd/csrc/rl_host.h
+++ b/runlmc_amd/csrc/rl_host.h
@@ -71,6 +71,7 @@
     bool no_precond_approx = false;
     long long precond_hi_min = 100000;
     int precond_hi_use = 0;
+    int dz_device = -1;
     int precond_hi_rank = 192;
     bool no_precond_hi_mixed = false;
     bool precond_hi_passes = false;
@@ -339,6 +340,19 @@
     size_t dz_smp_cap = 0;
     double* dz_rec = nullptr;
     size_t dz_rec_cap = 0;
+    double* dzd_W[3] = {nullptr, nullptr, nullptr};
+    size_t dzd_W_cap = 0;
+    double* dzd_ws = nullptr;
+    size_t dzd_ws_cap = 0;
+    double* dzd_in = nullptr;
+    size_t dzd_in_cap = 0;
+    double* dzd_aux = nullptr;
+    size_t dzd_aux_cap = 0;
+    int dzd_ncu = 0;
+    std::vector<double> dzd_L;
+    unsigned long long dzd_L_ver = ~0ull;
+    int dzd_L_R = 0;
+    bool dzd_L_hz = false, dzd_L_dev = false;
     bool dz_hz = false;
     int hz_R = 0;
     bool hz_traced = false;
diff --git a/runlmc_amd/csrc/rl_ski.hip b/runlmc_amd/csrc/rl_ski.hip
--- a/runlmc_amd/csrc/rl_ski.hip
+++ b/runlmc_amd/csrc/rl_ski.hip
@@ -236,7 +236,8 @@
                     s->poly_part, s->rp_F, s->rp_Fc, s->rp_runs, s->rp_run_ptr, s->rp_out_end, s->rp_part, s->rp_nrm, s->rp_pp,
                     s->rp_base_c, s->rp_w4_c, s->dz_Zt, s->dz_inv, s->dz_res, s->dz_cor, s->dz_part,
                     s->dz_go, s->dz_p, s->dz_q, s->dz_scal, s->hz_beta, s->hz_phi, s->hz_tphi, s->hz_C,
-                    s->hz_F, s->hz_ones, s->hz_part, s->hz_zhat, s->hz_tmp, s->hz_S, s->hz_P, s->dz_Zh, s->dz_isq, s->dz_smp, s->dz_rec};
+                    s->hz_F, s->hz_ones, s->hz_part, s->hz_zhat, s->hz_tmp, s->hz_S, s->hz_P, s->dz_Zh, s->dz_isq, s->dz_smp, s->dz_rec,
+                    s->dzd_W[0], s->dzd_W[1], s->dzd_W[2], s->dzd_ws, s->dzd_in, s->dzd_aux};
     for (void* p : ptrs)
         if (p) (void)hipFree(p);
     delete s;
diff --git a/runlmc_amd/csrc/rl_solve.hip b/runlmc_amd/csrc/rl_solve.hip
--- a/runlmc_amd/csrc/rl_solve.hip
+++ b/runlmc_amd/csrc/rl_solve.hip
@@ -2,6 +2,7 @@
 #include "rl_solver.h"
 #include "rl_direct.h"
 #include "rl_loo.h"
+#include "rl_dense.h"
 
 void free_work(SolverWork& w) {
     for (double*& p : w.vec) { if (p) (void)hipFree(p); p = nullptr; }
@@ -948,6 +949,165 @@
     return true;
 }
 
+template <class T>
+static int hz_grow(T** p, size_t count) {
+    if (*p) RL_HIP(hipFree(*p));
+    *p = nullptr;
+    RL_HIP(hipMalloc((void**)p, count * sizeof(T)));
+    return RL_OK;
+}
+
+#define RL_DZ_DEVICE_MIN 480
+static bool dz_on_device(const rl_ski* s, int Dr) {
+    if (s->kn.dz_device >= 0) return s->kn.dz_device == 1;
+    return Dr >= RL_DZ_DEVICE_MIN;
+}
+
+static int dz_device_map(rl_ski* s, int D, int R, int Q, const double* U, const double* nu,
+                         const std::vector<double>& eps, const std::vector<int>& rows, const double* hB,
+                         const double* hC, bool hz, double* logdet_out, double* pmin_out, double* pmax_out,
+                         bool* ok, const char** why) {
+    *ok = false;
+    const int n = D * R;
+    const size_t RR = (size_t)R * R, nn = (size_t)n * n;
+    const hipStream_t st = nullptr;
+    if (s->dzd_L_ver != s->noise_ver || s->dzd_L_R != R || s->dzd_L_hz != hz || s->dzd_L.size() != 2 * D * RR) {
+        s->dzd_L_ver = ~0ull;
+        s->dzd_L_dev = false;
+        s->dzd_L.assign(2 * D * RR, 0.0);
+        std::vector<char> broke(D, 0);
+        dz_parallel(D, 1, [&](int first, int step) {
+            std::vector<double> L, Li;
+            for (int d = first; d < D; d += step) {
+                L.assign(RR, 0.0);
+                for (int i = 0; i < R; ++i)
+                    for (int j = 0; j < R; ++j) {
+                        const double u = 0.5 * (U[((size_t)d * R + i) * R + j] + U[((size_t)d * R + j) * R + i]);
+                        L[(size_t)i * R + j] = nu[i] * nu[j] * u / eps[d];
+                    }
+                if (!dz_chol(L, R)) { broke[d] = 1; continue; }
+                for (int i = 0; i < R; ++i)
+                    for (int j = i + 1; j < R; ++j) L[(size_t)i * R + j] = 0.0;
+                dz_tri_inverse(L, R, Li);
+                std::memcpy(s->dzd_L.data() + (size_t)d * RR, L.data(), RR * sizeof(double));
+                std::memcpy(s->dzd_L.data() + ((size_t)D + d) * RR, Li.data(), RR * sizeof(double));
+            }
+        });
+        for (int d = 0; d < D; ++d)
+            if (broke[d]) { *why = "an output has too few (or degenerate) rows for the basis"; return RL_OK; }
+        s->dzd_L_ver = s->noise_ver;
+        s->dzd_L_R = R;
+        s->dzd_L_hz = hz;
+    }
+    if (s->dzd_ncu == 0) {
+        hipDeviceProp_t prop;
+        RL_HIP(hipGetDeviceProperties(&prop, s->g->device));
+        s->dzd_ncu = std::max(1, prop.multiProcessorCount);
+    }
+    if (s->dzd_W_cap < nn) {
+        s->dzd_W_cap = 0;
+        for (double*& w : s->dzd_W) RL_TRY(hz_grow(&w, nn));
+        s->dzd_W_cap = nn;
+    }
+    const size_t small = (size_t)R + D + (size_t)Q * D * D + (size_t)Q * RR, in_len = 2 * D * RR + small;
+    if (s->dzd_in_cap < in_len) {
+        s->dzd_in_cap = 0;
+        s->dzd_L_dev = false;
+        RL_TRY(hz_grow(&s->dzd_in, in_len));
+        s->dzd_in_cap = in_len;
+    }
+    const size_t aux_len = (size_t)n + (size_t)n * EX_T + 8 + 1;
+    if (s->dzd_aux_cap < aux_len) {
+        s->dzd_aux_cap = 0;
+        RL_TRY(hz_grow(&s->dzd_aux, aux_len));
+        s->dzd_aux_cap = aux_len;
+    }
+    if (s->dz_Zt_cap < nn) {
+        s->dz_Zt_cap = 0;
+        RL_TRY(hz_grow(&s->dz_Zt, nn));
+        s->dz_Zt_cap = nn;
+    }
+    s->dz_Zh_valid = false;
+    if (s->dz_want_sample && s->dz_Zh_cap < nn) {
+        s->dz_Zh_cap = 0;
+        RL_TRY(hz_grow(&s->dz_Zh, nn));
+        s->dz_Zh_cap = nn;
+    }
+    double* const dL = s->dzd_in;
+    double* const dLi = dL + D * RR;
+    double* const dnu = dLi + D * RR;
+    const double* deps = dnu + R;
+    const double* dB = deps + D;
+    const double* dC = dB + (size_t)Q * D * D;
+    if (!s->dzd_L_dev) {
+        RL_HIP(hipMemcpy(dL, s->dzd_L.data(), 2 * D * RR * sizeof(double), hipMemcpyHostToDevice));
+        s->dzd_L_dev = true;
+    }
+    {
+        std::vector<double> in(small);
+        std::memcpy(in.data(), nu, (size_t)R * sizeof(double));
+        std::memcpy(in.data() + R, eps.data(), (size_t)D * sizeof(double));
+        std::memcpy(in.data() + R + D, hB, (size_t)Q * D * D * sizeof(double));
+        std::memcpy(in.data() + R + D + (size_t)Q * D * D, hC, (size_t)Q * RR * sizeof(double));
+        RL_HIP(hipMemcpy(dnu, in.data(), small * sizeof(double), hipMemcpyHostToDevice));
+    }
+    double* const W0 = s->dzd_W[0];
+    double* const W1 = s->dzd_W[1];
+    double* const W2 = s->dzd_W[2];
+    double* const logd = s->dzd_aux;
+    double* const panel = logd + n;
+    double* const res = panel + (size_t)n * EX_T;
+    int* const flag = reinterpret_cast<int*>(res + 8);
+    const DenseCtx cx{&s->dzd_ws, &s->dzd_ws_cap, s->dzd_ncu, st, "direct solve"};
+    const dim3 eg((unsigned)((nn + 255) / 256)), eb(256);
+    auto sandwich = [&](const double* X, const double* T, double* T1, double* out) -> int {
+        for (int b = 0; b < D; ++b) {
+            const size_t at = (size_t)b * R * n + (size_t)b * R;
+            RL_TRY(dn_gemm(cx, T1 + at, n, X + at, n, 1, T + b * RR, 1, R, (D - b) * R, R, R, 1.0, 0, 0, 0, false));
+        }
+        for (int a = 0; a < D; ++a) {
+            const size_t at = (size_t)a * R * n;
+            RL_TRY(dn_gemm(cx, out + at, n, T + a * RR, 1, R, T1 + at, 1, n, R, (a + 1) * R, R, 1.0, 0, 0, 0, false));
+        }
+        return RL_OK;
+    };
+    RL_HIP(hipMemsetAsync(res, 0, 8 * sizeof(double), st));
+    RL_HIP(hipMemsetAsync(flag, 0x7f, sizeof(int), st));
+    RL_LAUNCH(k_dzd_couple, eg, eb, 0, st, dB, dC, R, (long long)RR, D, R, Q, W0);
+    RL_TRY(sandwich(W0, dL, W1, W0));
+    RL_LAUNCH(k_dzd_spd, eg, eb, 0, st, W0, D, R);
+    RL_TRY(dn_potrf(cx, W0, n, logd, flag));
+    RL_LAUNCH(k_dzd_pivots, dim3(1), eb, 3 * 256 * sizeof(double), st, (const double*)W0, n, (const int*)flag, res);
+    if (s->dz_want_sample) RL_HIP(hipMemcpyAsync(W2, W0, nn * sizeof(double), hipMemcpyDeviceToDevice, st));
+    RL_TRY(dn_trtri(cx, W0, n, panel));
+    RL_TRY(dn_lauum(cx, W0, n));
+    RL_LAUNCH(k_dzd_complement, eg, eb, 0, st, W0, n);
+    RL_TRY(sandwich(W0, dLi, W1, W0));
+    RL_LAUNCH(k_dzd_scale, eg, eb, 0, st, (const double*)W0, (const double*)dnu, deps, D, R, 0, s->dz_Zt, res + 4);
+    if (s->dz_want_sample) {
+        RL_LAUNCH(k_dzd_factor_minus_eye, eg, eb, 0, st, W2, n);
+        RL_TRY(sandwich(W2, dLi, W1, W0));
+        RL_LAUNCH(k_dzd_scale, eg, eb, 0, st, (const double*)W0, (const double*)dnu, deps, D, R, 1, s->dz_Zh,
+                  (double*)nullptr);
+    }
+    RL_HIP(hipGetLastError());
+    double h[5];
+    RL_HIP(hipMemcpy(h, res, sizeof(h), hipMemcpyDeviceToHost));
+    if (h[3] >= 0.0 && h[3] < (double)n) {
+        *why = "I + L^T M L is not positive definite (M is not positive semi-definite to roundoff)";
+        return RL_OK;
+    }
+    if (h[4] != 0.0) { *why = "the solve map is not finite"; return RL_OK; }
+    double logdet = h[0];
+    for (int d = 0; d < D; ++d) logdet += rows[d] * std::log(eps[d]);
+    *logdet_out = logdet;
+    *pmin_out = h[1];
+    *pmax_out = h[2];
+    s->dz_Zh_valid = s->dz_want_sample;
+    *ok = true;
+    return RL_OK;
+}
+
 static_assert(RL_HZ_BLK == RL_RP_RMAX, "the blocks run the rank-48 kernels");
 #define RL_HZ_RDEF 192
 static int hz_rank(const rl_ski* s) {
@@ -958,13 +1118,6 @@
         if (s->g->m >= 8 * R && (double)s->n >= 1e5 * f * f * f) return R;
     }
     return 0;
-}
-template <class T>
-static int hz_grow(T** p, size_t count) {
-    if (*p) RL_HIP(hipFree(*p));
-    *p = nullptr;
-    RL_HIP(hipMalloc((void**)p, count * sizeof(T)));
-    return RL_OK;
 }
 
 static int dz_upload_sample_map(rl_ski* s, const std::vector<double>& Zh) {
@@ -1148,18 +1301,25 @@
         U = Usub.data();
     }
     std::vector<double> Zh;
-    if (!dz_host_map(D, R, Q, U, s->hz_hnu.data(), eps, rows, g->lr_hB.data(), hC.data(), Zs,
-                     &logdet, &pmin, &pmax, why, s->dz_want_sample ? &Zh : nullptr))
-        return RL_OK;
-    RL_TRY(dz_upload_sample_map(s, Zh));
-    for (double v : Zs)
-        if (!std::isfinite(v)) { *why = "the solve map is not finite"; return RL_OK; }
-    if (s->dz_Zt_cap < Zs.size()) {
-        s->dz_Zt_cap = 0;
-        RL_TRY(hz_grow(&s->dz_Zt, Zs.size()));
-        s->dz_Zt_cap = Zs.size();
-    }
-    RL_HIP(hipMemcpy(s->dz_Zt, Zs.data(), Zs.size() * sizeof(double), hipMemcpyHostToDevice));
+    if (dz_on_device(s, D * R)) {
+        bool map_ok = false;
+        RL_TRY(dz_device_map(s, D, R, Q, U, s->hz_hnu.data(), eps, rows, g->lr_hB.data(), hC.data(), true,
+                             &logdet, &pmin, &pmax, &map_ok, why));
+        if (!map_ok) return RL_OK;
+    } else {
+        if (!dz_host_map(D, R, Q, U, s->hz_hnu.data(), eps, rows, g->lr_hB.data(), hC.data(), Zs,
+                         &logdet, &pmin, &pmax, why, s->dz_want_sample ? &Zh : nullptr))
+            return RL_OK;
+        RL_TRY(dz_upload_sample_map(s, Zh));
+        for (double v : Zs)
+            if (!std::isfinite(v)) { *why = "the solve map is not finite"; return RL_OK; }
+        if (s->dz_Zt_cap < Zs.size()) {
+            s->dz_Zt_cap = 0;
+            RL_TRY(hz_grow(&s->dz_Zt, Zs.size()));
+            s->dz_Zt_cap = Zs.size();
+        }
+        RL_HIP(hipMemcpy(s->dz_Zt, Zs.data(), Zs.size() * sizeof(double), hipMemcpyHostToDevice));
+    }
     s->dz_logdet = logdet;
     s->dz_cond = (pmax / pmin) * (pmax / pmin);
     s->hz_Ruse = R;
@@ -1370,20 +1530,27 @@
     std::vector<double> Zs;
     double logdet = 0.0, pmin = 1.0, pmax = 1.0;
     std::vector<double> Zh;
-    if (!dz_host_map(D, R, Q, s->dz_U.data(), g->lr_hnu.data(), eps, rows, g->lr_hB.data(), hC, Zs, &logdet,
-                     &pmin, &pmax, why, s->dz_want_sample ? &Zh : nullptr))
-        return RL_OK;
-    RL_TRY(dz_upload_sample_map(s, Zh));
-    for (double v : Zs)
-        if (!std::isfinite(v)) { *why = "the solve map is not finite"; return RL_OK; }
-    if (s->dz_Zt_cap < Zs.size()) {
-        if (s->dz_Zt) RL_HIP(hipFree(s->dz_Zt));
-        s->dz_Zt = nullptr;
-        s->dz_Zt_cap = 0;
-        RL_HIP(hipMalloc((void**)&s->dz_Zt, Zs.size() * sizeof(double)));
-        s->dz_Zt_cap = Zs.size();
-    }
-    RL_HIP(hipMemcpy(s->dz_Zt, Zs.data(), Zs.size() * sizeof(double), hipMemcpyHostToDevice));
+    if (dz_on_device(s, Dr)) {
+        bool map_ok = false;
+        RL_TRY(dz_device_map(s, D, R, Q, s->dz_U.data(), g->lr_hnu.data(), eps, rows, g->lr_hB.data(), hC, false,
+                             &logdet, &pmin, &pmax, &map_ok, why));
+        if (!map_ok) return RL_OK;
+    } else {
+        if (!dz_host_map(D, R, Q, s->dz_U.data(), g->lr_hnu.data(), eps, rows, g->lr_hB.data(), hC, Zs, &logdet,
+                         &pmin, &pmax, why, s->dz_want_sample ? &Zh : nullptr))
+            return RL_OK;
+        RL_TRY(dz_upload_sample_map(s, Zh));
+        for (double v : Zs)
+            if (!std::isfinite(v)) { *why = "the solve map is not finite"; return RL_OK; }
+        if (s->dz_Zt_cap < Zs.size()) {
+            if (s->dz_Zt) RL_HIP(hipFree(s->dz_Zt));
+            s->dz_Zt = nullptr;
+            s->dz_Zt_cap = 0;
+            RL_HIP(hipMalloc((void**)&s->dz_Zt, Zs.size() * sizeof(double)));
+            s->dz_Zt_cap = Zs.size();
+        }
+        RL_HIP(hipMemcpy(s->dz_Zt, Zs.data(), Zs.size() * sizeof(double), hipMemcpyHostToDevice));
+    }
     s->dz_logdet = logdet;
     s->dz_cond = (pmax / pmin) * (pmax / pmin);
     s->dz_param_ver = g->param_ver;
```

New measurement: 299,600. -9.1%, worse.
